# ilya16/isp-tts

Measured on AMD Instinct MI355X. Metric: mel-frames/s (whole node), batch=64 x 512-frame utterances per GPU, full forward incl. MAS, higher is better.
Workload: dtype bf16; 1 GPU; BASELINE config 3: AcousticModel.forward (TextEncoder + Aligner/MAS + TemporalAdaptor 1 flow eval + MelDecoder + to_mel), fixed-length synthetic random-phoneme batch, random-init weights of the recipe architecture (23.2 M params); batch_per_gpu=64, global_batch=64, text_len=100, mel_len=512, parallelism=single GPU, device=gfx950:sramecc+:xnack-, compute_units=256, launch=HIP graph replay, batches_in_flight=1

## Files before the change

include/ispk.h:

```cpp
#ifndef ISPK_H
#define ISPK_H

#include <stdint.h>

#ifdef __cplusplus
extern "C" {
#endif

typedef struct ihipStream_t* ispk_stream_t;

#define ISPK_ABI_VERSION 2

#define ISPK_E_NULL (-1)
#define ISPK_E_SHAPE (-2)
#define ISPK_E_ALIGN (-3)
#define ISPK_E_UNSUPPORTED (-4)

int32_t ispk_abi_version(void);
const char* ispk_last_error_string(void);
int32_t ispk_device_info(char* name, int32_t cap);

int32_t ispk_mas_f32(const float* logits, const int64_t* text_len, const int64_t* mel_len, int16_t* attn_hard,
                     int64_t* dur, int16_t* path, int32_t B, int32_t M_max, int32_t L_max, int64_t stride_b,
                     int64_t stride_m, ispk_stream_t stream);

int32_t ispk_layernorm_f32(const float* x, int64_t ldx, const float* gamma, const float* beta, const float* ada_scale,
                           const float* ada_shift, int64_t ada_stride, int32_t rows_per_batch,
                           const uint8_t* row_mask, float* y, int64_t ldy, int32_t rows, int32_t D, float eps,
                           ispk_stream_t stream);
int32_t ispk_layernorm_f32_bf16(const float* x, int64_t ldx, const float* gamma, const float* beta,
                                const float* ada_scale, const float* ada_shift, int64_t ada_stride,
                                int32_t rows_per_batch, const uint8_t* row_mask, uint16_t* y, int64_t ldy, int32_t rows,
                                int32_t D, float eps, ispk_stream_t stream);

#define ISPK_EP_GELU 1u
#define ISPK_EP_SILU 2u
#define ISPK_EP_MASK_ACC 4u
#define ISPK_EP_MASK_OUT 8u
#define ISPK_EP_BIAS_ROW 16u
#define ISPK_EP_MASK_COL 32u
#define ISPK_EP_OUT_BF16 64u
#define ISPK_EP_RESID_BF16 128u
#define ISPK_EP_DUAL_GELU 1024u
#define ISPK_EP_GELU_BWD 2048u
#define ISPK_EP_OUT_SPLIT 512u
#define ISPK_EP_ROWS_T 256u

int32_t ispk_gemm_f32_tile(int32_t M, int32_t N, int32_t K);
int32_t ispk_gemm_f32(const float* A, int64_t lda, const float* W, int64_t ldw, float* C, int64_t ldc, const float* bias,
                      const float* resid, int64_t ldr, const uint8_t* mask, int32_t M, int32_t N, int32_t K,
                      uint32_t flags, int32_t cols_per_batch, int64_t batch_stride, ispk_stream_t stream);
int32_t ispk_gemm_f32_batched(const float* A, int64_t lda, int64_t stride_a, const float* W, int64_t ldw, int64_t stride_w,
                              float* C, int64_t ldc, int64_t stride_c, int32_t batch, int32_t M, int32_t N, int32_t K,
                              ispk_stream_t stream);
int32_t ispk_gemm_bf16_gelu_train(const uint16_t* A, int64_t lda, const uint16_t* W, int64_t ldw, uint16_t* u, int64_t ldu,
                                  uint16_t* a, int64_t ld_a, int32_t M, int32_t N, int32_t K, float dropout_p, uint64_t seed,
                                  ispk_stream_t stream);
int32_t ispk_gemm_bf16_gelu_bwd(const uint16_t* dY, int64_t lddy, const uint16_t* W2t, int64_t ldw, const uint16_t* u,
                                int64_t ldu, uint16_t* du, int64_t lddu, const uint8_t* row_mask, int32_t M, int32_t N,
                                int32_t K, float dropout_p, uint64_t seed, ispk_stream_t stream);
int32_t ispk_gemm_bf16_last_variant(void);
int32_t ispk_gemm_bf16(const uint16_t* A, int64_t lda, const uint16_t* W, int64_t ldw, void* C, int64_t ldc,
                       const float* bias, const void* resid, int64_t ldr, const uint8_t* mask, int32_t M, int32_t N,
                       int32_t K, uint32_t flags, int32_t cols_per_batch, int64_t batch_stride, ispk_stream_t stream);
int32_t ispk_gemm_bf16_splitk_plan(int32_t M, int32_t N, int32_t K, uint32_t flags);
int32_t ispk_gemm_bf16_splitk(const uint16_t* A, int64_t lda, const uint16_t* W, int64_t ldw, void* C, int64_t ldc,
                              const float* bias, const void* resid, int64_t ldr, const uint8_t* mask, int32_t M, int32_t N,
                              int32_t K, uint32_t flags, float* workspace, int32_t ksplit, ispk_stream_t stream);

int32_t ispk_ffn_bf16(const uint16_t* x, int64_t ldx, const uint16_t* W1, int64_t ldw1, const float* bias1,
                      const uint16_t* W2, int64_t ldw2, const float* bias2, const float* resid, int64_t ldr,
                      const uint8_t* mask, float* out, int64_t ldo, int32_t rows, int32_t dim, int32_t inner, uint32_t flags,
                      ispk_stream_t stream);

int32_t ispk_ffn_bf16_prenorm(const float* x, int64_t ldx, const float* norm_gamma, const float* norm_beta, float norm_eps,
                              const uint16_t* W1, int64_t ldw1, const uint16_t* W2_packed, const float* bias2,
                              const uint8_t* mask, float* out, int64_t ldo, int32_t rows, int32_t dim, int32_t inner,
                              uint32_t flags, float* row_stats, float stats_eps, ispk_stream_t stream);

int32_t ispk_ffn_chunk_w2_bf16(const uint16_t* W2, int64_t ldw2, int32_t dim, int32_t inner, uint16_t* out,
                               ispk_stream_t stream);
int32_t ispk_ffn_bf16_prenorm2_split(const float* x, int64_t ldx, const float* norm_gamma, const float* norm_beta,
                                     float norm_eps, const uint16_t* W1, const uint16_t* W2_chunks, float* parts,
                                     int64_t part_stride, int32_t splits, int32_t rows, int32_t dim, int32_t inner,
                                     ispk_stream_t stream);
int32_t ispk_ffn_combine_ln_f32(const float* x, int64_t ldx, const float* parts, int64_t part_stride, int32_t splits,
                                const uint8_t* mask, float* y, int64_t ldy, const float* ln_gamma, const float* ln_beta,
                                float ln_eps, int32_t ln_mask, void* ln_out, int64_t ld_ln, int32_t ln_bf16, int32_t rows,
                                int32_t dim, ispk_stream_t stream);
int32_t ispk_ffn_bf16_prenorm2(const float* x, int64_t ldx, const float* norm_gamma, const float* norm_beta, float norm_eps,
                               const uint16_t* W1, const uint16_t* W2_chunks, const uint8_t* mask, float* out, int64_t ldo,
                               int32_t rows, int32_t dim, int32_t inner, uint32_t flags, float* row_stats, float stats_eps,
                               ispk_stream_t stream);
int32_t ispk_attn_out_ffn_bf16(const float* x, int64_t ldx, const uint16_t* attn_out, int64_t ld_attn,
                               const uint16_t* Wo_chunks, const float* norm_gamma, const float* norm_beta, float norm_eps,
                               const uint16_t* W1, const uint16_t* W2_chunks, const uint8_t* mask, float* out, int64_t ldo,
                               int32_t rows, int32_t dim, int32_t inner, uint32_t flags, float* row_stats, float stats_eps,
                               ispk_stream_t stream);

int32_t ispk_attn_out_ffn_norm_bf16(const float* x, int64_t ldx, const uint16_t* attn_out, int64_t ld_attn,
                                    const uint16_t* Wo_chunks, const float* norm_gamma, const float* norm_beta, float norm_eps,
                                    const uint16_t* W1, const uint16_t* W2_chunks, const uint8_t* mask, float* out, int64_t ldo,
                                    int32_t rows, int32_t dim, int32_t inner, uint32_t flags, const float* final_gamma,
                                    const float* final_beta, float final_eps, int32_t ln_mask, void* ln_out, int64_t ld_ln,
                                    int32_t ln_bf16, ispk_stream_t stream);
int32_t ispk_attn_out_ffn_split_bf16(const float* x, int64_t ldx, const uint16_t* attn_out, int64_t ld_attn,
                                     const uint16_t* Wo_chunks, const float* norm_gamma, const float* norm_beta, float norm_eps,
                                     const uint16_t* W1, const uint16_t* W2_chunks, const uint8_t* mask, uint32_t flags,
                                     float* parts, int64_t part_stride, int32_t splits, int32_t rows, int32_t dim, int32_t inner,
                                     ispk_stream_t stream);
int32_t ispk_chunk_k16_bf16(const uint16_t* W, int64_t ldw, int32_t N, int32_t K, uint16_t* out, ispk_stream_t stream);
int32_t ispk_attn_out_ffn_qkv_bf16(const float* x, int64_t ldx, const uint16_t* attn_out, int64_t ld_attn,
                                   const uint16_t* Wo_chunks, const float* norm_gamma, const float* norm_beta, float norm_eps,
                                   const uint16_t* W1, const uint16_t* W2_chunks, const uint8_t* mask, float* out, int64_t ldo,
                                   int32_t rows, int32_t dim, int32_t inner, uint32_t flags, const float* next_gamma,
                                   const float* next_beta, float next_eps, const uint16_t* Wqkv_chunks, uint16_t* qkv,
                                   int64_t ld_qkv, ispk_stream_t stream);

int32_t ispk_gemm_bf16_lnin(const float* x, int64_t ldx, const float* row_stats, const float* ln_gamma, const float* ln_beta,
                            float ln_eps, const uint16_t* W, int64_t ldw, void* C, int64_t ldc, const float* bias, const void* resid,
                            int64_t ldr, const uint8_t* mask, int32_t M, int32_t N, int32_t K, uint32_t flags,
                            ispk_stream_t stream);

int32_t ispk_ffn_pack_w2_bf16(const uint16_t* W2, int64_t ldw2, int32_t dim, int32_t inner, uint16_t* packed,
                              ispk_stream_t stream);

int32_t ispk_linear_small_f32(const float* a, int64_t lda, const float* w, int64_t ldw, const float* bias,
                              const float* resid, int64_t ldr, float* out, int64_t ldo, int32_t M, int32_t N, int32_t K,
                              uint32_t act, ispk_stream_t stream);

int32_t ispk_alibi_mqa_attn_f32(const float* q, int64_t ldq, const float* k, const float* v, int64_t ldkv,
                                const float* slopes, const int64_t* key_len, float* out, int64_t ldo, int32_t B,
                                int32_t N, int32_t H, ispk_stream_t stream);
int32_t ispk_alibi_mqa_attn_bf16(const uint16_t* q, int64_t ldq, const uint16_t* k, const uint16_t* v, int64_t ldkv,
                                 const float* slopes, const int64_t* key_len, uint16_t* out, int64_t ldo, int32_t B,
                                 int32_t N, int32_t H, ispk_stream_t stream);
int32_t ispk_alibi_mqa_attn_bf16_tiles(const uint16_t* q, int64_t ldq, const uint16_t* k, const uint16_t* v, int64_t ldkv,
                                       const float* slopes, const int64_t* key_len, uint16_t* out, int64_t ldo, int32_t B,
                                       int32_t N, int32_t H, int32_t q_tiles_per_workgroup, ispk_stream_t stream);

int32_t ispk_pad_rows_f32(const float* x, int64_t stride_b, int64_t stride_t, int64_t stride_c, const int64_t* len,
                          void* out, int32_t out_bf16, int32_t B, int32_t T, int32_t C, ispk_stream_t stream);
int32_t ispk_masked_instnorm_f32(const float* y, const float* weight, const float* bias, const int64_t* len, void* out,
                                 int32_t out_bf16, int32_t B, int32_t T, int32_t C, float eps, ispk_stream_t stream);
int32_t ispk_aligner_scores_f32(const float* q_enc, int64_t q_stride_b, const float* k_enc, int64_t k_stride_b,
                                const int64_t* text_len, const int64_t* mel_len, float* attn_logits, float* attn_soft,
                                int32_t B, int32_t M, int32_t L, int32_t D, ispk_stream_t stream);
int32_t ispk_aligner_scores_fast_f32(const float* q_enc, int64_t q_stride_b, const float* k_enc, int64_t k_stride_b,
                                const int64_t* text_len, const int64_t* mel_len, float* attn_logits, float* attn_soft,
                                int32_t B, int32_t M, int32_t L, int32_t D, ispk_stream_t stream);
int32_t ispk_soft_average_f32(const float* attn_soft, const float* pitch, const float* energy, const int64_t* duration,
                              const int64_t* text_len, float* feats, int32_t B, int32_t M, int32_t L,
                              ispk_stream_t stream);

int32_t ispk_flow_head_f32(const float* y, int64_t ldy, const float* norm_gamma, const float* norm_beta, float norm_eps,
                           const float* W, const float* bias, const float* flow, const float* x0, const uint8_t* mask,
                           float* pred, float* duration, float* loss_ratio, float* loss_mean, float* workspace, int32_t B,
                           int32_t L, int32_t D, int32_t C, ispk_stream_t stream);
int32_t ispk_flow_euler_f32(const float* x_t, const float* velocity, float dt, const uint8_t* mask, float* out, int32_t B,
                            int32_t L, int32_t C, ispk_stream_t stream);
int32_t ispk_infer_features_f32(const float* pred, const float* duration_target_f32, const int64_t* duration_target_i64,
                                const float* pitch_target, const float* energy_target, float duration_factor, float pitch_factor,
                                float pitch_delta, float energy_factor, float energy_delta, float* duration, float* features,
                                int32_t B, int32_t L, ispk_stream_t stream);
int32_t ispk_infer_features_round_f32(const float* pred, const float* duration_target_f32, const int64_t* duration_target_i64,
                                      const float* pitch_target, const float* energy_target, float duration_factor,
                                      float pitch_factor, float pitch_delta, float energy_factor, float energy_delta,
                                      float* duration, float* features, int32_t B, int32_t L, ispk_stream_t stream);
int32_t ispk_flow_mix_f32(const float* x0, const float* x1, const float* t, float sigma, float* x_t, float* flow, int32_t B,
                          int32_t L, int32_t C, ispk_stream_t stream);
int32_t ispk_flow_finish_f32(const float* pred_raw, const float* flow, const float* x0, const uint8_t* mask, float* pred,
                             float* duration, float* loss_ratio, float* loss_mean, int32_t B, int32_t L, int32_t C,
                             ispk_stream_t stream);

int32_t ispk_embed_tokens_f32(const int64_t* text, const float* table, int64_t ld_table, int32_t vocab,
                              const int64_t* text_len, float* emb, uint8_t* mask, int32_t B, int32_t L, int32_t D,
                              ispk_stream_t stream);
int32_t ispk_add_speaker_f32(float* x, const float* table, int64_t ld_table, int32_t speakers, const int64_t* speaker,
                             int32_t id_stride, int32_t B, int32_t L, int32_t D, ispk_stream_t stream);
int32_t ispk_add_speaker_out_f32(const float* x, float* out, const float* table, int64_t ld_table, int32_t speakers,
                                 const int64_t* speaker, int32_t id_stride, int32_t B, int32_t L, int32_t D, ispk_stream_t stream);
int32_t ispk_speaker_grad_f32(const float* d_x, const int64_t* speaker, int32_t id_stride, const int64_t* text_len,
                              float* workspace, int64_t workspace_floats, float* d_table, int64_t ld_table, int32_t speakers,
                              int32_t B, int32_t L, int32_t D, int32_t accumulate, ispk_stream_t stream);
int32_t ispk_time_embedding_f32(const float* t, int32_t n, const float* inv_freq, const float* freq_scale, int32_t half_dim,
                                const float* w0, const float* b0, const float* w1, const float* b1, int32_t emb_dim,
                                float* out, ispk_stream_t stream);
int32_t ispk_length_regulate_f32(const float* alignment, const float* dur_f32, const int64_t* dur_i64, const int64_t* enc_len,
                                 const float* x, int64_t ldx, float* out, int64_t* dec_len, uint8_t* dec_mask, int32_t B,
                                 int32_t M, int32_t L, int32_t D, int32_t max_len, int32_t dur_cols, ispk_stream_t stream);
int32_t ispk_length_regulate_split_bf16(const float* alignment, const float* dur_f32, const int64_t* dur_i64, const int64_t* enc_len,
                                 const float* x, int64_t ldx, float* out, int64_t* dec_len, uint8_t* dec_mask, int32_t B,
                                 int32_t M, int32_t L, int32_t D, int32_t max_len, int32_t dur_cols, ispk_stream_t stream);
int32_t ispk_length_regulate_split_f16(const float* alignment, const float* dur_f32, const int64_t* dur_i64, const int64_t* enc_len,
                                const float* x, int64_t ldx, float* out, int64_t* dec_len, uint8_t* dec_mask, int32_t B,
                                int32_t M, int32_t L, int32_t D, int32_t max_len, int32_t dur_cols, ispk_stream_t stream);

int32_t ispk_hard_regulate_f32(const float* dur_f32, const int64_t* dur_i64, const float* x, int64_t ldx, float* out,
                               int64_t* dec_len, uint8_t* dec_mask, int32_t B, int32_t frames, int32_t L, int32_t D,
                               int32_t max_len, ispk_stream_t stream);
int32_t ispk_hard_regulate_bwd_f32(const float* dur_f32, const int64_t* dur_i64, const float* d_out, float* d_x, int32_t B,
                                   int32_t rows, int32_t L, int32_t D, int32_t max_len, ispk_stream_t stream);
int32_t ispk_hard_average_f32(const float* pitch, const float* energy, const int64_t* duration, const int64_t* text_len,
                              float* feats, int32_t B, int32_t M, int32_t L, ispk_stream_t stream);

int32_t ispk_transpose_f32(const float* x, int64_t ldx, float* y, int64_t ldy, int32_t rows, int32_t cols,
                           ispk_stream_t stream);
int32_t ispk_gemm_tn_f32(const float* A, int64_t lda, const float* B, int64_t ldb, float* C, int64_t ldc, int32_t M,
                         int32_t N1, int32_t N2, const uint8_t* row_mask, int32_t accumulate, float* workspace,
                         int64_t workspace_floats, ispk_stream_t stream);
int32_t ispk_gemm_tn_bf16(const float* A, int64_t lda, const float* B, int64_t ldb, float* C, int64_t ldc, int32_t M,
                          int32_t N1, int32_t N2, const uint8_t* row_mask, int32_t accumulate, float* workspace,
                          int64_t workspace_floats, ispk_stream_t stream);
int32_t ispk_gemm_tn_b16(const uint16_t* A, int64_t lda, const uint16_t* B, int64_t ldb, float* C, int64_t ldc, int32_t M,
                         int32_t N1, int32_t N2, const uint8_t* row_mask, int32_t accumulate, float* workspace,
                         int64_t workspace_floats, ispk_stream_t stream);
int32_t ispk_gemm_tn_last_plan(int32_t* splits, int32_t* rows_per_split);
int32_t ispk_gemm_tn_batched_f32(const float* A, int64_t lda, int64_t stride_a, const float* B, int64_t ldb, int64_t stride_b,
                                 float* C, int64_t ldc, int64_t stride_c, int32_t batch, int32_t M, int32_t N1, int32_t N2,
                                 const uint8_t* row_mask, int32_t accumulate, float* workspace, int64_t workspace_floats,
                                 ispk_stream_t stream);
int32_t ispk_layernorm_bwd_f32(const float* x, int64_t ldx, const float* dy, int64_t lddy, const float* gamma,
                               const uint8_t* row_mask, float* dx, int64_t lddx, int32_t add_to_dx, float* dgamma,
                               float* dbeta, float* workspace, int64_t workspace_floats, int64_t rows, int32_t dim,
                               float eps, ispk_stream_t stream);
int32_t ispk_layernorm_bwd_dual_f32(const float* x, int64_t ldx, const float* dy, int64_t lddy, const float* gamma,
                                    const uint8_t* row_mask, float* dx, int64_t lddx, int32_t add_to_dx, float* dgamma,
                                    float* dbeta, float* workspace, int64_t workspace_floats, int64_t rows, int32_t dim,
                                    float eps, uint16_t* dx_bf16, int64_t ld_dx_bf16, ispk_stream_t stream);
int32_t ispk_gelu_f32(const float* u, float* a, int64_t n, float dropout_p, uint64_t seed, ispk_stream_t stream);
int32_t ispk_gelu_bwd_f32(const float* da, const float* u, float* du, int64_t n, float dropout_p, uint64_t seed,
                          ispk_stream_t stream);
int32_t ispk_gelu_f32_bf16(const float* u, uint16_t* a, int64_t n, float dropout_p, uint64_t seed, ispk_stream_t stream);
int32_t ispk_gelu_bwd_bf16(const uint16_t* da, const float* u, uint16_t* du, int64_t n, float dropout_p, uint64_t seed,
                           ispk_stream_t stream);
int32_t ispk_gelu_bf16(const uint16_t* u, uint16_t* a, int64_t n, float dropout_p, uint64_t seed, ispk_stream_t stream);
int32_t ispk_gelu_bwd_b16(const uint16_t* da, const uint16_t* u, uint16_t* du, int64_t n, float dropout_p, uint64_t seed,
                          ispk_stream_t stream);
int32_t ispk_dropout_mask_u8(uint8_t* out, int64_t n, float dropout_p, uint64_t seed, ispk_stream_t stream);
int32_t ispk_alibi_mqa_attn_train_f32(const float* qkv, int64_t ld_qkv, const float* slopes, const int64_t* key_len, float* o,
                                      int64_t ld_o, float* lse, int32_t B, int32_t N, int32_t H, float dropout_p, uint64_t seed,
                                      ispk_stream_t stream);
int32_t ispk_alibi_mqa_attn_bwd_f32(const float* qkv, int64_t ld_qkv, const float* o, const float* d_o, int64_t ld_o,
                                    const float* slopes, const int64_t* key_len, float* dqkv, float* dlogslopes,
                                    float* workspace, int64_t workspace_floats, int32_t B, int32_t N, int32_t H,
                                    const float* lse_in, float dropout_p, uint64_t seed, ispk_stream_t stream);
int32_t ispk_alibi_mqa_attn_train_bf16(const uint16_t* qkv, int64_t ld_qkv, const float* slopes, const int64_t* key_len,
                                       uint16_t* o, int64_t ld_o, float* lse, int32_t B, int32_t N, int32_t H, float dropout_p,
                                       uint64_t seed, ispk_stream_t stream);
int32_t ispk_alibi_mqa_attn_bwd_bf16(const uint16_t* qkv, int64_t ld_qkv, const uint16_t* o, const uint16_t* d_o, int64_t ld_o,
                                     const float* slopes, const int64_t* key_len, const float* lse, uint16_t* dqkv,
                                     float* dlogslopes, float* workspace, int64_t workspace_floats, int32_t B, int32_t N,
                                     int32_t H, float dropout_p, uint64_t seed, ispk_stream_t stream);
int32_t ispk_mel_loss_f32(const float* mel_out, const float* mel_target, const int64_t* mel_len, float* ratio, float* loss,
                          float* grad, float grad_out, int32_t B, int32_t C, int32_t T, ispk_stream_t stream);
int32_t ispk_acoustic_metrics_f32(const float* mel_out, int64_t out_sb, int64_t out_sc, int64_t out_st, const float* mel_target,
                                  int64_t tgt_sb, int64_t tgt_sc, int64_t tgt_st, const int64_t* mel_len, const int64_t* text_len,
                                  const float* attn_soft, int64_t attn_sb, int64_t attn_st, const float* dct, float* workspace,
                                  int64_t workspace_floats, float* out, int32_t B, int32_t C, int32_t T, int32_t L,
                                  int32_t n_mfcc, ispk_stream_t stream);
int32_t ispk_dtw_f32(const float* cost, int64_t cost_sb, int64_t cost_sn, const int64_t* n_len, const int64_t* m_len,
                     float* total, int32_t* steps, int16_t* path, float* workspace, int64_t workspace_floats, int32_t B,
                     int32_t N, int32_t M, ispk_stream_t stream);
int32_t ispk_mcd_dtw_f32(const float* mel_out, int64_t out_sb, int64_t out_sc, int64_t out_st, const float* mel_target,
                         int64_t tgt_sb, int64_t tgt_sc, int64_t tgt_st, const float* dct, const int64_t* n_len,
                         const int64_t* m_len, const float* pitch_out, int64_t pitch_out_sb, const float* pitch_target,
                         int64_t pitch_target_sb, float* workspace, int64_t workspace_floats, float* per_item, float* means,
                         float* cost_out, int32_t B, int32_t C, int32_t N, int32_t M, int32_t n_mfcc, ispk_stream_t stream);
int32_t ispk_audio_features_f32(const float* audio, int64_t ld_audio, const int64_t* audio_len, const float* tables,
                                int64_t table_floats, const int32_t* fb_index, int32_t n_mels, float* mel, int64_t* mel_len, float* pitch, float* energy,
                                int32_t B, int32_t S, int32_t M, int32_t tau_min, int32_t tau_max, float sample_rate,
                                float threshold, float pitch_mean, float pitch_std, ispk_stream_t stream);
int32_t ispk_resample_f32(const float* audio, int64_t ld_b, int64_t ld_c, const int64_t* audio_len, const float* taps,
                          int64_t tap_floats, const int32_t* first, float* out, int64_t ld_out, int64_t* out_len, int32_t B,
                          int32_t C, int32_t S, int32_t S_out, int32_t orig, int32_t dest, int32_t width, int32_t T,
                          ispk_stream_t stream);
int32_t ispk_feature_stats_f64(const float* pitch, int64_t ld_pitch, const float* energy, int64_t ld_energy,
                               const int64_t* mel_len, double* partial, double* state, int32_t B, int32_t M, int32_t reset,
                               ispk_stream_t stream);
int32_t ispk_audio_measure_f64(const float* audio, int64_t ld_audio, const int64_t* audio_len, const double* table,
                               int64_t table_doubles, int64_t* bounds, double* loudness, float* peak, float* gain,
                               float* workspace, int64_t workspace_floats, int32_t B, int32_t S, int32_t sample_rate,
                               int32_t trim_mode, double trim_threshold, int32_t pad_frames, int32_t gain_mode,
                               double target_lufs, double peak_limit, ispk_stream_t stream);
int32_t ispk_audio_apply_f32(const float* audio, int64_t ld_audio, const int64_t* bounds, const float* gain, float* out,
                             int64_t ld_out, int64_t* out_len, int32_t B, int32_t S, int32_t S_out, ispk_stream_t stream);
int32_t ispk_pcm16(const float* audio, int64_t ld_audio, const int64_t* audio_len, int16_t* out, int64_t ld_out, int32_t B,
                   int32_t S, int32_t dither, uint64_t seed, ispk_stream_t stream);
int32_t ispk_vocoder_unfold(const void* mel, int32_t mel_f16, int64_t sb, int64_t sc, int64_t st, const int64_t* mel_len,
                            void* rows, int32_t rows_bf16, int64_t ldr, uint8_t* row_mask, int32_t B, int32_t C, int32_t T,
                            int32_t K, ispk_stream_t stream);
int32_t ispk_dwconv7_ln_f32(const float* x, int64_t ldx, const float* w, const float* bias, const float* gamma,
                            const float* beta, float eps, const int64_t* mel_len, void* y, int32_t y_bf16, int64_t ldy,
                            int32_t B, int32_t T, int32_t D, ispk_stream_t stream);
int32_t ispk_istft_head_f32(const float* h, int64_t ldh, const int64_t* mel_len, const float* tables, int64_t table_floats,
                            float* audio, int64_t ld_audio, int64_t* audio_len, int32_t B, int32_t T, int32_t S,
                            ispk_stream_t stream);
int32_t ispk_aligner_scores_bwd_f32(const float* attn_logits, const float* attn_soft, const float* d_soft, const float* d_logits,
                                    const int64_t* text_len, const int64_t* mel_len, float* dS, int64_t ld_s, float* dSt,
                                    int64_t ld_t, int32_t B, int32_t M, int32_t L, float scale, ispk_stream_t stream);
int32_t ispk_masked_instnorm_bwd_f32(const float* y, const float* d_out, const float* weight, const int64_t* lengths, float* d_y,
                                     float* d_weight, float* d_bias, float* workspace, int64_t workspace_floats, int32_t B,
                                     int32_t T, int32_t C, float eps, ispk_stream_t stream);
int32_t ispk_soft_average_bwd_f32(const float* attn_soft, const float* pitch, const float* energy, const float* d_feats,
                                  const int64_t* text_len, float* workspace, int64_t workspace_floats, float* d_attn,
                                  int32_t accumulate, int32_t B, int32_t M, int32_t L, ispk_stream_t stream);
int32_t ispk_flow_loss_bwd_f32(const float* pred_raw, const float* flow, const uint8_t* mask, float grad_out, float* d_raw, int32_t B,
                               int32_t L, int32_t C, ispk_stream_t stream);
int32_t ispk_adaln_bwd_f32(const float* x, int64_t ldx, const float* dy, int64_t lddy, const float* scale, int64_t ld_scale,
                           const uint8_t* row_mask, float* dx, int64_t lddx, int32_t add_to_dx, float* dscale, float* dshift,
                           int64_t ld_out, int32_t B, int32_t rows_per_batch, int32_t dim, float eps, ispk_stream_t stream);
int32_t ispk_time_embedding_bwd_f32(const float* t, int32_t n, const float* inv_freq, const float* freq_scale, int32_t half_dim,
                                    const float* w0, const float* b0, const float* w1, int32_t emb_dim, const float* d_out,
                                    float* dw0, float* db0, float* dw1, float* db1, ispk_stream_t stream);
int32_t ispk_attn_ctc_loss_f32(const float* attn_logits, const int64_t* text_len, const int64_t* mel_len, float blank_logprob,
                               float* workspace, int64_t workspace_floats, float* loss, float* grad, float grad_out, int32_t B,
                               int32_t M, int32_t L, ispk_stream_t stream);
int32_t ispk_attn_bin_loss_f32(const float* attn_soft, const int16_t* attn_hard, float eps, float* workspace, float* loss,
                               float* grad, float grad_out, int32_t B, int32_t M, int32_t L, ispk_stream_t stream);
int32_t ispk_mel_grad_rows_f32(const float* dmel, const uint8_t* mask, float* g, int32_t B, int32_t C, int32_t T,
                               ispk_stream_t stream);
int32_t ispk_colsum_f32(const float* x, int64_t ldx, int64_t rows, int32_t cols, const uint8_t* row_mask, float* workspace,
                        int64_t workspace_floats, float* out, ispk_stream_t stream);
int32_t ispk_smallk_wgrad_f32(const float* g, int64_t ldg, const float* x, int64_t ldx, int64_t rows, int32_t N, int32_t K,
                              float* workspace, int64_t workspace_floats, float* out, ispk_stream_t stream);
int32_t ispk_embedding_bwd_f32(const int64_t* ids, const float* d_emb, int64_t rows, int32_t dim, int32_t vocab,
                               int32_t padding_idx, float* d_table, int64_t ld_table, ispk_stream_t stream);
int32_t ispk_grad_sqnorm_f32(const float* g, int64_t n, float* partial, float* out, ispk_stream_t stream);
int32_t ispk_adamw_f32(float* p, const float* g, float* m, float* v, int64_t n, int64_t n_decay, float lr, float beta1,
                       float beta2, float eps, float weight_decay, int32_t step, const float* grad_sqnorm, float max_norm,
                       float grad_scale, ispk_stream_t stream);

int32_t ispk_split_f16(const float* x, int64_t ldx, uint16_t* hi, uint16_t* lo, int64_t ldy, int32_t rows, int32_t cols,
                       ispk_stream_t stream);
int32_t ispk_gemm_split_f16_tile(int32_t M, int32_t N, int32_t K);
int32_t ispk_gemm_split_f16(const uint16_t* A, int64_t lda, int64_t a_plane, const uint16_t* W, int64_t ldw, int64_t w_plane,
                            void* C, int64_t ldc, int64_t c_plane, const float* bias, const float* resid, int64_t ldr,
                            const uint8_t* mask, int32_t M, int32_t N, int32_t K, uint32_t flags, int32_t cols_per_batch,
                            int64_t batch_stride, ispk_stream_t stream);
int32_t ispk_layernorm_f32_split(const float* x, int64_t ldx, const float* gamma, const float* beta, const float* ada_scale,
                                 const float* ada_shift, int64_t ada_stride, int32_t rows_per_batch, const uint8_t* row_mask,
                                 uint16_t* y_hi, int64_t ldy, int64_t y_plane, int32_t rows, int32_t D, float eps,
                                 ispk_stream_t stream);
int32_t ispk_alibi_mqa_attn_split_f16(const float* q, int64_t ldq, const float* k, const float* v, int64_t ldkv,
                                      const float* slopes, const int64_t* key_len, void* out, int64_t ldo, int64_t o_plane,
                                      int32_t B, int32_t N, int32_t H, ispk_stream_t stream);
// ... 49 lines not shown
```

isp_tts_amd/acoustic/model.py:

```python
from __future__ import annotations

import warnings
from typing import NamedTuple, Optional

import torch
import torch.nn as nn
import torch.nn.functional as F
from torch import Tensor

from .. import runtime
from ..staging import StagedWeights
from ..modules.constructor import Constructor
from ..modules.transformer import Transformer
from ..utils import get_mask_from_lengths
from .alignment import Aligner, AlignerOutput
from .temporal_adaptor import FlowTemporalAdaptor, TemporalAdaptorOutput


class AcousticModelOutput(NamedTuple):
    mel: Tensor
    adaptor_output: TemporalAdaptorOutput
    aligner_output: AlignerOutput
    loss: Optional[Tensor] = None
    losses: Optional[dict] = None


class AcousticModel(nn.Module, Constructor):
    def __init__(self, encoding_map: dict, mel_dim: int, text_dim: int = 384, encoder=None, decoder=None,
                 temporal_adaptor=None, aligner=None, num_speakers: Optional[int] = 0, pitch_mean=None, pitch_std=None,
                 speaker_in_forward: bool = False):
        super().__init__()
        self.encoding_map = dict(encoding_map)
        self.mel_dim, self.text_dim = mel_dim, text_dim
        self.text_embedding = nn.Embedding(len(encoding_map), text_dim, padding_idx=0)
        self.encoder = Transformer.init(encoder, emb_dim=text_dim)
        enc_dim = self.encoder.dim
        self.aligner = Aligner.init(aligner, mel_dim=mel_dim, text_dim=enc_dim)
        self.speaker_embedding = None
        if (num_speakers or 0) > 0:
            self.speaker_embedding = nn.Embedding(num_speakers, enc_dim)
            nn.init.xavier_uniform_(self.speaker_embedding.weight)
        self.speaker_in_forward = bool(speaker_in_forward)
        self.train_amp: Optional[bool] = None
        self.temporal_adaptor = FlowTemporalAdaptor.init(temporal_adaptor, encoder_dim=enc_dim)
        self.decoder = Transformer.init(decoder, emb_dim=enc_dim)
        self.to_mel = nn.Linear(self.decoder.dim, mel_dim)
        self.overlap_streams = True
        self._side_streams: dict = {}
        self.register_buffer("pitch_mean", torch.tensor(float(pitch_mean or 0.)))
        self.register_buffer("pitch_std", torch.tensor(float(pitch_std or 1.)))
        self.compute_dtype = torch.float32
        self._cache = StagedWeights()

    def set_compute_dtype(self, dtype: torch.dtype, *, alignment_dtype: Optional[torch.dtype] = None):
        chain = alignment_dtype if alignment_dtype is not None else dtype
        assert chain in (torch.float32, torch.bfloat16, torch.float16)
        self.encoder.set_compute_dtype(chain)
        self.decoder.set_compute_dtype(dtype)
        self.temporal_adaptor.predictor.transformer.set_compute_dtype(dtype)
        self.temporal_adaptor.embedding.transformer.set_compute_dtype(dtype)
        self.aligner.attention.compute_dtype = chain
        self.temporal_adaptor.length_regulator.split_bf16 = (True if dtype == torch.bfloat16 else
                                                             "f16" if dtype == torch.float16 else False)
        self.compute_dtype = dtype
        return self

    def _to_mel(self, dec_out: Tensor, dec_mask: Optional[Tensor]) -> Tensor:
        w = self.to_mel.weight
        if dec_out.dtype == torch.float16:
            ws = self._cache.get(torch.float16, (w,), lambda: runtime.split_f16(w.detach().float().contiguous()))
            return runtime.to_mel_split(dec_out, ws, self.to_mel.bias, dec_mask)
        if dec_out.dtype == torch.bfloat16:
            w = self._cache.get(torch.bfloat16, (w,), lambda: w.detach().to(torch.bfloat16).contiguous())
        return runtime.to_mel(dec_out, w, self.to_mel.bias, dec_mask)

    def forward(self, text: Tensor, text_len: Tensor, mel: Tensor, mel_len: Tensor, pitch: Optional[Tensor] = None,
                energy: Optional[Tensor] = None, speaker: Optional[Tensor] = None, sigma: float = 0., steps: int = 1, *,
                flow_noise: Optional[Tensor] = None, flow_time: Optional[Tensor] = None) -> AcousticModelOutput:
        if self.speaker_embedding is None:
            speaker = None
        elif not self.speaker_in_forward:
            raise AttributeError(f"'{type(self).__name__}' object has no attribute 'speaker_encoder'")
        elif speaker is None:
            raise ValueError("speaker_in_forward is on and the model has a speaker table: forward() needs `speaker` "
                             "([B, 1] int64 ids, or a single id for the whole batch)")
        if torch.is_grad_enabled() and text.is_cuda and any(p.requires_grad for p in self.parameters()):
            from ..train.model import acoustic_train_outputs
            amp = self.train_amp if self.train_amp is not None else torch.is_autocast_enabled("cuda")
            train_aligner = any(p.requires_grad for p in self.aligner.parameters())
            with torch.autocast("cuda", enabled=False):
                return acoustic_train_outputs(self, text, text_len, mel, mel_len, pitch, energy, flow_noise, flow_time, amp=amp,
                                              train_aligner=train_aligner, speaker=speaker)
        with torch.no_grad():
            return self._forward_values(text, text_len, mel, mel_len, pitch, energy, flow_noise=flow_noise, flow_time=flow_time,
                                        speaker=speaker)

    def _forward_values(self, text: Tensor, text_len: Tensor, mel: Tensor, mel_len: Tensor, pitch: Optional[Tensor] = None,
                        energy: Optional[Tensor] = None, *, flow_noise: Optional[Tensor] = None,
                        flow_time: Optional[Tensor] = None, speaker: Optional[Tensor] = None) -> AcousticModelOutput:
        q_proj = None
        if mel.is_cuda and self.overlap_streams:
            main = torch.cuda.current_stream()
            side = self._side_streams.setdefault(mel.device, torch.cuda.Stream(device=mel.device))
            side.wait_stream(main)
            with torch.cuda.stream(side):
                q_proj = self.aligner.attention.project_queries(mel, mel_len)
        token_emb, enc_mask = runtime.embed_tokens(text, self.text_embedding.weight, text_len)
        enc_out = self.encoder(token_emb, mask=enc_mask, key_len=text_len).out
        if q_proj is not None:
            main.wait_stream(side)
            q_proj.record_stream(main)
        branch = side if q_proj is not None else None
        hard = not self.temporal_adaptor.soft_duration
        aligner_output = self.aligner(mel=mel, enc_text=enc_out.transpose(1, 2).detach(), mel_len=mel_len,
                                      text_len=text_len, q_proj=q_proj, mas_stream=None if hard else branch)
        if speaker is not None:
            enc_out = runtime.add_speaker(enc_out, self.speaker_embedding.weight, speaker)
        adaptor_output = self.temporal_adaptor(
            enc_out=enc_out, enc_mask=enc_mask, max_dec_len=mel.size(2),
            duration_target=aligner_output.attn_hard_duration, alignment=aligner_output.attn_soft,
            pitch_target_dense=pitch, energy_target_dense=energy, noise=flow_noise, time_steps=flow_time,
            enc_len=text_len, predictor_stream=branch, duration_sum=mel_len if branch is not None and not hard else None)
        dec_len = adaptor_output.dec_lengths
        dec_mask = adaptor_output.dec_mask
        dec_out = self.decoder(adaptor_output.enc_out, mask=dec_mask, key_len=dec_len, out_dtype=self.compute_dtype).out
        mel_out = self._to_mel(dec_out, dec_mask)
        if q_proj is not None:
            main.wait_stream(side)
            for t in (adaptor_output.log_duration, adaptor_output.duration, adaptor_output.pitch, adaptor_output.energy,
                      aligner_output.attn_hard, aligner_output.attn_hard_duration, *(adaptor_output.losses or {}).values()):
                if isinstance(t, Tensor):
                    t.record_stream(main)
        return AcousticModelOutput(mel=mel_out, adaptor_output=adaptor_output, aligner_output=aligner_output)

    @torch.no_grad()
    def forward_front(self, text: Tensor, text_len: Tensor, mel: Tensor, mel_len: Tensor, pitch: Tensor, energy: Tensor):
        main = torch.cuda.current_stream()
        side = self._side_streams.setdefault(mel.device, torch.cuda.Stream(device=mel.device))
        side.wait_stream(main)
        with torch.cuda.stream(side):
            q_proj = self.aligner.attention.project_queries(mel, mel_len)
        token_emb, enc_mask = runtime.embed_tokens(text, self.text_embedding.weight, text_len)
        enc_out = self.encoder(token_emb, mask=enc_mask, key_len=text_len).out
        main.wait_stream(side)
        q_proj.record_stream(main)
        attn_soft, attn_logits = self.aligner.attention(mel, enc_out.transpose(1, 2).detach(), mel_len, text_len,
                                                        q_proj=q_proj)
        feats = runtime.soft_average(attn_soft, pitch, energy, None, text_len)
        return {"enc_out": enc_out, "enc_mask": enc_mask, "attn_soft": attn_soft, "attn_logits": attn_logits, "feats": feats}

    @torch.no_grad()
    def forward_side(self, st: dict, text_len: Tensor, mel_len: Tensor, pitch: Tensor, energy: Tensor,
                     flow_noise: Optional[Tensor], flow_time: Optional[Tensor]):
        attn_hard, dur = self.aligner.binarize_attention_parallel(st["attn_logits"], text_len, mel_len, return_duration=True)
        ad = self.temporal_adaptor
        targets = runtime.soft_average(st["attn_soft"], pitch, energy, dur, text_len)
        pred, losses = ad.predictor(st["enc_out"], targets, st["enc_mask"][..., None], noise=flow_noise, time_steps=flow_time,
                                    key_len=text_len)
        return {"attn_hard": attn_hard, "dur": dur, "pred": pred, "losses": losses,
                "duration_pred": ad.predictor._duration_estimate}

    @torch.no_grad()
    def forward_back(self, st: dict, text_len: Tensor, mel_len: Tensor, max_dec_len: int):
        ad = self.temporal_adaptor
        feats = st["feats"]
        x = ad.embedding(feats[..., 1:3], mask=st["enc_mask"][..., None], key_len=text_len, residual=st["enc_out"])
        dec_in, dec_len = ad.length_regulator(x, mel_len.view(-1, 1), max_len=max_dec_len, alignment=st["attn_soft"])
        dec_mask = ad.length_regulator.dec_mask
        dec_out = self.decoder(dec_in, mask=dec_mask, key_len=dec_len, out_dtype=self.compute_dtype).out
        return {"mel": self._to_mel(dec_out, dec_mask), "dec_in": dec_in, "dec_len": dec_len, "dec_mask": dec_mask}

    @staticmethod
    def assemble_output(front: dict, side: dict, back: dict) -> AcousticModelOutput:
        feats, pred = front["feats"], side["pred"]
        adaptor = TemporalAdaptorOutput(enc_out=back["dec_in"], log_duration=pred[..., 0], duration=side["duration_pred"],
                                        dec_lengths=back["dec_len"], pitch=pred[..., 1], energy=pred[..., 2],
                                        pitch_target=feats[..., 1], energy_target=feats[..., 2], losses=side["losses"],
                                        dec_mask=back["dec_mask"])
        aligner = AlignerOutput(attn_soft=front["attn_soft"], attn_logits=front["attn_logits"], attn_hard=side["attn_hard"],
                                attn_hard_duration=side["dur"])
        return AcousticModelOutput(mel=back["mel"], adaptor_output=adaptor, aligner_output=aligner)

    @torch.no_grad()
    def infer(self, input_sequence: Tensor, text_lengths: Optional[Tensor] = None,
              duration_target: Optional[Tensor] = None, duration_factor: float = 1.0,
              pitch_target: Optional[Tensor] = None, pitch_factor: float = 1.0, pitch_delta: float = 0.,
              pitch_normalize: bool = False, energy_target: Optional[Tensor] = None, steps: int = 4,
              speaker: Optional[Tensor] = None, *, flow_noise: Optional[Tensor] = None,
              max_dec_len: Optional[int] = None):
        batch_infer = input_sequence.shape[0] > 1
        token_emb, enc_mask = runtime.embed_tokens(input_sequence, self.text_embedding.weight,
                                                   text_lengths if batch_infer else None, want_mask=batch_infer)
        enc_out = self.encoder(token_emb, mask=enc_mask, key_len=text_lengths if batch_infer else None).out
        if self.speaker_embedding is not None and speaker is not None:
            enc_out = runtime.add_speaker_(enc_out, self.speaker_embedding.weight, speaker)
        if pitch_normalize:
            if pitch_target is not None:
                pitch_target = (pitch_target - self.pitch_mean) / self.pitch_std
            pitch_delta = pitch_delta / self.pitch_std
        adaptor_output = self.temporal_adaptor.infer(
            enc_out=enc_out, enc_mask=enc_mask, duration_target=duration_target, pitch_target=pitch_target,
            energy_target=energy_target, duration_factor=duration_factor, pitch_factor=pitch_factor,
            pitch_delta=pitch_delta, steps=steps, noise=flow_noise, max_dec_len=max_dec_len,
            enc_len=text_lengths if batch_infer else None)
        dec_mask = adaptor_output.dec_mask if batch_infer else None
        dec_out = self.decoder(adaptor_output.enc_out, mask=dec_mask, key_len=adaptor_output.dec_lengths if batch_infer else None,
                               out_dtype=self.compute_dtype).out
        return self._to_mel(dec_out, dec_mask), adaptor_output

    @classmethod
    def from_pretrained(cls, checkpoint_path: str, strict: bool = True) -> "AcousticModel":
        checkpoint = torch.load(checkpoint_path, map_location="cpu", weights_only=False)
        model = cls.init(checkpoint["model"]["config"])
        state_dict = dict(checkpoint["model"]["state_dict"])
        for key, weight in model.state_dict().items():
            if key not in state_dict:
                state_dict[key] = weight
        model.load_state_dict(state_dict, strict=strict)
        return model

    def load(self, state_dict: dict, ignore_layers: Optional[list] = None, ignore_mismatched_keys: bool = False):
        own = self.state_dict()
        extra = [k for k in state_dict if k not in own]
        if extra:
            warnings.warn(f"checkpoint keys absent from the model are ignored: {extra}")
        kept = {k: v for k, v in state_dict.items() if k in own}
        ignored = []
        if ignore_mismatched_keys:
            ignored += [k for k, v in kept.items() if v.shape != own[k].shape]
        if ignore_layers:
            ignored += [k for k in kept if any(layer in k for layer in ignore_layers)]
        kept = {k: v for k, v in kept.items() if k not in ignored}
        own.update(kept)
        self.load_state_dict(own)
        return self

    def freeze(self, exception_list: Optional[list] = None):
        exception_list = exception_list or []
        for name, param in self.named_parameters():
            param.requires_grad = any(name.startswith(layer) for layer in exception_list)
        return self

    def extend_speakers(self, count: int) -> int:
        if self.speaker_embedding is None:
            raise ValueError("extend_speakers: the model has no speaker table (num_speakers = 0)")
        if count < 1:
            raise ValueError(f"extend_speakers: count = {count}")
        old = self.speaker_embedding.weight
        first = old.shape[0]
        table = nn.Embedding(first + count, old.shape[1], device=old.device, dtype=old.dtype)
        with torch.no_grad():
            table.weight[:first] = old
            table.weight[first:] = old.double().mean(dim=0).to(old.dtype)
        table.weight.requires_grad_(old.requires_grad)
        self.speaker_embedding = table
        return first

    def prepare_inputs(self, inputs: dict) -> dict:
        return {"text": inputs["text_vector"], "text_len": inputs["text_vector_len"], "mel": inputs["mel"],
                "mel_len": inputs["mel_len"], "pitch": inputs["pitch"], "energy": inputs["energy"],
                "speaker": inputs.get("speaker")}
```

isp_tts_amd/acoustic/temporal_adaptor.py:

```python
from __future__ import annotations

from typing import NamedTuple, Optional

import torch
import torch.nn as nn
import torch.nn.functional as F
from torch import Tensor

from .. import runtime
from ..staging import StagedWeights
from ..modules.constructor import Constructor
from ..modules.transformer import Transformer, TimePositionalEmbedding
from ..utils import get_float_mask_from_lengths, get_mask_3d, masked_mean


class TransformerTemporalModule(nn.Module, Constructor):

    def __init__(self, input_dim: int = 256, output_dim: int = 256, transformer=None, detach_inputs: bool = False):
        super().__init__()
        self.transformer = Transformer.init(transformer, emb_dim=input_dim)
        self.linear_layer = nn.Linear(self.transformer.dim, output_dim, bias=True)
        self.detach_inputs = detach_inputs
        self._cache = StagedWeights()

    def _weight(self, dtype: torch.dtype) -> Tensor:
        w = self.linear_layer.weight
        if dtype == torch.float16:
            return self._cache.get(dtype, (w,), lambda: runtime.split_f16(w.detach().float().contiguous()))
        return self._cache.get(dtype, (w,), lambda: w.detach().to(dtype).contiguous())

    def forward(self, x: Tensor, mask: Optional[Tensor] = None, *, key_len: Optional[Tensor] = None,
                residual: Optional[Tensor] = None) -> Tensor:
        m2 = mask[..., 0] if mask is not None else None
        cdt = self.transformer.layers[0].attention.compute_dtype
        out = self.transformer(x, mask=m2, out_dtype=cdt, key_len=key_len if m2 is not None else None).out
        flags = runtime.EP_MASK_ACC if m2 is not None else 0
        if cdt == torch.float16:
            return runtime.gemm_split(out, self._weight(cdt), bias=self.linear_layer.bias, mask=m2, flags=flags, resid=residual)
        return runtime.gemm(out, self._weight(cdt), bias=self.linear_layer.bias, mask=m2, flags=flags, resid=residual,
                            out_dtype=torch.float32)

    def infer(self, x: Tensor, mask: Optional[Tensor] = None, steps: int = 4) -> Tensor:
        return self.forward(x, mask)


class FlowTransformerTemporalModule(nn.Module, Constructor):

    def __init__(self, input_dim: int = 256, output_dim: int = 256, transformer=None,
                 time_embedding_dim: Optional[int] = None, sigma: float = 1e-5, detach_inputs: bool = False):
        super().__init__()
        time_embedding_dim = time_embedding_dim or input_dim
        self.time_embedding = TimePositionalEmbedding(freq_dim=64, emb_dim=time_embedding_dim, with_steps=True)
        self.transformer = Transformer.init(transformer, emb_dim=output_dim + input_dim, adaptive_norm=True,
                                            condition_dim=time_embedding_dim)
        self.linear_layer = nn.Linear(self.transformer.dim, output_dim, bias=True)
        self.output_dim, self.sigma, self.detach_inputs = output_dim, sigma, detach_inputs
        self.fused_head = True
        self._cache = StagedWeights()
        self._grids: dict = {}

    def _cond_weight(self, dtype: torch.dtype) -> Tensor:
        w = self.transformer.project_emb.weight
        if dtype == torch.float16:
            return self._cache.get(dtype, (w,), lambda: runtime.split_f16(w.detach()[:, self.output_dim:].float().contiguous()))
        return self._cache.get(dtype, (w,), lambda: w.detach()[:, self.output_dim:].to(dtype).contiguous())

    def _project(self, x_t: Tensor, cond_proj: Tensor) -> Tensor:
        w = self.transformer.project_emb.weight
        return runtime.linear_small(x_t.contiguous(), w[:, :self.output_dim], None, resid=cond_proj)

    def _cond_projection(self, cond: Tensor) -> Tensor:
        cdt = self.transformer.layers[0].attention.compute_dtype
        c = cond.float().contiguous()
        if cdt == torch.float16:
            return runtime.gemm_split(runtime.split_f16(c), self._cond_weight(cdt), bias=self.transformer.project_emb.bias)
        if cdt == torch.bfloat16:
            c = runtime.cast_bf16(c)
        return runtime.gemm(c, self._cond_weight(cdt), bias=self.transformer.project_emb.bias, out_dtype=torch.float32)

    def forward(self, x: Tensor, targets: Tensor, mask: Optional[Tensor] = None, *, noise: Optional[Tensor] = None,
                time_steps: Optional[Tensor] = None, key_len: Optional[Tensor] = None):
        cond = x
        have_mask = mask is not None
        if mask is None:
            mask = torch.ones(x.shape[:2], dtype=torch.bool, device=x.device)
        elif mask.ndim == 3:
            mask = mask[..., 0]
        x1 = targets.detach()
        x0 = torch.randn_like(x1) if noise is None else noise.to(x1)
        t = torch.rand((x1.shape[0],), dtype=x1.dtype, device=x1.device) if time_steps is None else time_steps.to(x1)
        time_emb = self.time_embedding(t)
        x_t, flow = runtime.flow_mix(x0, x1, t, self.sigma)
        proj = self._project(x_t, self._cond_projection(cond))
        tr = self.transformer
        head = (self.fused_head and tr.dim == 256 and self.output_dim == 3 and tr.norm.weight is not None and tr.norm.bias is not None
                and self.linear_layer.bias is not None)
        out = tr(None, mask=mask, adaptive_condition=time_emb, projected=proj, key_len=key_len if have_mask else None,
                 final_norm=not head).out
        if head:
            pred, self._duration_estimate, _, loss = runtime.flow_head(out, tr.norm.weight, tr.norm.bias, tr.norm.eps,
                                                                       self.linear_layer.weight, self.linear_layer.bias, flow, x0, mask)
            return pred, {"flow_loss": loss}
        raw = runtime.linear_small(out, self.linear_layer.weight, self.linear_layer.bias)
        pred, self._duration_estimate, _, loss = runtime.flow_finish(raw, flow, x0, mask)
        return pred, {"flow_loss": loss}

    def euler_grid(self, steps: int, step_factor: float, device=None) -> Tensor:
        assert step_factor <= 1.
        key = (int(steps), float(step_factor))
        grid = self._grids.get(key)
        if grid is None:
            if step_factor == 1.:
                grid = torch.linspace(0, 1, steps + 1)
            else:
                ts = -torch.diff(torch.logspace(0, steps, steps + 1, base=step_factor))
                ts = torch.cat([torch.zeros(1), ts])
                grid = torch.cumsum(ts / ts.sum(), dim=0)
            self._grids[key] = grid
        return grid if device is None else grid.to(device)

    def infer(self, x: Tensor, mask: Optional[Tensor] = None, steps: int = 4, step_factor: float = 0.75, *,
              noise: Optional[Tensor] = None, key_len: Optional[Tensor] = None) -> Tensor:
        dev = x.device
        if mask is not None and mask.ndim == 3:
            mask = mask.squeeze(-1)
        x_t = (torch.randn(x.shape[0], x.shape[1], self.output_dim, device=dev) if noise is None
               else noise.to(device=dev, dtype=torch.float32))
        dts = self._grids.get(("dt", int(steps), float(step_factor)))
        if dts is None:
            ts = self.euler_grid(steps, step_factor)
            dts = self._grids[("dt", int(steps), float(step_factor))] = (ts[1:] - ts[:-1]).tolist()
        temb = self.time_embedding(self._grid_on(dev, steps, step_factor)[:steps])
        cond_proj = self._cond_projection(x)
        if mask is not None and key_len is None:
            key_len = mask.sum(dim=1)
        for i in range(steps):
            out = self.transformer(None, mask=mask, adaptive_condition=temb[i].view(1, 1, -1),
                                   projected=self._project(x_t, cond_proj), key_len=key_len).out
            vel = runtime.linear_small(out, self.linear_layer.weight, self.linear_layer.bias)
            x_t = runtime.flow_euler(x_t, vel, dts[i], mask if i == steps - 1 else None)
        return x_t

    def _grid_on(self, device, steps: int, step_factor: float) -> Tensor:
        key = (str(device), int(steps), float(step_factor))
        g = self._grids.get(key)
        if g is None:
            g = self._grids[key] = self.euler_grid(steps, step_factor).to(device)
        return g


class TemporalAdaptorOutput(NamedTuple):
    enc_out: Tensor
    log_duration: Optional[Tensor]
    duration: Tensor
    dec_lengths: Tensor
    pitch: Optional[Tensor]
    energy: Optional[Tensor]
    pitch_target: Optional[Tensor]
    energy_target: Optional[Tensor]
    losses: Optional[dict] = None
    dec_mask: Optional[Tensor] = None


class LengthRegulator(nn.Module):
    split_bf16 = False

    def forward(self, x: Tensor, durations: Tensor, max_len: Optional[int] = None, alignment: Optional[Tensor] = None, *,
                enc_len: Optional[Tensor] = None, frames: Optional[int] = None, hard: bool = False):
        if alignment is None and (hard or frames is None or durations.dtype == torch.int64):
            if frames is None:
                frames = int((durations.float() + 0.5).long().sum(dim=1).max().item())
            if max_len is not None:
                frames = min(frames, max_len)
            if frames == 0:
                self.dec_mask = torch.zeros((x.shape[0], 0), dtype=torch.bool, device=x.device)
                return x.new_zeros((x.shape[0], 0, x.shape[2])), torch.zeros((x.shape[0],), dtype=torch.int64, device=x.device)
            out, dec_lens, self.dec_mask = runtime.hard_regulate(x.float(), durations, frames,
                                                                 max_len=-1 if max_len is None else max_len)
            return out, dec_lens
        rows = alignment.shape[1] if alignment is not None else frames
        if max_len is not None and alignment is not None:
            rows = min(rows, max_len)
            alignment = alignment[:, :rows]
        out, dec_lens, self.dec_mask = runtime.length_regulate(x.float(), durations, alignment, rows,
                                                               max_len=-1 if max_len is None else max_len, enc_len=enc_len,
                                                               split_bf16=self.split_bf16)
        return out, dec_lens


class TemporalAverager(nn.Module):

    def forward(self, x: Tensor, durations: Tensor, alignment: Optional[Tensor] = None) -> Tensor:
        if alignment is None:
            b, c, _ = x.shape
            if durations.dtype != torch.int64:
                ends = torch.cumsum(durations, dim=1).long()
                durations = torch.diff(ends, dim=1, prepend=torch.zeros_like(ends[:, :1]))
            every = torch.full((b,), durations.shape[1], dtype=torch.int64, device=x.device)
            cols = []
            for i in range(0, c, 2):
                f = runtime.hard_average(x[:, i], x[:, min(i + 1, c - 1)], durations, every)
                cols.append(f[..., 1:min(3, 1 + c - i)])
            return torch.cat(cols, dim=-1).transpose(1, 2)
        return x @ alignment / (alignment.sum(dim=1, keepdim=True) + 1e-5)


def generate_soft_path(duration: Tensor, mask: Tensor) -> Tensor:
    b, t_x, t_y = mask.shape
    cum = torch.cumsum(duration, 1).view(b * t_x)
    path = get_float_mask_from_lengths(cum, t_y).to(mask.dtype).view(b, t_x, t_y)
    path = path - F.pad(path, [0, 0, 1, 0, 0, 0])[:, :-1]
    return path * mask


class FlowTemporalAdaptor(nn.Module, Constructor):
    predictor_first = False

    def __init__(self, encoder_dim: int = 384, predictor=None, embedding=None, pitch: bool = True, energy: bool = True,
                 soft_duration: bool = False):
        super().__init__()
        if not (pitch and energy):
            raise NotImplementedError("built with pitch and energy both on (either duration mode): without one of them the "
                                      "feature tensors change shape")
        self.length_regulator = LengthRegulator()
        self.averager = TemporalAverager()
        self.encoder_dim = encoder_dim
        self.feature_dim = 3
        self.pitch, self.energy, self.soft_duration = pitch, energy, soft_duration
        self.pitch_idx, self.energy_idx = 1, 2
        self.predictor = FlowTransformerTemporalModule.init(predictor, input_dim=encoder_dim, output_dim=self.feature_dim)
        self.embedding = TransformerTemporalModule.init(embedding, input_dim=self.feature_dim - 1, output_dim=encoder_dim)

    def _process_target(self, dense: Tensor, duration_target: Tensor, alignment: Tensor, enc_mask: Tensor) -> Tensor:
        if dense.ndim == 2:
            dense = dense[:, None]
        return self.averager(dense, duration_target, alignment).transpose(1, 2) * enc_mask

    def forward(self, enc_out: Tensor, enc_mask: Tensor, max_dec_len: int, duration_target: Optional[Tensor] = None,
                alignment: Optional[Tensor] = None, pitch_target_dense: Optional[Tensor] = None,
                energy_target_dense: Optional[Tensor] = None, *, noise: Optional[Tensor] = None,
                time_steps: Optional[Tensor] = None, enc_len: Optional[Tensor] = None,
                predictor_stream=None, duration_sum: Optional[Tensor] = None) -> TemporalAdaptorOutput:
        assert duration_target is not None and (alignment is not None or not self.soft_duration)
        assert pitch_target_dense is not None and energy_target_dense is not None
        hard = not self.soft_duration
        m3 = enc_mask[..., None]
        if enc_len is None:
            enc_len = enc_mask.sum(dim=1)
        side = predictor_stream if (predictor_stream is not None and enc_out.is_cuda) else None
        cond = enc_out
        if hard:
            alignment = None
            targets = runtime.hard_average(pitch_target_dense, energy_target_dense, duration_target, enc_len)
            feats = targets
            len_src = duration_target
        elif side is None or duration_sum is None:
            targets = runtime.soft_average(alignment, pitch_target_dense, energy_target_dense, duration_target, enc_len)
            feats = targets
            len_src = duration_target
        else:
            feats = runtime.soft_average(alignment, pitch_target_dense, energy_target_dense, None, enc_len)
            targets = None
            len_src = duration_sum.view(-1, 1)
        if side is not None:
            ready = torch.cuda.Event()
            ready.record()
        pitch_target, energy_target = feats[..., 1:2], feats[..., 2:3]
        features = feats[..., 1:3]

        def decoder_input(enc_out_):
            enc_out_ = self.embedding(features, mask=m3, key_len=enc_len, residual=enc_out_)
            return self.length_regulator(enc_out_, len_src, max_len=max_dec_len, alignment=alignment,
                                         frames=max_dec_len if hard else None)

        if not (side is not None and self.predictor_first):
            enc_out, dec_lens = decoder_input(enc_out)

        def predict():
            tg = targets
            if tg is None:
                tg = runtime.soft_average(alignment, pitch_target_dense, energy_target_dense, duration_target, enc_len)
            pred_, losses_ = self.predictor(cond, tg, m3, noise=noise, time_steps=time_steps, key_len=enc_len)
            return pred_, losses_, self.predictor._duration_estimate

        if side is not None:
            side.wait_event(ready)
            with torch.cuda.stream(side):
                pred, losses, duration_pred = predict()
            for t in (cond, feats, alignment, pitch_target_dense, energy_target_dense):
                if t is not None:
                    t.record_stream(side)
            if self.predictor_first:
                enc_out, dec_lens = decoder_input(enc_out)
        else:
            pred, losses, duration_pred = predict()
        log_duration_pred = pred[..., 0]
        return TemporalAdaptorOutput(enc_out=enc_out, log_duration=log_duration_pred, duration=duration_pred,
                                     dec_lengths=dec_lens, pitch=pred[..., 1], energy=pred[..., 2],
                                     pitch_target=pitch_target.squeeze(-1), energy_target=energy_target.squeeze(-1),
                                     losses=losses, dec_mask=self.length_regulator.dec_mask)

    def infer(self, enc_out: Tensor, enc_mask: Optional[Tensor] = None, duration_target: Optional[Tensor] = None,
              duration_factor: float = 1.0, pitch_target: Optional[Tensor] = None, pitch_factor: float = 1.0,
              pitch_delta: float = 0., energy_target: Optional[Tensor] = None, energy_factor: float = 1.0,
              energy_delta: float = 0., steps: int = 4, *, noise: Optional[Tensor] = None,
              max_dec_len: Optional[int] = None, enc_len: Optional[Tensor] = None) -> TemporalAdaptorOutput:
        m3 = enc_mask[..., None] if enc_mask is not None else None
        pred = self.predictor.infer(enc_out, mask=m3, steps=steps, noise=noise, key_len=enc_len)
        duration_pred, feats = runtime.infer_features(pred, duration_target, pitch_target, energy_target, duration_factor,
                                                      pitch_factor, pitch_delta, energy_factor, energy_delta,
                                                      round_duration=not self.soft_duration)
        pitch, energy = feats[..., 0:1], feats[..., 1:2]
        enc_out = self.embedding(feats, residual=enc_out)
        enc_lens = enc_len
        if enc_lens is None and enc_mask is not None:
            enc_lens = enc_mask.sum(dim=1)
        if not self.soft_duration:
            enc_out, dec_lens = self.length_regulator(enc_out, duration_pred, alignment=None, frames=max_dec_len, hard=True)
            return TemporalAdaptorOutput(enc_out=enc_out, log_duration=None, duration=duration_pred, dec_lengths=dec_lens,
                                         pitch=pitch.squeeze(-1), energy=energy.squeeze(-1), pitch_target=pitch_target,
                                         energy_target=energy_target, dec_mask=self.length_regulator.dec_mask)
        if max_dec_len is None:
            max_dec_len = int((duration_pred.sum(dim=1) + 0.5).long().max().item())
        enc_out, dec_lens = self.length_regulator(enc_out, duration_pred, alignment=None, enc_len=enc_lens,
                                                  frames=max_dec_len)
        return TemporalAdaptorOutput(enc_out=enc_out, log_duration=None, duration=duration_pred, dec_lengths=dec_lens,
                                     pitch=pitch.squeeze(-1), energy=energy.squeeze(-1), pitch_target=pitch_target,
                                     energy_target=energy_target, dec_mask=self.length_regulator.dec_mask)
```

isp_tts_amd/csrc/glue.hip:

```cpp
#include "common.h"

namespace {

__global__ __launch_bounds__(256) void embed_tokens_kernel(const int64_t* __restrict__ text, const float* __restrict__ table,
                                                           int64_t ld_table, int vocab, const int64_t* __restrict__ text_len,
                                                           float* __restrict__ emb, uint8_t* __restrict__ mask, int rows,
                                                           int L, int D) {
    const int row = blockIdx.x * 4 + (threadIdx.x >> 6), lane = threadIdx.x & 63;
    if (row >= rows) return;
    int64_t id = text[row];
    id = (id < 0 || id >= vocab) ? 0 : id;
    const f32x4* src = reinterpret_cast<const f32x4*>(table + id * ld_table);
    f32x4* dst = reinterpret_cast<f32x4*>(emb + (int64_t)row * D);
    for (int c = lane; c < D / 4; c += 64) dst[c] = src[c];
    if (mask && lane == 0) {
        const int b = row / L, l = row - b * L;
        mask[row] = text_len ? (uint8_t)(l < text_len[b]) : (uint8_t)1;
    }
}

__device__ __forceinline__ int64_t speaker_row(const int64_t* __restrict__ speaker, int b, int id_stride, int speakers) {
    const int64_t id = speaker[(int64_t)b * id_stride];
    return id < 0 ? 0 : (id >= speakers ? speakers - 1 : id);
}

__global__ __launch_bounds__(256) void add_speaker_kernel(float* __restrict__ x, const float* __restrict__ table, int64_t ld_table,
                                                          int speakers, const int64_t* __restrict__ speaker, int id_stride,
                                                          int rows, int L, int D) {
    const int row = blockIdx.x * 4 + (threadIdx.x >> 6), lane = threadIdx.x & 63;
    if (row >= rows) return;
    const int64_t id = speaker_row(speaker, row / L, id_stride, speakers);
    const f32x4* src = reinterpret_cast<const f32x4*>(table + id * ld_table);
    f32x4* dst = reinterpret_cast<f32x4*>(x + (int64_t)row * D);
    for (int c = lane; c < D / 4; c += 64) {
        f32x4 v = dst[c];
        const f32x4 e = src[c];
        v[0] += e[0]; v[1] += e[1]; v[2] += e[2]; v[3] += e[3];
        dst[c] = v;
    }
}

__global__ __launch_bounds__(256) void add_speaker_out_kernel(const float* __restrict__ x, float* __restrict__ out,
                                                              const float* __restrict__ table, int64_t ld_table, int speakers,
                                                              const int64_t* __restrict__ speaker, int id_stride, int rows,
                                                              int L, int D) {
    const int row = blockIdx.x * 4 + (threadIdx.x >> 6), lane = threadIdx.x & 63;
    if (row >= rows) return;
    const int64_t id = speaker_row(speaker, row / L, id_stride, speakers);
    const f32x4* src = reinterpret_cast<const f32x4*>(table + id * ld_table);
    const f32x4* in = reinterpret_cast<const f32x4*>(x + (int64_t)row * D);
    f32x4* dst = reinterpret_cast<f32x4*>(out + (int64_t)row * D);
    for (int c = lane; c < D / 4; c += 64) {
        f32x4 v = in[c];
        const f32x4 e = src[c];
        v[0] += e[0]; v[1] += e[1]; v[2] += e[2]; v[3] += e[3];
        dst[c] = v;
    }
}

constexpr int kSgRows = 16;
__device__ __forceinline__ int speaker_grad_len(const int64_t* __restrict__ text_len, int b, int L) {
    if (!text_len) return L;
    const int64_t n = text_len[b];
    return n < 0 ? 0 : (n > L ? L : (int)n);
}

__global__ __launch_bounds__(256) void speaker_grad_stage1_kernel(const float* __restrict__ d_x, const int64_t* __restrict__ text_len,
                                                                  float* __restrict__ part, int L, int D, int chunks) {
    __shared__ f32x4 sums[3][64];
    const int b = blockIdx.z, chunk = blockIdx.y, wave = threadIdx.x >> 6, lane = threadIdx.x & 63;
    const int n = speaker_grad_len(text_len, b, L), r0 = chunk * kSgRows;
    if (r0 >= n) return;
    const int r1 = r0 + kSgRows < n ? r0 + kSgRows : n, c = blockIdx.x * 64 + lane;
    const bool live = c < D / 4;
    f32x4 s = {0.f, 0.f, 0.f, 0.f};
    if (live)
        for (int r = r0 + wave; r < r1; r += 4) {
            const f32x4 v = *reinterpret_cast<const f32x4*>(d_x + ((int64_t)b * L + r) * D + 4 * c);
            s[0] += v[0]; s[1] += v[1]; s[2] += v[2]; s[3] += v[3];
        }
    if (wave > 0) sums[wave - 1][lane] = s;
    __syncthreads();
    if (wave == 0 && live) {
#pragma unroll
        for (int w = 0; w < 3; ++w) {
            const f32x4 v = sums[w][lane];
            s[0] += v[0]; s[1] += v[1]; s[2] += v[2]; s[3] += v[3];
        }
        *reinterpret_cast<f32x4*>(part + ((int64_t)b * chunks + chunk) * D + 4 * c) = s;
    }
}

__global__ __launch_bounds__(256) void speaker_grad_stage2_kernel(const float* __restrict__ part, const int64_t* __restrict__ speaker,
                                                                  int id_stride, const int64_t* __restrict__ text_len,
                                                                  float* __restrict__ d_table, int64_t ld_table, int speakers,
                                                                  int B, int L, int D, int chunks, int accumulate) {
    __shared__ f32x4 sums[3][64];
    const int s = blockIdx.x, wave = threadIdx.x >> 6, lane = threadIdx.x & 63, c = blockIdx.y * 64 + lane;
    const bool live = c < D / 4;
    f32x4 acc = {0.f, 0.f, 0.f, 0.f};
    for (int b = wave; b < B; b += 4) {
        if (speaker_row(speaker, b, id_stride, speakers) != s) continue;
        const int nk = (speaker_grad_len(text_len, b, L) + kSgRows - 1) / kSgRows;
        const float* src = part + (int64_t)b * chunks * D + 4 * c;
        for (int k0 = 0; k0 < nk && live; k0 += 8) {
            f32x4 v[8];
#pragma unroll
            for (int u = 0; u < 8; ++u)
                if (k0 + u < nk) v[u] = *reinterpret_cast<const f32x4*>(src + (int64_t)(k0 + u) * D);
#pragma unroll
            for (int u = 0; u < 8; ++u)
                if (k0 + u < nk) { acc[0] += v[u][0]; acc[1] += v[u][1]; acc[2] += v[u][2]; acc[3] += v[u][3]; }
        }
    }
    if (wave > 0) sums[wave - 1][lane] = acc;
    __syncthreads();
    if (wave == 0 && live) {
#pragma unroll
        for (int w = 0; w < 3; ++w) {
            const f32x4 v = sums[w][lane];
            acc[0] += v[0]; acc[1] += v[1]; acc[2] += v[2]; acc[3] += v[3];
        }
        f32x4* dst = reinterpret_cast<f32x4*>(d_table + (int64_t)s * ld_table + 4 * c);
        if (accumulate) {
            const f32x4 old = *dst;
            acc[0] += old[0]; acc[1] += old[1]; acc[2] += old[2]; acc[3] += old[3];
        }
        *dst = acc;
    }
}

__global__ __launch_bounds__(64) void time_embedding_kernel(const float* __restrict__ t, const float* __restrict__ inv_freq,
                                                            const float* __restrict__ freq_scale, int H,
                                                            const float* __restrict__ w0, const float* __restrict__ b0,
                                                            const float* __restrict__ w1, const float* __restrict__ b1,
                                                            int E, float* __restrict__ out) {
#pragma clang fp contract(off)
    __shared__ float f[1 + 2 * 64];
    __shared__ float h[64];
    const int n = blockIdx.x, j = threadIdx.x;
    const float pos = t[n], fs = freq_scale[0];
    if (j == 0) f[0] = pos;
    for (int i = j; i < H; i += 64) {
        const float a = pos * fs * inv_freq[i];
        f[1 + i] = sinf(a);
        f[1 + H + i] = cosf(a);
    }
    __syncthreads();
    const int K0 = 1 + 2 * H;
    if (j < E) {
        float acc = b0[j];
        for (int k = 0; k < K0; ++k) acc = fmaf(f[k], w0[(int64_t)j * K0 + k], acc);
        h[j] = acc / (1.0f + expf(-acc));
    }
    __syncthreads();
    if (j < E) {
        float acc = b1[j];
        for (int k = 0; k < E; ++k) acc = fmaf(h[k], w1[(int64_t)j * E + k], acc);
        out[(int64_t)n * E + j] = acc;
    }
}

constexpr int kLrRows = 64, kLrChunk = 16, kLrAld = kLrChunk + 1;

typedef uint32_t lr_u32x4 __attribute__((ext_vector_type(4)));
typedef _Float16 lr_f16x8 __attribute__((ext_vector_type(8)));
template <int kSplit>
__device__ __forceinline__ void lr_split8(const float (&v)[8], bf16x8& hi, bf16x8& lo) {
    typedef float f2 __attribute__((ext_vector_type(2)));
    union { lr_u32x4 u; bf16x8 f; } h, l;
#pragma unroll
    for (int e = 0; e < 4; ++e) {
        f2 a;
        a.x = v[2 * e]; a.y = v[2 * e + 1];
        if constexpr (kSplit == 2) {
            typedef _Float16 h2 __attribute__((ext_vector_type(2)));
            a.x = __builtin_amdgcn_fmed3f(a.x, -65504.0f, 65504.0f);
            a.y = __builtin_amdgcn_fmed3f(a.y, -65504.0f, 65504.0f);
            h2 ph, pl;
            ph.x = (_Float16)a.x; ph.y = (_Float16)a.y;
            pl.x = (_Float16)(a.x - (float)ph.x); pl.y = (_Float16)(a.y - (float)ph.y);
            h.u[e] = __builtin_bit_cast(uint32_t, ph);
            l.u[e] = __builtin_bit_cast(uint32_t, pl);
        } else {
            typedef __bf16 bf2 __attribute__((ext_vector_type(2)));
            const uint32_t ph = __builtin_bit_cast(uint32_t, __builtin_convertvector(a, bf2));
            f2 r;
            r.x = a.x - __builtin_bit_cast(float, ph << 16);
            r.y = a.y - __builtin_bit_cast(float, ph & 0xffff0000u);
            h.u[e] = ph;
            l.u[e] = __builtin_bit_cast(uint32_t, __builtin_convertvector(r, bf2));
        }
    }
    hi = h.f;
    lo = l.f;
}
template <int kSplit>
__device__ __forceinline__ f32x16 lr_mfma(const bf16x8& a, const bf16x8& b, const f32x16& c) {
    if constexpr (kSplit == 2)
        return __builtin_amdgcn_mfma_f32_32x32x16_f16(__builtin_bit_cast(lr_f16x8, a), __builtin_bit_cast(lr_f16x8, b), c, 0, 0, 0);
    else
        return __builtin_amdgcn_mfma_f32_32x32x16_bf16(a, b, c, 0, 0, 0);
}

template <int NT, int kSplit = 0>
__global__ __launch_bounds__(256) void length_regulate_kernel(const float* __restrict__ align, const float* __restrict__ dur_f,
                                                              const int64_t* __restrict__ dur_i,
                                                              const int64_t* __restrict__ enc_len,
                                                              const float* __restrict__ x, int64_t ldx,
                                                              float* __restrict__ out, int64_t* __restrict__ dec_len,
                                                              uint8_t* __restrict__ dec_mask, int M, int L, int max_len,
                                                              int dur_cols) {
    constexpr int D = 128 * NT;
    extern __shared__ __attribute__((aligned(16))) char smem[];
    int64_t& s_dec = *reinterpret_cast<int64_t*>(smem);
    float* As = reinterpret_cast<float*>(smem + 16);
    float* Xs = As + kLrRows * kLrAld;
    float* cum = Xs + kLrChunk * D;
    const int b = blockIdx.y, y0 = blockIdx.x * kLrRows, tid = threadIdx.x, lane = tid & 63, wave = __builtin_amdgcn_readfirstlane(tid >> 6);
    const bool soft = align == nullptr;

    if (wave == 0) {
        int64_t dl;
        if (dur_i) {
            int64_t s = 0;
            for (int t = lane; t < dur_cols; t += 64) s += dur_i[(int64_t)b * dur_cols + t];
#pragma unroll
            for (int off = 32; off > 0; off >>= 1) s += __shfl_xor(s, off, 64);
            dl = (int64_t)((float)s + 0.5f);
        } else {
            float s = 0.f;
            if (lane == 0) {
                cum[0] = 0.f;
                for (int t = 0; t < L; ++t) {
                    s += dur_f[(int64_t)b * L + t];
                    cum[t + 1] = s;
                }
            }
            s = __builtin_bit_cast(float, __builtin_amdgcn_readfirstlane(__builtin_bit_cast(int, s)));
            dl = (int64_t)(s + 0.5f);
        }
        if (max_len >= 0 && dl > max_len) dl = max_len;
        if (lane == 0) {
            s_dec = dl;
            if (blockIdx.x == 0) dec_len[b] = dl;
        }
    }
    __syncthreads();
    const int64_t dl = s_dec;
    if (dec_mask)
        for (int r = tid; r < kLrRows; r += 256)
            if (y0 + r < M) dec_mask[(int64_t)b * M + y0 + r] = (uint8_t)(y0 + r < dl);
    const int el = enc_len ? (int)enc_len[b] : L;

    f32x16 acc[2][NT];
#pragma unroll
    for (int rt = 0; rt < 2; ++rt)
#pragma unroll
        for (int ct = 0; ct < NT; ++ct)
#pragma unroll
            for (int i = 0; i < 16; ++i) acc[rt][ct][i] = 0.f;

    const float* xb = x + (int64_t)b * L * ldx;
    const float* ab = soft ? nullptr : align + (int64_t)b * M * L;
    float ar[4];
    f32x4 xr[D / 64];
    const int a_row = tid >> 2, a_k = (tid & 3) * 4, x_t = tid >> 4, x_c = tid & 15;
    auto fetch = [&](int t0) {
        const int y = y0 + a_row;
#pragma unroll
        for (int u = 0; u < 4; ++u) {
            const int t = t0 + a_k + u;
            float v = 0.f;
            if (y < M && t < L) {
                if (!soft) {
                    v = ab[(int64_t)y * L + t];
                } else {
                    const float fy = (float)y;
                    const float hi = fminf(fmaxf(cum[t + 1] - fy, 0.f), 1.f), lo = fminf(fmaxf(cum[t] - fy, 0.f), 1.f);
                    v = (t < el && y < dl) ? hi - lo : 0.f;
                }
            }
            ar[u] = v;
        }
        const int t = t0 + x_t;
#pragma unroll
        for (int i = 0; i < D / 64; ++i) {
            f32x4 v = {0.f, 0.f, 0.f, 0.f};
            if (t < L) v = *reinterpret_cast<const f32x4*>(xb + (int64_t)t * ldx + (x_c + 16 * i) * 4);
            xr[i] = v;
        }
    };
    auto stash = [&]() {
#pragma unroll
        for (int u = 0; u < 4; ++u) As[a_row * kLrAld + a_k + u] = ar[u];
#pragma unroll
        for (int i = 0; i < D / 64; ++i) *reinterpret_cast<f32x4*>(Xs + x_t * D + (x_c + 16 * i) * 4) = xr[i];
    };

    fetch(0);
    for (int t0 = 0; t0 < L; t0 += kLrChunk) {
        __syncthreads();
        stash();
        __syncthreads();
        if (t0 + kLrChunk < L) fetch(t0 + kLrChunk);
        const int r = lane & 31, kh = lane >> 5;
        if constexpr (kSplit != 0) {
            bf16x8 ah[2], al[2];
#pragma unroll
            for (int rt = 0; rt < 2; ++rt) {
                float av[8];
#pragma unroll
                for (int e = 0; e < 8; ++e) av[e] = As[(32 * rt + r) * kLrAld + 8 * kh + e];
                lr_split8<kSplit>(av, ah[rt], al[rt]);
            }
#pragma unroll
            for (int ct = 0; ct < NT; ++ct) {
                float bv[8];
#pragma unroll
                for (int e = 0; e < 8; ++e) bv[e] = Xs[(8 * kh + e) * D + wave * (32 * NT) + ct * 32 + r];
                bf16x8 bh, bl;
                lr_split8<kSplit>(bv, bh, bl);
#pragma unroll
                for (int rt = 0; rt < 2; ++rt) {
                    acc[rt][ct] = lr_mfma<kSplit>(al[rt], bh, acc[rt][ct]);
                    acc[rt][ct] = lr_mfma<kSplit>(ah[rt], bl, acc[rt][ct]);
                    acc[rt][ct] = lr_mfma<kSplit>(ah[rt], bh, acc[rt][ct]);
                }
            }
            continue;
        }
#pragma unroll
        for (int kk = 0; kk < kLrChunk; kk += 2) {
            const float a0 = As[r * kLrAld + kk + kh], a1 = As[(32 + r) * kLrAld + kk + kh];
#pragma unroll
            for (int ct = 0; ct < NT; ++ct) {
                const float bv = Xs[(kk + kh) * D + wave * (32 * NT) + ct * 32 + r];
                acc[0][ct] = __builtin_amdgcn_mfma_f32_32x32x2f32(a0, bv, acc[0][ct], 0, 0, 0);
                acc[1][ct] = __builtin_amdgcn_mfma_f32_32x32x2f32(a1, bv, acc[1][ct], 0, 0, 0);
            }
        }
    }
    float* ob = out + (int64_t)b * M * D;
#pragma unroll
    for (int rt = 0; rt < 2; ++rt)
#pragma unroll
        for (int ct = 0; ct < NT; ++ct)
#pragma unroll
            for (int i = 0; i < 16; ++i) {
                const int y = y0 + rt * 32 + (i & 3) + 8 * (i >> 2) + 4 * (lane >> 5);
                if (y < M) ob[(int64_t)y * D + wave * (32 * NT) + ct * 32 + (lane & 31)] = acc[rt][ct][i];
            }
}

}

extern "C" int32_t ispk_embed_tokens_f32(const int64_t* text, const float* table, int64_t ld_table, int32_t vocab,
                                         const int64_t* text_len, float* emb, uint8_t* mask, int32_t B, int32_t L,
                                         int32_t D, ispk_stream_t stream) {
    ISPK_REQUIRE(text && table && emb, ISPK_E_NULL, "embed_tokens: null pointer");
    ISPK_REQUIRE(B >= 0 && L >= 1 && D >= 4 && vocab >= 1, ISPK_E_SHAPE, "embed_tokens: bad shape B=%d L=%d D=%d V=%d", B, L,
                 D, vocab);
    ISPK_REQUIRE(D % 4 == 0 && ld_table % 4 == 0 && ld_table >= D && ispk_aligned(table, 16) && ispk_aligned(emb, 16),
                 ISPK_E_ALIGN, "embed_tokens: D / ld_table must be multiples of 4 and table / emb 16-byte aligned");
    if (B == 0) return 0;
    const int rows = B * L;
    hipLaunchKernelGGL(embed_tokens_kernel, dim3((rows + 3) / 4), dim3(256), 0, reinterpret_cast<hipStream_t>(stream), text,
                       table, ld_table, vocab, text_len, emb, mask, rows, L, D);
    return ispk_launch_status();
}

extern "C" int32_t ispk_add_speaker_f32(float* x, const float* table, int64_t ld_table, int32_t speakers, const int64_t* speaker,
                                        int32_t id_stride, int32_t B, int32_t L, int32_t D, ispk_stream_t stream) {
    ISPK_REQUIRE(x && table && speaker, ISPK_E_NULL, "add_speaker: null pointer");
    ISPK_REQUIRE(B >= 0 && L >= 1 && D >= 4 && speakers >= 1 && (id_stride == 0 || id_stride == 1), ISPK_E_SHAPE,
                 "add_speaker: bad shape B=%d L=%d D=%d speakers=%d id_stride=%d", B, L, D, speakers, id_stride);
    ISPK_REQUIRE(D % 4 == 0 && ld_table % 4 == 0 && ld_table >= D && ispk_aligned(table, 16) && ispk_aligned(x, 16),
                 ISPK_E_ALIGN, "add_speaker: D / ld_table must be multiples of 4 and table / x 16-byte aligned");
    if (B == 0) return 0;
    const int rows = B * L;
    hipLaunchKernelGGL(add_speaker_kernel, dim3((rows + 3) / 4), dim3(256), 0, reinterpret_cast<hipStream_t>(stream), x, table,
                       ld_table, speakers, speaker, id_stride, rows, L, D);
    return ispk_launch_status();
}

extern "C" int32_t ispk_add_speaker_out_f32(const float* x, float* out, const float* table, int64_t ld_table, int32_t speakers,
                                            const int64_t* speaker, int32_t id_stride, int32_t B, int32_t L, int32_t D,
                                            ispk_stream_t stream) {
    ISPK_REQUIRE(x && out && table && speaker, ISPK_E_NULL, "add_speaker_out: null pointer");
    ISPK_REQUIRE(B >= 0 && L >= 1 && D >= 4 && speakers >= 1 && (id_stride == 0 || id_stride == 1), ISPK_E_SHAPE,
                 "add_speaker_out: bad shape B=%d L=%d D=%d speakers=%d id_stride=%d", B, L, D, speakers, id_stride);
    ISPK_REQUIRE(D % 4 == 0 && ld_table % 4 == 0 && ld_table >= D && ispk_aligned(table, 16) && ispk_aligned(x, 16) &&
                     ispk_aligned(out, 16),
                 ISPK_E_ALIGN, "add_speaker_out: D / ld_table must be multiples of 4 and table / x / out 16-byte aligned");
    ISPK_REQUIRE(x != out, ISPK_E_UNSUPPORTED, "add_speaker_out: x and out are the same buffer (ispk_add_speaker_f32 works in place)");
    if (B == 0) return 0;
    const int rows = B * L;
    hipLaunchKernelGGL(add_speaker_out_kernel, dim3((rows + 3) / 4), dim3(256), 0, reinterpret_cast<hipStream_t>(stream), x, out,
                       table, ld_table, speakers, speaker, id_stride, rows, L, D);
    return ispk_launch_status();
}

extern "C" int32_t ispk_speaker_grad_f32(const float* d_x, const int64_t* speaker, int32_t id_stride, const int64_t* text_len,
                                         float* workspace, int64_t workspace_floats, float* d_table, int64_t ld_table,
                                         int32_t speakers, int32_t B, int32_t L, int32_t D, int32_t accumulate,
                                         ispk_stream_t stream) {
    ISPK_REQUIRE(d_x && speaker && workspace && d_table, ISPK_E_NULL, "speaker_grad: null pointer");
    ISPK_REQUIRE(B >= 0 && B <= 65535 && L >= 1 && L <= 512 && D >= 4 && speakers >= 1 && (id_stride == 0 || id_stride == 1),
                 ISPK_E_SHAPE, "speaker_grad: bad shape B=%d L=%d (<= 512) D=%d speakers=%d id_stride=%d", B, L, D, speakers,
                 id_stride);
    ISPK_REQUIRE(D % 4 == 0 && ld_table % 4 == 0 && ld_table >= D && ispk_aligned(d_table, 16) && ispk_aligned(d_x, 16) &&
                     ispk_aligned(workspace, 16),
                 ISPK_E_ALIGN, "speaker_grad: D / ld_table must be multiples of 4 and d_x / d_table / workspace 16-byte aligned");
    const int chunks = (L + kSgRows - 1) / kSgRows;
    ISPK_REQUIRE(workspace_floats >= (int64_t)B * chunks * D, ISPK_E_SHAPE, "speaker_grad: workspace needs %lld floats (B * ceil(L / %d) * D)",
                 (long long)B * chunks * D, kSgRows);
    hipStream_t s = reinterpret_cast<hipStream_t>(stream);
    if (B > 0)
        hipLaunchKernelGGL(speaker_grad_stage1_kernel, dim3((D / 4 + 63) / 64, chunks, B), dim3(256), 0, s, d_x, text_len, workspace,
                           L, D, chunks);
    hipLaunchKernelGGL(speaker_grad_stage2_kernel, dim3(speakers, (D / 4 + 63) / 64), dim3(256), 0, s, workspace, speaker, id_stride, text_len, d_table,
                       ld_table, speakers, B, L, D, chunks, accumulate);
    return ispk_launch_status();
}

extern "C" int32_t ispk_time_embedding_f32(const float* t, int32_t n, const float* inv_freq, const float* freq_scale,
                                           int32_t half_dim, const float* w0, const float* b0, const float* w1,
                                           const float* b1, int32_t emb_dim, float* out, ispk_stream_t stream) {
    ISPK_REQUIRE(t && inv_freq && freq_scale && w0 && b0 && w1 && b1 && out, ISPK_E_NULL, "time_embedding: null pointer");
    ISPK_REQUIRE(n >= 0 && half_dim >= 1 && half_dim <= 64 && emb_dim >= 1 && emb_dim <= 64, ISPK_E_SHAPE,
                 "time_embedding: bad shape n=%d half_dim=%d emb_dim=%d (both <= 64)", n, half_dim, emb_dim);
    if (n == 0) return 0;
    hipLaunchKernelGGL(time_embedding_kernel, dim3(n), dim3(64), 0, reinterpret_cast<hipStream_t>(stream), t, inv_freq,
                       freq_scale, half_dim, w0, b0, w1, b1, emb_dim, out);
    return ispk_launch_status();
}

static int32_t length_regulate_launch(const float* alignment, const float* dur_f32, const int64_t* dur_i64, const int64_t* enc_len,
                                      const float* x, int64_t ldx, float* out, int64_t* dec_len, uint8_t* dec_mask, int32_t B,
                                      int32_t M, int32_t L, int32_t D, int32_t max_len, int32_t dur_cols, ispk_stream_t stream,
                                      int split) {
    ISPK_REQUIRE(x && out && dec_len, ISPK_E_NULL, "length_regulate: null pointer");
    ISPK_REQUIRE((dur_f32 != nullptr) != (dur_i64 != nullptr), ISPK_E_NULL,
                 "length_regulate: exactly one of dur_f32 / dur_i64 must be given");
    ISPK_REQUIRE(alignment || dur_f32, ISPK_E_NULL, "length_regulate: the soft path (alignment NULL) needs fp32 durations");
    ISPK_REQUIRE(dur_cols == L || (dur_i64 && dur_cols >= 1), ISPK_E_SHAPE,
                 "length_regulate: dur_cols=%d (L, or any width >= 1 for int64 durations that are only summed)", dur_cols);
    ISPK_REQUIRE(B >= 0 && M >= 1 && L >= 1 && L <= 4096 && B <= 65535, ISPK_E_SHAPE,
                 "length_regulate: bad shape B=%d M=%d L=%d", B, M, L);
    ISPK_REQUIRE(D == 256 || D == 384, ISPK_E_UNSUPPORTED, "length_regulate: dim %d (built for 256 / 384)", D);
    ISPK_REQUIRE(ldx % 4 == 0 && ldx >= D && ispk_aligned(x, 16) && ispk_aligned(out, 16), ISPK_E_ALIGN,
                 "length_regulate: x / out must be 16-byte aligned, ldx a multiple of 4");
    if (B == 0) return 0;
    const size_t lds = 16 + (size_t)(kLrRows * kLrAld + kLrChunk * D + L + 1) * sizeof(float);
    const dim3 grid((M + kLrRows - 1) / kLrRows, B);
    hipStream_t s = reinterpret_cast<hipStream_t>(stream);
#define ISPK_LR(NT_, SP_)                                                                                              \
    do {                                                                                                               \
        ISPK_RESERVE_LDS((&length_regulate_kernel<NT_, SP_>), lds, "length_regulate");                                 \
        hipLaunchKernelGGL((length_regulate_kernel<NT_, SP_>), grid, dim3(256), lds, s, alignment, dur_f32, dur_i64, enc_len, x, \
                           ldx, out, dec_len, dec_mask, M, L, max_len, dur_cols);                                      \
    } while (0)
    if (D == 384) { if (split == 2) ISPK_LR(3, 2); else if (split) ISPK_LR(3, 1); else ISPK_LR(3, 0); }
    else { if (split == 2) ISPK_LR(2, 2); else if (split) ISPK_LR(2, 1); else ISPK_LR(2, 0); }
#undef ISPK_LR
    return ispk_launch_status();
}

extern "C" int32_t ispk_length_regulate_f32(const float* alignment, const float* dur_f32, const int64_t* dur_i64,
                                            const int64_t* enc_len, const float* x, int64_t ldx, float* out,
                                            int64_t* dec_len, uint8_t* dec_mask, int32_t B, int32_t M, int32_t L, int32_t D,
                                            int32_t max_len, int32_t dur_cols, ispk_stream_t stream) {
    return length_regulate_launch(alignment, dur_f32, dur_i64, enc_len, x, ldx, out, dec_len, dec_mask, B, M, L, D, max_len, dur_cols,
                                  stream, 0);
}

extern "C" int32_t ispk_length_regulate_split_bf16(const float* alignment, const float* dur_f32, const int64_t* dur_i64,
                                                   const int64_t* enc_len, const float* x, int64_t ldx, float* out,
                                                   int64_t* dec_len, uint8_t* dec_mask, int32_t B, int32_t M, int32_t L,
                                                   int32_t D, int32_t max_len, int32_t dur_cols, ispk_stream_t stream) {
    return length_regulate_launch(alignment, dur_f32, dur_i64, enc_len, x, ldx, out, dec_len, dec_mask, B, M, L, D, max_len, dur_cols,
                                  stream, 1);
}

extern "C" int32_t ispk_length_regulate_split_f16(const float* alignment, const float* dur_f32, const int64_t* dur_i64,
                                                  const int64_t* enc_len, const float* x, int64_t ldx, float* out,
                                                  int64_t* dec_len, uint8_t* dec_mask, int32_t B, int32_t M, int32_t L,
                                                  int32_t D, int32_t max_len, int32_t dur_cols, ispk_stream_t stream) {
    return length_regulate_launch(alignment, dur_f32, dur_i64, enc_len, x, ldx, out, dec_len, dec_mask, B, M, L, D, max_len, dur_cols,
                                  stream, 2);
}
```

isp_tts_amd/graph.py:

```python
from __future__ import annotations

import gc
from typing import Optional

import torch
from torch import Tensor

from . import staging


class GraphedCall:

    def __init__(self, fn, warmup: int = 2):
        self._fn = fn
        side = torch.cuda.Stream()
        side.wait_stream(torch.cuda.current_stream())
        with torch.cuda.stream(side):
            for _ in range(warmup):
                self.out = fn()
        torch.cuda.current_stream().wait_stream(side)
        torch.cuda.synchronize()
        self.graph = torch.cuda.CUDAGraph()
        gc.collect()
        gc_was_on = gc.isenabled()
        gc.disable()
        try:
            with torch.cuda.graph(self.graph):
                self.out = fn()
        finally:
            if gc_was_on:
                gc.enable()
        self._staged_at_capture = staging.replacements()

    def replay(self):
        if staging.replacements() != self._staged_at_capture:
            raise RuntimeError("a staged weight image was rebuilt after this graph was captured (parameters changed: "
                               "load() / an optimizer step); the graph points at freed memory - capture a new one")
        self.graph.replay()
        return self.out


class GraphedForward(GraphedCall):
    def __init__(self, model, text: Tensor, text_len: Tensor, mel: Tensor, mel_len: Tensor, pitch: Tensor,
                 energy: Tensor, flow_noise: Optional[Tensor] = None, flow_time: Optional[Tensor] = None,
                 warmup: int = 2, *, speaker: Optional[Tensor] = None):
        self.model = model
        self.static = {"text": text.clone(), "text_len": text_len.clone(), "mel": mel.clone(), "mel_len": mel_len.clone(),
                       "pitch": pitch.clone(), "energy": energy.clone()}
        b, l = text.shape
        dev = text.device
        self.static["flow_noise"] = (flow_noise.clone() if flow_noise is not None
                                     else torch.randn(b, l, 3, device=dev))
        self.static["flow_time"] = flow_time.clone() if flow_time is not None else torch.rand(b, device=dev)
        if speaker is not None:
            self.static["speaker"] = speaker.clone()
        super().__init__(self._run, warmup)

    def _run(self):
        s = self.static
        with torch.no_grad():
            return self.model(s["text"], s["text_len"], s["mel"], s["mel_len"], s["pitch"], s["energy"],
                              speaker=s.get("speaker"), flow_noise=s["flow_noise"], flow_time=s["flow_time"])

    def __call__(self, **inputs: Tensor):
        for k, v in inputs.items():
            self.static[k].copy_(v)
        return self.replay()


class SegmentedForward:

    def __init__(self, model, text: Tensor, text_len: Tensor, mel: Tensor, mel_len: Tensor, pitch: Tensor, energy: Tensor,
                 flow_noise: Optional[Tensor] = None, flow_time: Optional[Tensor] = None, warmup: int = 2, side_priority: int = 0):
        if not model.temporal_adaptor.soft_duration:
            raise NotImplementedError("SegmentedForward is built for soft durations: its back piece (embedding stack, length "
                                      "regulator, decoder) is launched without waiting for the side piece, and with hard "
                                      "durations both its targets and its regulator read the MAS durations that piece computes; "
                                      "use GraphedForward")
        if model.speaker_embedding is not None and model.speaker_in_forward:
            raise NotImplementedError("SegmentedForward does not add the speaker rows (its three pieces hand the encoder output "
                                      "on as one tensor); use GraphedForward(..., speaker=ids)")
        b, l = text.shape
        dev = text.device
        s = self.static = {"text": text.clone(), "text_len": text_len.clone(), "mel": mel.clone(), "mel_len": mel_len.clone(),
                           "pitch": pitch.clone(), "energy": energy.clone(),
                           "flow_noise": flow_noise.clone() if flow_noise is not None else torch.randn(b, l, 3, device=dev),
                           "flow_time": flow_time.clone() if flow_time is not None else torch.rand(b, device=dev)}
        self.model, self.side = model, torch.cuda.Stream(device=dev, priority=side_priority)
        frames = mel.shape[2]
        self.g_front = GraphedCall(lambda: model.forward_front(s["text"], s["text_len"], s["mel"], s["mel_len"], s["pitch"],
                                                               s["energy"]), warmup)
        st = self.g_front.out
        self.side.wait_stream(torch.cuda.current_stream())
        with torch.cuda.stream(self.side):
            self.g_side = GraphedCall(lambda: model.forward_side(st, s["text_len"], s["mel_len"], s["pitch"], s["energy"],
                                                                 s["flow_noise"], s["flow_time"]), warmup)
        torch.cuda.current_stream().wait_stream(self.side)
        self.g_back = GraphedCall(lambda: model.forward_back(st, s["text_len"], s["mel_len"], frames), warmup)
        self.out = model.assemble_output(st, self.g_side.out, self.g_back.out)
        self.front_done, self.side_done = torch.cuda.Event(), torch.cuda.Event()

    def replay(self):
        main = torch.cuda.current_stream()
        self.g_front.replay()
        self.front_done.record(main)
        self.side.wait_event(self.front_done)
        with torch.cuda.stream(self.side):
            self.g_side.replay()
            self.side_done.record(self.side)
        self.g_back.replay()
        main.wait_event(self.side_done)
        return self.out

    def __call__(self, **inputs: Tensor):
        for k, v in inputs.items():
            self.static[k].copy_(v)
        return self.replay()


class GraphedForwardLanes:

    def __init__(self, model, *inputs, lanes: int = 2, calibrate: bool = True, **kw):
        self.dev = inputs[0].device
        self.lanes = [(GraphedForward(model, *inputs, **kw), None) for _ in range(max(1, lanes))]
        self.count = 0
        self._new_streams()
        self.overlap = None
        if calibrate and len(self.lanes) > 1:
            for _ in range(6):
                one, alt = self._time(False), self._time(True)
                self.overlap = one / alt
                if alt < 0.93 * one:
                    break
                self._new_streams()

    def _new_streams(self) -> None:
        self.lanes = [(g, torch.cuda.Stream(device=self.dev)) for g, _ in self.lanes]
        for _, stream in self.lanes:
            with torch.cuda.stream(stream):
                torch.zeros(1, device=self.dev)
        torch.cuda.synchronize()

    def _time(self, alternate: bool, n: int = 6) -> float:
        import time
        torch.cuda.synchronize()
        t0 = time.perf_counter()
        for k in range(n):
            g, stream = self.lanes[k % len(self.lanes) if alternate else 0]
            with torch.cuda.stream(stream):
                g.replay()
        torch.cuda.synchronize()
        return (time.perf_counter() - t0) / n

    def __len__(self) -> int:
        return len(self.lanes)

    def next_lane(self):
        lane = self.lanes[self.count % len(self.lanes)]
        self.count += 1
        return lane

    def replay(self):
        g, stream = self.next_lane()
        stream.wait_stream(torch.cuda.current_stream())
        with torch.cuda.stream(stream):
            return g.replay()
```

isp_tts_amd/modules/transformer/transformer.py:

```python
from __future__ import annotations

from dataclasses import dataclass, field
from typing import NamedTuple, Optional, Union

import torch
import torch.nn as nn
from torch import Tensor

from ... import runtime
from ...staging import StagedWeights
from ..constructor import Constructor, ModuleConfig
from .attend import AttentionIntermediates
from .attention import Attention, AttentionConfig, AttentionSharedIntermediates
from .feedforward import FeedForward, FeedForwardConfig
from .normalization import AdaptiveLayerNorm, LayerNorm
from .plan import ATTN_OUT_FFN_FORMS, Consumer, Form, Hand, Handed, Next, Plan, Qkv, Seams, select_plan


class TransformerLayerIntermediates(NamedTuple):
    attention: Optional[AttentionIntermediates] = None


class TransformerLayerOutput(NamedTuple):
    out: Optional[Tensor]
# ... 25 lines not shown
        self.attention = Attention.init(attention if attention is not None else AttentionConfig(), dim=dim)
        self.feed_forward_norm = norm()
        self.feed_forward = FeedForward.init(feed_forward if feed_forward is not None else FeedForwardConfig(), dim=dim)

    def _plan(self, dim: int, rows: int, prev: Handed, consumer: Consumer, seams: Optional[Seams]) -> Plan:
        att, ff = self.attention, self.feed_forward
        plain = all(isinstance(n, nn.LayerNorm) and n.weight is not None and n.bias is not None
                    for n in (self.attention_norm, self.feed_forward_norm))
        nxt = consumer.attention
        return select_plan(cdt=att.compute_dtype, dim=dim, heads=att.heads, out_dim=att.out_dim, inner=ff.net[0].weight.shape[0],
                           rows=rows, plain_norms=plain, bias1=ff.net[0].bias is not None, bias2=ff.net[3].bias is not None,
                           gelu=ff.act_flag == runtime.EP_GELU, dropout=ff.training and ff.dropout_p > 0, prev=prev.kind,
                           consumer=consumer.kind, consumer_dtype=consumer.dtype, next_heads=nxt.heads if nxt is not None else 0,
                           next_dim=nxt.dim if nxt is not None else 0, only_normed=consumer.only_normed, seams=seams)

    def forward(self, x: Tensor, mask: Optional[Tensor] = None, context: Optional[Tensor] = None,
                context_mask: Optional[Tensor] = None, attention_mask: Optional[Tensor] = None,
                adaptive_condition: Optional[Tensor] = None, cache: Optional[TransformerLayerIntermediates] = None,
                shared_cache: Optional[AttentionSharedIntermediates] = None, *, key_len: Optional[Tensor] = None,
                ada: Optional[tuple] = None, prev: Handed = Handed(), consumer: Consumer = Consumer(),
                seams: Optional[Seams] = None):
        assert not self.adaptive_norm or adaptive_condition is not None or ada is not None, \
            "`adaptive_condition` should be provided for AdaptiveLayerNorm"
        if cache is not None:
            raise NotImplementedError("KV caches are not on the acoustic-model forward path")
        if context is not None or context_mask is not None or attention_mask is not None:
            raise NotImplementedError("cross-attention / explicit attention masks are not on the forward path")
        x = x.float().contiguous()
        if mask is not None and key_len is None:
            key_len = mask.sum(dim=1)
        att, ff, fn = self.attention, self.feed_forward, self.feed_forward_norm
        cdt = att.compute_dtype
        p = self._plan(x.shape[-1], x.numel() // x.shape[-1], prev, consumer, seams)

        def norm(n, t: Tensor, scale_shift: Optional[tuple], row_mask: Optional[Tensor] = None) -> Tensor:
            if cdt == torch.float16:
                return self._norm_split(n, t, adaptive_condition, scale_shift, row_mask)
            kw = {} if scale_shift is None else {"scale_shift": scale_shift}
            return n(t, adaptive_condition, row_mask=row_mask, out_dtype=cdt, **kw)

        qkv = None
        if p.qkv is Qkv.HANDED_QKV:
            qkv = prev.tensor
        elif p.qkv in (Qkv.LNIN_STATS, Qkv.LNIN_SELF):
            qkv = att.qkv_lnin(x, self.attention_norm, prev.tensor if p.qkv is Qkv.LNIN_STATS else None)
        h = x if qkv is not None else prev.tensor if p.qkv is Qkv.HANDED_ROWS else norm(self.attention_norm, x, ada and ada[0])
        x1, inter, shared = att(h, mask=mask, key_len=key_len, residual=x, qkv=qkv, defer_out=p.defer_out)

        second = None
        served = consumer if p.hands is not Hand.NONE else None
        if p.form in ATTN_OUT_FFN_FORMS:
            y, second = ff.attn_out_ffn(x, x1, att._chunked_wo(), fn, mask, p.form, served, p.store_out)
        elif p.form in (Form.FFN_PRENORM2, Form.FFN_PRENORM):
            y, second = ff.prenorm(x1, fn, mask, p.form is Form.FFN_PRENORM2, served.eps if served is not None else None)
        elif p.form is Form.SPLIT_PROJ:
            y, second = ff.prenorm_split(x, fn, mask, p.splits, served, p.hand_dtype, attn_proj=(x1, att._chunked_wo()))
        elif p.form is Form.SPLIT:
            y, second = ff.prenorm_split(x1, fn, mask, p.splits, served, p.hand_dtype)
        elif p.form is Form.LNIN_GEMM:
            y = ff.lnin_gemm(x1, fn, mask)
        else:
            y = ff(norm(fn, x1, ada and ada[1], mask), residual=x1, mask=mask, fused=p.form is Form.NORM_FFN_FUSED)
        return TransformerLayerOutput(out=y, intermediates=TransformerLayerIntermediates(attention=inter),
                                      shared_intermediates=shared, handed=Handed(p.hands, second))

    def _norm_split(self, norm, x: Tensor, condition: Optional[Tensor], scale_shift: Optional[tuple],
                    row_mask: Optional[Tensor]) -> Tensor:
        if isinstance(norm, AdaptiveLayerNorm):
            if scale_shift is None and condition is not None:
                cond = condition.reshape(-1, condition.shape[-1]).float().contiguous()
                scale_shift = (runtime.linear_small(cond, norm.weight.weight, norm.weight.bias),
                               runtime.linear_small(cond, norm.bias.weight, norm.bias.bias) if norm.bias is not None else None)
            if scale_shift is None:
                return runtime.layernorm_split(x, None, None, row_mask=row_mask, eps=norm.eps)
            rows_per_batch = x.numel() // (x.shape[0] * x.shape[-1])
            return runtime.layernorm_split(x, None, None, scale_shift[0], scale_shift[1], rows_per_batch, row_mask, norm.eps)
        return runtime.layernorm_split(x, norm.weight, norm.bias, row_mask=row_mask, eps=norm.eps)


class TransformerOutput(NamedTuple):
    out: Tensor
    intermediates: Optional[list] = None


@dataclass
class TransformerConfig(ModuleConfig):
    dim: int = 384
    depth: int = 6
    transformer_layer: Union[TransformerLayerConfig, dict] = field(default_factory=TransformerLayerConfig)
    emb_dim: Optional[int] = None
    use_abs_pos_emb: bool = True
    adaptive_norm: bool = False
    condition_dim: Optional[int] = None


class Transformer(nn.Module, Constructor):
    seams: Optional[Seams] = None

    def __init__(self, dim: int = 384, depth: int = 6, transformer_layer=None, emb_dim: Optional[int] = None,
                 use_abs_pos_emb: bool = True, adaptive_norm: bool = False, condition_dim: Optional[int] = None):
        super().__init__()
        self.dim = dim
        self.emb_dim = emb_dim = emb_dim or dim
        self.adaptive_norm = adaptive_norm
        layer_cfg = transformer_layer if transformer_layer is not None else TransformerLayerConfig()
        self.layers = nn.ModuleList([
            TransformerLayer.init(layer_cfg, dim=dim, adaptive_norm=adaptive_norm, condition_dim=condition_dim)
            for _ in range(depth)])
        if use_abs_pos_emb and self.layers[0].attention.rel_pos is None:
            raise NotImplementedError("absolute sinusoidal position embeddings (no ALiBi) are unused by the recipes")
        self.pos_emb = None
        self.project_emb = nn.Linear(emb_dim, dim) if emb_dim != dim else nn.Identity()
        self.norm = nn.LayerNorm(dim)
        self._ada_cache = StagedWeights()

    def _ada_all(self, condition: Tensor):
        norms = [n for layer in self.layers for n in (layer.attention_norm, layer.feed_forward_norm)]
        ps = [p for n in norms for p in (n.weight.weight, n.weight.bias, n.bias.weight, n.bias.bias)]

        def build():
            with torch.no_grad():
                return (torch.cat([torch.cat([n.weight.weight, n.bias.weight]) for n in norms]).contiguous(),
                        torch.cat([torch.cat([n.weight.bias, n.bias.bias]) for n in norms]).contiguous())
        w_all, b_all = self._ada_cache.get("ada", ps, build)
        cond = condition.reshape(-1, condition.shape[-1]).float().contiguous()
        proj = runtime.linear_small(cond, w_all, b_all)
        d = self.dim
        parts = [(proj[:, (2 * i) * d:(2 * i + 1) * d], proj[:, (2 * i + 1) * d:(2 * i + 2) * d])
                 for i in range(len(norms))]
        return [(parts[2 * li], parts[2 * li + 1]) for li in range(len(self.layers))]

    def set_compute_dtype(self, dtype: torch.dtype):
        assert dtype in (torch.float32, torch.bfloat16, torch.float16)
        for layer in self.layers:
            layer.attention.compute_dtype = dtype
            layer.feed_forward.compute_dtype = dtype
        return self

    def _consumer(self, li: int, mask: Optional[Tensor], out_dtype: torch.dtype, final_norm: bool) -> Consumer:
        if li + 1 < len(self.layers):
            nxt = self.layers[li + 1]
            c = Consumer(Next.LAYER, nxt.attention_norm.weight, nxt.attention_norm.bias, nxt.attention_norm.eps,
                         attention=nxt.attention)
        else:
            c = Consumer(Next.FINAL, self.norm.weight, self.norm.bias, self.norm.eps, mask is not None, out_dtype,
                         only_normed=True)
        served = not self.adaptive_norm and (li + 1 < len(self.layers) or final_norm)
        return c if served and c.weight is not None and c.bias is not None else Consumer()

    def forward(self, x: Tensor, mask: Optional[Tensor] = None, context: Optional[Tensor] = None,
                context_mask: Optional[Tensor] = None, attention_mask: Optional[Tensor] = None,
                adaptive_condition: Optional[Tensor] = None, return_intermediates: bool = False, *,
                key_len: Optional[Tensor] = None, projected: Optional[Tensor] = None,
                out_dtype: torch.dtype = torch.float32, final_norm: bool = True):
        if projected is not None:
            out = projected
        elif isinstance(self.project_emb, nn.Identity):
            out = x.float()
        else:
            out = runtime.linear(x.float(), self.project_emb.weight, self.project_emb.bias)
        if mask is not None and key_len is None:
            key_len = mask.sum(dim=1)
        intermediates = []
        ada = self._ada_all(adaptive_condition) if (self.adaptive_norm and adaptive_condition is not None) else None
        handed = Handed()
        for li, layer in enumerate(self.layers):
            res = layer(out, mask=mask, context=context, context_mask=context_mask, attention_mask=attention_mask,
                        adaptive_condition=adaptive_condition, key_len=key_len, ada=None if ada is None else ada[li],
                        prev=handed, consumer=self._consumer(li, mask, out_dtype, final_norm), seams=self.seams)
            out, handed = res.out, res.handed
            if return_intermediates:
                intermediates.append(res.intermediates)
        if not final_norm:
            return TransformerOutput(out=out, intermediates=intermediates)
        if handed.kind is Hand.ROWS:
            normed = handed.tensor
        elif out_dtype == torch.float16:
            normed = runtime.layernorm_split(out, self.norm.weight, self.norm.bias, row_mask=mask, eps=self.norm.eps)
        else:
            normed = runtime.layernorm(out, self.norm.weight, self.norm.bias, row_mask=mask, eps=self.norm.eps,
                                       out_dtype=out_dtype)
        return TransformerOutput(out=normed, intermediates=intermediates)
```

isp_tts_amd/runtime.py:

```python
from __future__ import annotations

import ctypes
import os
from typing import Optional

import torch
from torch import Tensor

_HERE = os.path.dirname(os.path.abspath(__file__))
LIB_PATH = os.path.join(_HERE, "libispk.so")

EP_GELU, EP_SILU, EP_MASK_ACC, EP_MASK_OUT, EP_BIAS_ROW, EP_MASK_COL, EP_OUT_BF16, EP_RESID_BF16, EP_ROWS_T, EP_OUT_SPLIT = (
    1, 2, 4, 8, 16, 32, 64, 128, 256, 512)

_P, _I32, _I64, _U32, _F32 = ctypes.c_void_p, ctypes.c_int32, ctypes.c_int64, ctypes.c_uint32, ctypes.c_float
_U64, _F64 = ctypes.c_uint64, ctypes.c_double

SIGNATURES = {
    "ispk_abi_version": [],
    "ispk_last_error_string": [],
    "ispk_device_info": [ctypes.c_char_p, _I32],
    "ispk_mas_f32": [_P, _P, _P, _P, _P, _P, _I32, _I32, _I32, _I64, _I64, _P],
    "ispk_layernorm_f32": [_P, _I64, _P, _P, _P, _P, _I64, _I32, _P, _P, _I64, _I32, _I32, _F32, _P],
    "ispk_layernorm_f32_bf16": [_P, _I64, _P, _P, _P, _P, _I64, _I32, _P, _P, _I64, _I32, _I32, _F32, _P],
    "ispk_gemm_f32_tile": [_I32, _I32, _I32],
    "ispk_gemm_f32": [_P, _I64, _P, _I64, _P, _I64, _P, _P, _I64, _P, _I32, _I32, _I32, _U32, _I32, _I64, _P],
    "ispk_gemm_f32_batched": [_P, _I64, _I64, _P, _I64, _I64, _P, _I64, _I64, _I32, _I32, _I32, _I32, _P],
    "ispk_gemm_bf16_gelu_train": [_P, _I64, _P, _I64, _P, _I64, _P, _I64, _I32, _I32, _I32, _F32, _U64, _P],
    "ispk_gemm_bf16_gelu_bwd": [_P, _I64, _P, _I64, _P, _I64, _P, _I64, _P, _I32, _I32, _I32, _F32, _U64, _P],
    "ispk_segments_f32": [_P, _I32, _P],
    "ispk_stage_weights": [_P, _I32, _P],
    "ispk_fill_zero": [_P, _I64, _P],
    "ispk_scale_f32": [_P, _I64, _P, _F32, _P],
    "ispk_sum_scalars_f32": [_P, _P, _I32, _P, _P],
    "ispk_exp_pad_f32": [_P, _P, _I32, _I32, _P],
    "ispk_sqrt_scale_f32": [_P, _P, _I32, _F32, _P],
    "ispk_copy2d_f32": [_P, _I64, _P, _I64, _I32, _I32, _P],
    "ispk_permute021_f32": [_P, _P, _I32, _I32, _I32, _P],
    "ispk_conv_weight_flip_f32": [_P, _P, _I32, _I32, _I32, _P],
    "ispk_gemm_bf16_last_variant": [],
    "ispk_gemm_bf16": [_P, _I64, _P, _I64, _P, _I64, _P, _P, _I64, _P, _I32, _I32, _I32, _U32, _I32, _I64, _P],
    "ispk_gemm_bf16_splitk_plan": [_I32, _I32, _I32, _U32],
    "ispk_gemm_bf16_splitk": [_P, _I64, _P, _I64, _P, _I64, _P, _P, _I64, _P, _I32, _I32, _I32, _U32, _P, _I32, _P],
    "ispk_ffn_bf16": [_P, _I64, _P, _I64, _P, _P, _I64, _P, _P, _I64, _P, _P, _I64, _I32, _I32, _I32, _U32, _P],
    "ispk_ffn_pack_w2_bf16": [_P, _I64, _I32, _I32, _P, _P],
    "ispk_ffn_bf16_prenorm": [_P, _I64, _P, _P, _F32, _P, _I64, _P, _P, _P, _P, _I64, _I32, _I32, _I32, _U32, _P, _F32, _P],
    "ispk_ffn_chunk_w2_bf16": [_P, _I64, _I32, _I32, _P, _P],
    "ispk_ffn_bf16_prenorm2_split": [_P, _I64, _P, _P, _F32, _P, _P, _P, _I64, _I32, _I32, _I32, _I32, _P],
    "ispk_ffn_combine_ln_f32": [_P, _I64, _P, _I64, _I32, _P, _P, _I64, _P, _P, _F32, _I32, _P, _I64, _I32, _I32, _I32, _P],
    "ispk_ffn_bf16_prenorm2": [_P, _I64, _P, _P, _F32, _P, _P, _P, _P, _I64, _I32, _I32, _I32, _U32, _P, _F32, _P],
    "ispk_attn_out_ffn_bf16": [_P, _I64, _P, _I64, _P, _P, _P, _F32, _P, _P, _P, _P, _I64, _I32, _I32, _I32, _U32, _P, _F32, _P],
    "ispk_attn_out_ffn_qkv_bf16": [_P, _I64, _P, _I64, _P, _P, _P, _F32, _P, _P, _P, _P, _I64, _I32, _I32, _I32, _U32, _P, _P, _F32,
                                   _P, _P, _I64, _P],
    "ispk_chunk_k16_bf16": [_P, _I64, _I32, _I32, _P, _P],
    "ispk_attn_out_ffn_norm_bf16": [_P, _I64, _P, _I64, _P, _P, _P, _F32, _P, _P, _P, _P, _I64, _I32, _I32, _I32, _U32, _P, _P, _F32,
                                    _I32, _P, _I64, _I32, _P],
    "ispk_attn_out_ffn_split_bf16": [_P, _I64, _P, _I64, _P, _P, _P, _F32, _P, _P, _P, _U32, _P, _I64, _I32, _I32, _I32, _I32, _P],
    "ispk_gemm_bf16_lnin": [_P, _I64, _P, _P, _P, _F32, _P, _I64, _P, _I64, _P, _P, _I64, _P, _I32, _I32, _I32, _U32, _P],
    "ispk_linear_small_f32": [_P, _I64, _P, _I64, _P, _P, _I64, _P, _I64, _I32, _I32, _I32, _U32, _P],
    "ispk_alibi_mqa_attn_f32": [_P, _I64, _P, _P, _I64, _P, _P, _P, _I64, _I32, _I32, _I32, _P],
    "ispk_alibi_mqa_attn_bf16": [_P, _I64, _P, _P, _I64, _P, _P, _P, _I64, _I32, _I32, _I32, _P],
    "ispk_alibi_mqa_attn_bf16_tiles": [_P, _I64, _P, _P, _I64, _P, _P, _P, _I64, _I32, _I32, _I32, _I32, _P],
    "ispk_cast_f32_bf16": [_P, _I64, _P, _I64, _I32, _I32, _P],
    "ispk_split_f16": [_P, _I64, _P, _P, _I64, _I32, _I32, _P],
    "ispk_gemm_split_f16_tile": [_I32, _I32, _I32],
    "ispk_gemm_split_f16": [_P, _I64, _I64, _P, _I64, _I64, _P, _I64, _I64, _P, _P, _I64, _P, _I32, _I32, _I32, _U32, _I32,
                            _I64, _P],
    "ispk_layernorm_f32_split": [_P, _I64, _P, _P, _P, _P, _I64, _I32, _P, _P, _I64, _I64, _I32, _I32, _F32, _P],
    "ispk_alibi_mqa_attn_split_f16": [_P, _I64, _P, _P, _I64, _P, _P, _P, _I64, _I64, _I32, _I32, _I32, _P],
    "ispk_flow_mix_f32": [_P, _P, _P, _F32, _P, _P, _I32, _I32, _I32, _P],
    "ispk_flow_finish_f32": [_P, _P, _P, _P, _P, _P, _P, _P, _I32, _I32, _I32, _P],
    "ispk_flow_head_f32": [_P, _I64, _P, _P, _F32, _P, _P, _P, _P, _P, _P, _P, _P, _P, _P, _I32, _I32, _I32, _I32, _P],
    "ispk_flow_euler_f32": [_P, _P, _F32, _P, _P, _I32, _I32, _I32, _P],
    "ispk_infer_features_f32": [_P, _P, _P, _P, _P, _F32, _F32, _F32, _F32, _F32, _P, _P, _I32, _I32, _P],
    "ispk_infer_features_round_f32": [_P, _P, _P, _P, _P, _F32, _F32, _F32, _F32, _F32, _P, _P, _I32, _I32, _P],
    "ispk_hard_regulate_f32": [_P, _P, _P, _I64, _P, _P, _P, _I32, _I32, _I32, _I32, _I32, _P],
    "ispk_hard_regulate_bwd_f32": [_P, _P, _P, _P, _I32, _I32, _I32, _I32, _I32, _P],
    "ispk_hard_average_f32": [_P, _P, _P, _P, _P, _I32, _I32, _I32, _P],
    "ispk_embed_tokens_f32": [_P, _P, _I64, _I32, _P, _P, _P, _I32, _I32, _I32, _P],
    "ispk_add_speaker_f32": [_P, _P, _I64, _I32, _P, _I32, _I32, _I32, _I32, _P],
    "ispk_add_speaker_out_f32": [_P, _P, _P, _I64, _I32, _P, _I32, _I32, _I32, _I32, _P],
    "ispk_speaker_grad_f32": [_P, _P, _I32, _P, _P, _I64, _P, _I64, _I32, _I32, _I32, _I32, _I32, _P],
    "ispk_time_embedding_f32": [_P, _I32, _P, _P, _I32, _P, _P, _P, _P, _I32, _P, _P],
    "ispk_length_regulate_f32": [_P, _P, _P, _P, _P, _I64, _P, _P, _P, _I32, _I32, _I32, _I32, _I32, _I32, _P],
    "ispk_length_regulate_split_bf16": [_P, _P, _P, _P, _P, _I64, _P, _P, _P, _I32, _I32, _I32, _I32, _I32, _I32, _P],
    "ispk_length_regulate_split_f16": [_P, _P, _P, _P, _P, _I64, _P, _P, _P, _I32, _I32, _I32, _I32, _I32, _I32, _P],
    "ispk_pad_rows_f32": [_P, _I64, _I64, _I64, _P, _P, _I32, _I32, _I32, _I32, _P],
    "ispk_masked_instnorm_f32": [_P, _P, _P, _P, _P, _I32, _I32, _I32, _I32, _F32, _P],
    "ispk_aligner_scores_f32": [_P, _I64, _P, _I64, _P, _P, _P, _P, _I32, _I32, _I32, _I32, _P],
    "ispk_aligner_scores_fast_f32": [_P, _I64, _P, _I64, _P, _P, _P, _P, _I32, _I32, _I32, _I32, _P],
    "ispk_soft_average_f32": [_P, _P, _P, _P, _P, _P, _I32, _I32, _I32, _P],
    "ispk_transpose_f32": [_P, _I64, _P, _I64, _I32, _I32, _P],
    "ispk_gemm_tn_f32": [_P, _I64, _P, _I64, _P, _I64, _I32, _I32, _I32, _P, _I32, _P, _I64, _P],
    "ispk_gemm_tn_bf16": [_P, _I64, _P, _I64, _P, _I64, _I32, _I32, _I32, _P, _I32, _P, _I64, _P],
    "ispk_gemm_tn_b16": [_P, _I64, _P, _I64, _P, _I64, _I32, _I32, _I32, _P, _I32, _P, _I64, _P],
    "ispk_gelu_f32_bf16": [_P, _P, _I64, _F32, _U64, _P],
    "ispk_gelu_bf16": [_P, _P, _I64, _F32, _U64, _P],
    "ispk_gelu_bwd_b16": [_P, _P, _P, _I64, _F32, _U64, _P],
    "ispk_gelu_bwd_bf16": [_P, _P, _P, _I64, _F32, _U64, _P],
    "ispk_gemm_tn_last_plan": [_P, _P],
    "ispk_gemm_tn_batched_f32": [_P, _I64, _I64, _P, _I64, _I64, _P, _I64, _I64, _I32, _I32, _I32, _I32, _P, _I32, _P, _I64, _P],
    "ispk_layernorm_bwd_f32": [_P, _I64, _P, _I64, _P, _P, _P, _I64, _I32, _P, _P, _P, _I64, _I64, _I32, _F32, _P],
    "ispk_layernorm_bwd_dual_f32": [_P, _I64, _P, _I64, _P, _P, _P, _I64, _I32, _P, _P, _P, _I64, _I64, _I32, _F32, _P, _I64, _P],
    "ispk_gelu_f32": [_P, _P, _I64, _F32, _U64, _P],
    "ispk_gelu_bwd_f32": [_P, _P, _P, _I64, _F32, _U64, _P],
    "ispk_dropout_mask_u8": [_P, _I64, _F32, _U64, _P],
    "ispk_alibi_mqa_attn_train_f32": [_P, _I64, _P, _P, _P, _I64, _P, _I32, _I32, _I32, _F32, _U64, _P],
    "ispk_alibi_mqa_attn_bwd_f32": [_P, _I64, _P, _P, _I64, _P, _P, _P, _P, _P, _I64, _I32, _I32, _I32, _P, _F32, _U64, _P],
    "ispk_alibi_mqa_attn_train_bf16": [_P, _I64, _P, _P, _P, _I64, _P, _I32, _I32, _I32, _F32, _U64, _P],
    "ispk_alibi_mqa_attn_bwd_bf16": [_P, _I64, _P, _P, _I64, _P, _P, _P, _P, _P, _P, _I64, _I32, _I32, _I32, _F32, _U64, _P],
    "ispk_mel_loss_f32": [_P, _P, _P, _P, _P, _P, _F32, _I32, _I32, _I32, _P],
    "ispk_acoustic_metrics_f32": [_P, _I64, _I64, _I64, _P, _I64, _I64, _I64, _P, _P, _P, _I64, _I64, _P, _P, _I64, _P, _I32,
                                  _I32, _I32, _I32, _I32, _P],
    "ispk_dtw_f32": [_P, _I64, _I64, _P, _P, _P, _P, _P, _P, _I64, _I32, _I32, _I32, _P],
    "ispk_mcd_dtw_f32": [_P, _I64, _I64, _I64, _P, _I64, _I64, _I64, _P, _P, _P, _P, _I64, _P, _I64, _P, _I64, _P, _P, _P, _I32,
                         _I32, _I32, _I32, _I32, _P],
    "ispk_audio_features_f32": [_P, _I64, _P, _P, _I64, _P, _I32, _P, _P, _P, _P, _I32, _I32, _I32, _I32, _I32, _F32, _F32, _F32,
                                _F32, _P],
    "ispk_resample_f32": [_P, _I64, _I64, _P, _P, _I64, _P, _P, _I64, _P, _I32, _I32, _I32, _I32, _I32, _I32, _I32, _I32, _P],
    "ispk_feature_stats_f64": [_P, _I64, _P, _I64, _P, _P, _P, _I32, _I32, _I32, _P],
    "ispk_audio_measure_f64": [_P, _I64, _P, _P, _I64, _P, _P, _P, _P, _P, _I64, _I32, _I32, _I32, _I32, _F64, _I32, _I32, _F64,
                               _F64, _P],
    "ispk_audio_apply_f32": [_P, _I64, _P, _P, _P, _I64, _P, _I32, _I32, _I32, _P],
    "ispk_pcm16": [_P, _I64, _P, _P, _I64, _I32, _I32, _I32, _U64, _P],
    "ispk_aligner_scores_bwd_f32": [_P, _P, _P, _P, _P, _P, _P, _I64, _P, _I64, _I32, _I32, _I32, _F32, _P],
    "ispk_masked_instnorm_bwd_f32": [_P, _P, _P, _P, _P, _P, _P, _P, _I64, _I32, _I32, _I32, _F32, _P],
    "ispk_soft_average_bwd_f32": [_P, _P, _P, _P, _P, _P, _I64, _P, _I32, _I32, _I32, _I32, _P],
    "ispk_flow_loss_bwd_f32": [_P, _P, _P, _F32, _P, _I32, _I32, _I32, _P],
    "ispk_adaln_bwd_f32": [_P, _I64, _P, _I64, _P, _I64, _P, _P, _I64, _I32, _P, _P, _I64, _I32, _I32, _I32, _F32, _P],
    "ispk_time_embedding_bwd_f32": [_P, _I32, _P, _P, _I32, _P, _P, _P, _I32, _P, _P, _P, _P, _P, _P],
    "ispk_attn_ctc_loss_f32": [_P, _P, _P, _F32, _P, _I64, _P, _P, _F32, _I32, _I32, _I32, _P],
    "ispk_attn_bin_loss_f32": [_P, _P, _F32, _P, _P, _P, _F32, _I32, _I32, _I32, _P],
    "ispk_mel_grad_rows_f32": [_P, _P, _P, _I32, _I32, _I32, _P],
    "ispk_colsum_f32": [_P, _I64, _I64, _I32, _P, _P, _I64, _P, _P],
    "ispk_smallk_wgrad_f32": [_P, _I64, _P, _I64, _I64, _I32, _I32, _P, _I64, _P, _P],
    "ispk_embedding_bwd_f32": [_P, _P, _I64, _I32, _I32, _I32, _P, _I64, _P],
    "ispk_grad_sqnorm_f32": [_P, _I64, _P, _P, _P],
    "ispk_adamw_f32": [_P, _P, _P, _P, _I64, _I64, _F32, _F32, _F32, _F32, _F32, _I32, _P, _F32, _F32, _P],
    "ispk_adamw_f32_dev": [_P, _P, _P, _P, _I64, _I64, _P, _P, _P],
    "ispk_adam_args_f32": [_F32, _F32, _F32, _F32, _F32, _I32, _F32, _F32, _P],
    "ispk_set_dropout_seed_source": [_P],
    "ispk_vocoder_unfold": [_P, _I32, _I64, _I64, _I64, _P, _P, _I32, _I64, _P, _I32, _I32, _I32, _I32, _P],
    "ispk_dwconv7_ln_f32": [_P, _I64, _P, _P, _P, _P, _F32, _P, _P, _I32, _I64, _I32, _I32, _I32, _P],
    "ispk_istft_head_f32": [_P, _I64, _P, _P, _I64, _P, _I64, _P, _I32, _I32, _I32, _P],
    "ispk_hifigan_tile_rows": [],
    "ispk_hifigan_conv_f32": [_P, _I64, _P, _P, _P, _I64, _P, _I64, _P, _I32, _I32, _I32, _I32, _I32, _I32, _I32, _F32, _F32,
                              _I32, _P],
    "ispk_hifigan_conv_bf16": [_P, _I64, _P, _P, _P, _I64, _P, _I64, _P, _I32, _I32, _I32, _I32, _I32, _I32, _I32, _F32, _F32,
                               _I32, _P],
    "ispk_hifigan_upsample_f32": [_P, _I64, _P, _P, _P, _I64, _P, _I32, _I32, _I32, _I32, _I32, _I32, _I32, _F32, _P],
    "ispk_hifigan_upsample_bf16": [_P, _I64, _P, _P, _P, _I64, _P, _I32, _I32, _I32, _I32, _I32, _I32, _I32, _F32, _P],
    "ispk_hifigan_post_f32": [_P, _I64, _P, _P, _P, _I32, _P, _I64, _P, _I32, _I32, _I32, _I32, _F32, _P],
}

_lib = None


class IspkError(RuntimeError):
    pass


def lib() -> ctypes.CDLL:
    global _lib
    if _lib is None:
        if not os.path.exists(LIB_PATH):
            raise IspkError(f"{LIB_PATH} is missing: the HIP extension was not built "
                            f"(run `python -m isp_tts_amd.build` or `__graft_entry__.build()`); there is no CPU fallback")
        handle = ctypes.CDLL(LIB_PATH)
        for name, argtypes in SIGNATURES.items():
            fn = getattr(handle, name)
            fn.argtypes = argtypes
            fn.restype = ctypes.c_char_p if name == "ispk_last_error_string" else ctypes.c_int32
        if handle.ispk_abi_version() != 2:
            raise IspkError(f"libispk.so ABI version {handle.ispk_abi_version()} != 2 (rebuild: python -m isp_tts_amd.build)")
        _lib = handle
    return _lib


class LaunchProfiler:

    def __init__(self):
        self.records = []

    def summary(self) -> dict:
        out: dict = {}
        for label, flops, nbytes, e0, e1 in self.records:
            d = out.setdefault(label, {"launches": 0, "total_ms": 0.0, "flops": 0.0, "bytes": 0.0})
            d["launches"] += 1
            d["total_ms"] += e0.elapsed_time(e1)
            d["flops"] += flops
            d["bytes"] += nbytes
        for d in out.values():
            d["avg_us"] = 1e3 * d["total_ms"] / d["launches"]
        return out


_profiler: Optional[LaunchProfiler] = None


def set_profiler(p: Optional[LaunchProfiler]) -> None:
    global _profiler
    _profiler = p


_PANEL_EPS = (64, 65, 4 | (1 << 17), 256 | 8 | (1 << 16))


def _launch(label: str, flops: float, nbytes: float, fn, *args) -> None:
    if _profiler is None:
        _check(fn(*args), label)
        return
    e0, e1 = torch.cuda.Event(enable_timing=True), torch.cuda.Event(enable_timing=True)
    e0.record()
    rc = fn(*args)
    e1.record()
    _check(rc, label)
    if label == "gemm_bf16_kernel":
        v = lib().ispk_gemm_bf16_last_variant()
        if v // 1000 == 1:
            ep = (args[13] & 0xffff) | ((1 << 16) if args[6] else 0) | ((1 << 17) if args[7] else 0)
            label = f"gemm_bf16_panel_kernel<{v % 1000},{ep if ep in _PANEL_EPS else -1}>"
        else:
            label = {2: f"gemm_bf16_wide_kernel<{(v % 1000) // 10},{v % 10}>",
                     3: f"gemm_bf16_kernel<{(v % 1000) // 10},{v % 10}>"}.get(v // 1000, label)
    elif label.startswith("gemm_tn_b16_kernel") and lib().ispk_gemm_tn_last_plan(None, None) == 4:
        label = "gemm_tn_dma_kernel" + label[len("gemm_tn_b16_kernel"):]
    _profiler.records.append((label, flops, nbytes, e0, e1))


def _check(rc: int, what: str) -> None:
    if rc != 0:
        msg = lib().ispk_last_error_string()
        raise IspkError(f"{what} failed (rc={rc}): {msg.decode() if msg else '?'}")


def _dev(*tensors: Optional[Tensor]) -> None:
    for t in tensors:
        if t is not None and not t.is_cuda:
# ... 566 lines not shown


def conv5_padded(xpad: Tensor, w2d: Tensor, flags: int = 0) -> Tensor:
    _dev(xpad, w2d)
    B, TP, C = xpad.shape
    O, K = w2d.shape
    taps = K // C
    assert taps * C == K and taps in (1, 5) and xpad.is_contiguous() and w2d.is_contiguous()
    assert xpad.dtype == w2d.dtype
    bf16 = xpad.dtype == torch.bfloat16
    out = torch.empty((B, TP, O), dtype=torch.float32, device=xpad.device)
    a_ptr = xpad.data_ptr() + (0 if taps == 5 else 2 * C * xpad.element_size())
    M = B * TP - 4
    fn = lib().ispk_gemm_bf16 if bf16 else lib().ispk_gemm_f32
    _launch(_gemm_label(bf16, M, O, K), 2.0 * M * O * K, float(xpad.element_size()) * (M * C + O * K) + 4.0 * M * O, fn,
            a_ptr, C, w2d.data_ptr(), K, out.data_ptr(), O, None, None, 0, None, M, O, K, flags, 0, 0, _stream())
    return out


def masked_instnorm(y: Tensor, weight: Tensor, bias: Tensor, lengths: Tensor, eps: float = 1e-5,
                    out_dtype: torch.dtype = torch.float32) -> Tensor:
    _dev(y, weight, bias, lengths)
    B, TP, C = y.shape
    split = out_dtype == torch.float16
    out = torch.empty((2, *y.shape) if split else y.shape, dtype=out_dtype, device=y.device)
    lengths = lengths.to(torch.int64).contiguous()
    _launch("masked_instnorm_kernel", 0.0, 16.0 * B * TP * C, lib().ispk_masked_instnorm_f32, y.data_ptr(),
            weight.data_ptr(), bias.data_ptr(), lengths.data_ptr(), out.data_ptr(), 2 if split else int(out_dtype == torch.bfloat16), B,
            TP - 4, C, eps, _stream())
    return out


def aligner_scores(q_enc: Tensor, k_enc: Tensor, text_len: Tensor, mel_len: Tensor, M: int, L: int, fast: bool = False):
    _dev(q_enc, k_enc, text_len, mel_len)
    B, D = q_enc.shape[0], q_enc.shape[2]
    logits = torch.empty((B, M, L), dtype=torch.float32, device=q_enc.device)
    soft = torch.empty((B, M, L), dtype=torch.float32, device=q_enc.device)
    text_len = text_len.to(torch.int64).contiguous()
    mel_len = mel_len.to(torch.int64).contiguous()
    _launch("aligner_scores_kernel<bf16x3>" if fast else "aligner_scores_kernel", 2.0 * B * M * L * D, 4.0 * B * (M * D + L * D + 2 * M * L),
            lib().ispk_aligner_scores_fast_f32 if fast else lib().ispk_aligner_scores_f32, q_enc.data_ptr(), q_enc.stride(0), k_enc.data_ptr(), k_enc.stride(0),
            text_len.data_ptr(), mel_len.data_ptr(), logits.data_ptr(), soft.data_ptr(), B, M, L, D, _stream())
    return soft, logits


def soft_average(attn_soft: Tensor, pitch: Tensor, energy: Tensor, duration: Optional[Tensor], text_len: Tensor) -> Tensor:
    _dev(attn_soft, pitch, energy, duration, text_len)
    B, M, L = attn_soft.shape
    feats = torch.empty((B, L, 3), dtype=torch.float32, device=attn_soft.device)
    dur = None if duration is None else duration.to(torch.int64).contiguous()
    _launch("soft_average_kernel", 0.0, 4.0 * B * M * L, lib().ispk_soft_average_f32, attn_soft.contiguous().data_ptr(),
            pitch.contiguous().data_ptr(), energy.contiguous().data_ptr(), _ptr(dur),
            text_len.to(torch.int64).contiguous().data_ptr(), feats.data_ptr(), B, M, L, _stream())
    return feats


def flow_mix(x0: Tensor, x1: Tensor, t: Tensor, sigma: float):
    _dev(x0, x1, t)
    B, L, C = x1.shape
    x0c, x1c, tc = x0.float().contiguous(), x1.float().contiguous(), t.float().contiguous()
    xt, flow = torch.empty_like(x1c), torch.empty_like(x1c)
    _launch("flow_mix_kernel", 0.0, 16.0 * B * L * C, lib().ispk_flow_mix_f32, x0c.data_ptr(), x1c.data_ptr(), tc.data_ptr(),
            float(sigma), xt.data_ptr(), flow.data_ptr(), B, L, C, _stream())
    return xt, flow


def flow_finish(pred_raw: Tensor, flow: Tensor, x0: Tensor, mask: Tensor):
    _dev(pred_raw, flow, x0, mask)
    B, L, C = pred_raw.shape
    assert mask.dtype == torch.bool and mask.shape == (B, L)
    pr, fl, x0c, mk = pred_raw.float().contiguous(), flow.contiguous(), x0.float().contiguous(), mask.contiguous()
    pred = torch.empty_like(pr)
    dur = torch.empty((B, L), dtype=torch.float32, device=pr.device)
    ratio = torch.empty((B,), dtype=torch.float32, device=pr.device)
    loss = torch.empty((), dtype=torch.float32, device=pr.device)
    _launch("flow_finish_kernel", 0.0, 20.0 * B * L * C, lib().ispk_flow_finish_f32, pr.data_ptr(), fl.data_ptr(),
            x0c.data_ptr(), mk.data_ptr(), pred.data_ptr(), dur.data_ptr(), ratio.data_ptr(), loss.data_ptr(), B, L, C,
            _stream())
    return pred, dur, ratio, loss


def flow_head(y: Tensor, norm_weight: Tensor, norm_bias: Tensor, norm_eps: float, weight: Tensor, bias: Tensor, flow: Tensor,
              x0: Tensor, mask: Tensor):
    _dev(y, norm_weight, norm_bias, weight, bias, flow, x0, mask)
    B, L, D = y.shape
    C = weight.shape[0]
    assert y.dtype == torch.float32 and y.stride(2) == 1 and y.stride(0) == L * y.stride(1) and weight.shape == (C, D) and weight.is_contiguous()
    assert mask.dtype == torch.bool and mask.shape == (B, L)
    fl, x0c, mk = flow.contiguous(), x0.float().contiguous(), mask.contiguous()
    pred = torch.empty((B, L, C), dtype=torch.float32, device=y.device)
    dur = torch.empty((B, L), dtype=torch.float32, device=y.device)
    ratio = torch.empty((B,), dtype=torch.float32, device=y.device)
    loss = torch.empty((), dtype=torch.float32, device=y.device)
    ws = torch.empty((2 * B * ((L + 15) // 16),), dtype=torch.float32, device=y.device)
    _launch("flow_head_kernels", 0.0, 4.0 * B * L * D, lib().ispk_flow_head_f32, y.data_ptr(), y.stride(1), norm_weight.data_ptr(),
            norm_bias.data_ptr(), float(norm_eps), weight.data_ptr(), bias.data_ptr(), fl.data_ptr(), x0c.data_ptr(), mk.data_ptr(),
            pred.data_ptr(), dur.data_ptr(), ratio.data_ptr(), loss.data_ptr(), ws.data_ptr(), B, L, D, C, _stream())
    return pred, dur, ratio, loss


def flow_euler(x_t: Tensor, velocity: Tensor, dt: float, mask: Optional[Tensor] = None) -> Tensor:
    _dev(x_t, velocity, mask)
    B, L, C = x_t.shape
    xc, vc = x_t.float().contiguous(), velocity.float().contiguous()
    out = torch.empty_like(xc)
    if mask is not None:
        mask = mask.contiguous()
        assert mask.dtype == torch.bool and mask.shape == (B, L)
    _launch("flow_euler_kernel", 0.0, 12.0 * B * L * C, lib().ispk_flow_euler_f32, xc.data_ptr(), vc.data_ptr(), float(dt),
            _ptr(mask), out.data_ptr(), B, L, C, _stream())
    return out


def infer_features(pred: Tensor, duration_target: Optional[Tensor], pitch_target: Optional[Tensor],
                   energy_target: Optional[Tensor], duration_factor: float = 1.0, pitch_factor: float = 1.0,
                   pitch_delta: float = 0.0, energy_factor: float = 1.0, energy_delta: float = 0.0, round_duration: bool = False):
    _dev(pred, duration_target, pitch_target, energy_target)
    B, L, C = pred.shape
    assert C == 3 and pred.dtype == torch.float32
    pc = pred.contiguous()
    dur_f = dur_i = None
    if duration_target is not None:
        assert duration_target.shape == (B, L)
        if duration_target.dtype == torch.int64:
            dur_i = duration_target.contiguous()
        else:
            dur_f = duration_target.float().contiguous()
    pt = None if pitch_target is None else pitch_target.float().reshape(B, L).contiguous()
    et = None if energy_target is None else energy_target.float().reshape(B, L).contiguous()
    duration = torch.empty((B, L), dtype=torch.float32, device=pred.device)
    feats = torch.empty((B, L, 2), dtype=torch.float32, device=pred.device)
    _launch("infer_features_kernel<round>" if round_duration else "infer_features_kernel", 0.0, 24.0 * B * L,
            lib().ispk_infer_features_round_f32 if round_duration else lib().ispk_infer_features_f32, pc.data_ptr(), _ptr(dur_f), _ptr(dur_i),
            _ptr(pt), _ptr(et), float(duration_factor), float(pitch_factor), float(pitch_delta), float(energy_factor),
            float(energy_delta), duration.data_ptr(), feats.data_ptr(), B, L, _stream())
    return duration, feats


def embed_tokens(text: Tensor, table: Tensor, text_len: Optional[Tensor] = None, want_mask: bool = True):
    _dev(text, table, text_len)
    assert text.dtype == torch.int64 and text.ndim == 2 and table.dtype == torch.float32 and table.stride(1) == 1
    B, L = text.shape
    V, D = table.shape
    text = text.contiguous()
    emb = torch.empty((B, L, D), dtype=torch.float32, device=text.device)
    mask = torch.empty((B, L), dtype=torch.bool, device=text.device) if want_mask else None
    if text_len is not None:
        text_len = text_len.to(torch.int64).contiguous()
    _launch("embed_tokens_kernel", 0.0, 8.0 * B * L * D, lib().ispk_embed_tokens_f32, text.data_ptr(), table.data_ptr(),
            table.stride(0), V, _ptr(text_len), emb.data_ptr(), _ptr(mask), B, L, D, _stream())
    return emb, mask


def _speaker_ids(speaker: Tensor, B: int):
    assert speaker.dtype == torch.int64
    if speaker.numel() == 1:
        return speaker.contiguous(), 0
    if speaker.ndim == 2 and tuple(speaker.shape) == (B, 1):
        return speaker.contiguous(), 1
    raise ValueError(f"speaker of shape {tuple(speaker.shape)} does not broadcast against enc_out [B={B}, L, D] "
                     "(the reference takes [B, 1] ids or a single id)")


def add_speaker_(x: Tensor, table: Tensor, speaker: Tensor) -> Tensor:
    _dev(x, table, speaker)
    assert x.dtype == torch.float32 and x.ndim == 3 and x.is_contiguous() and table.dtype == torch.float32 and table.stride(1) == 1
    B, L, D = x.shape
    assert table.shape[1] == D
    speaker, stride = _speaker_ids(speaker, B)
    _launch("add_speaker_kernel", 0.0, 8.0 * B * L * D, lib().ispk_add_speaker_f32, x.data_ptr(), table.data_ptr(), table.stride(0),
            table.shape[0], speaker.data_ptr(), stride, B, L, D, _stream())
    return x


def add_speaker(x: Tensor, table: Tensor, speaker: Tensor) -> Tensor:
    _dev(x, table, speaker)
    assert x.dtype == torch.float32 and x.ndim == 3 and x.is_contiguous() and table.dtype == torch.float32 and table.stride(1) == 1
    B, L, D = x.shape
    assert table.shape[1] == D
    speaker, stride = _speaker_ids(speaker, B)
    out = torch.empty_like(x)
    _launch("add_speaker_out_kernel", 0.0, 8.0 * B * L * D, lib().ispk_add_speaker_out_f32, x.data_ptr(), out.data_ptr(),
            table.data_ptr(), table.stride(0), table.shape[0], speaker.data_ptr(), stride, B, L, D, _stream())
    return out


def speaker_grad(d_x: Tensor, speaker: Tensor, speakers: int, text_len: Optional[Tensor] = None, out: Optional[Tensor] = None,
                 accumulate: bool = False) -> Tensor:
    _dev(d_x, speaker, text_len, out)
    assert d_x.dtype == torch.float32 and d_x.ndim == 3
    d_x = d_x.contiguous()
    B, L, D = d_x.shape
    speaker, stride = _speaker_ids(speaker, B)
    if text_len is not None:
        text_len = text_len.to(torch.int64).contiguous()
        assert text_len.numel() == B
    if out is None:
        assert not accumulate
        out = torch.empty((speakers, D), dtype=torch.float32, device=d_x.device)
    assert out.dtype == torch.float32 and tuple(out.shape) == (speakers, D) and out.stride(1) == 1
    ws = workspace(d_x.device, B * -(-L // 16) * D)
    _launch("speaker_grad_kernels", 1.0 * B * L * D, 4.0 * B * L * D + 4.0 * speakers * D, lib().ispk_speaker_grad_f32, d_x.data_ptr(),
            speaker.data_ptr(), stride, _ptr(text_len), ws.data_ptr(), ws.numel(), out.data_ptr(), out.stride(0), speakers, B, L, D,
            1 if accumulate else 0, _stream())
    return out


def time_embedding(t: Tensor, inv_freq: Tensor, freq_scale: Tensor, w0: Tensor, b0: Tensor, w1: Tensor, b1: Tensor) -> Tensor:
    _dev(t, inv_freq, freq_scale, w0, b0, w1, b1)
    tf = t.to(torch.float32).contiguous()
    E, H = w1.shape[0], inv_freq.numel()
    assert w0.shape == (E, 1 + 2 * H) and w1.shape == (E, E) and w0.is_contiguous() and w1.is_contiguous()
    out = torch.empty((*t.shape, E), dtype=torch.float32, device=t.device)
    _launch("time_embedding_kernel", 0.0, 0.0, lib().ispk_time_embedding_f32, tf.data_ptr(), tf.numel(), inv_freq.data_ptr(),
            freq_scale.data_ptr(), H, w0.data_ptr(), b0.data_ptr(), w1.data_ptr(), b1.data_ptr(), E, out.data_ptr(),
            _stream())
    return out


def length_regulate(x: Tensor, durations: Tensor, alignment: Optional[Tensor], frames: int, max_len: int = -1,
                    enc_len: Optional[Tensor] = None, want_mask: bool = True, split_bf16=False):
    _dev(x, durations, alignment, enc_len)
    assert x.dtype == torch.float32 and x.ndim == 3
    if x.stride(2) != 1 or x.stride(0) != x.shape[1] * x.stride(1):
        x = x.contiguous()
    B, L, D = x.shape
    if alignment is not None:
        assert alignment.dtype == torch.float32 and alignment.shape == (B, frames, L)
        alignment = alignment.contiguous()
    dur_f = dur_i = None
    dur_cols = L
    if durations.dtype == torch.int64:
        assert alignment is not None, "the soft path is generated from fp32 durations"
        dur_i = durations.reshape(B, -1).contiguous()
        dur_cols = dur_i.shape[1]
    else:
        dur_f = durations.to(torch.float32).contiguous()
        assert dur_f.shape == (B, L)
    if enc_len is not None:
        enc_len = enc_len.to(torch.int64).contiguous()
    out = torch.empty((B, frames, D), dtype=torch.float32, device=x.device)
    dec_len = torch.empty((B,), dtype=torch.int64, device=x.device)
    mask = torch.empty((B, frames), dtype=torch.bool, device=x.device) if want_mask else None
    nb = 4.0 * B * (frames * D + L * D + (frames * L if alignment is not None else 0))
    fn = (lib().ispk_length_regulate_split_f16 if split_bf16 == "f16" else
          lib().ispk_length_regulate_split_bf16 if split_bf16 else lib().ispk_length_regulate_f32)
    _launch("length_regulate_kernel<split_f16>" if split_bf16 == "f16" else "length_regulate_kernel<bf16x3>" if split_bf16
            else "length_regulate_kernel", 2.0 * B * frames * L * D, nb, fn, _ptr(alignment),
            _ptr(dur_f), _ptr(dur_i), _ptr(enc_len), x.data_ptr(), x.stride(1), out.data_ptr(), dec_len.data_ptr(),
            _ptr(mask), B, frames, L, D, max_len, dur_cols, _stream())
    return out, dec_len, mask


def _hard_durations(durations: Tensor, B: int, L: int):
    assert durations.shape == (B, L), f"durations {tuple(durations.shape)}: one per token, [{B}, {L}]"
    if durations.dtype == torch.int64:
        return None, durations.contiguous()
    return durations.to(torch.float32).contiguous(), None


def hard_regulate(x: Tensor, durations: Tensor, frames: int, max_len: int = -1, want_mask: bool = True):
    _dev(x, durations)
    assert x.dtype == torch.float32 and x.ndim == 3
    if x.stride(2) != 1 or x.stride(0) != x.shape[1] * x.stride(1):
        x = x.contiguous()
    B, L, D = x.shape
    dur_f, dur_i = _hard_durations(durations, B, L)
    out = torch.empty((B, frames, D), dtype=torch.float32, device=x.device)
    dec_len = torch.empty((B,), dtype=torch.int64, device=x.device)
    mask = torch.empty((B, frames), dtype=torch.bool, device=x.device) if want_mask else None
    _launch("hard_regulate_kernel", 0.0, 4.0 * B * D * (frames + L), lib().ispk_hard_regulate_f32, _ptr(dur_f), _ptr(dur_i),
            x.data_ptr(), x.stride(1), out.data_ptr(), dec_len.data_ptr(), _ptr(mask), B, frames, L, D, max_len, _stream())
    return out, dec_len, mask


def hard_regulate_bwd(d_out: Tensor, durations: Tensor, max_len: int = -1) -> Tensor:
    _dev(d_out, durations)
    assert d_out.dtype == torch.float32 and d_out.ndim == 3
    d_out = d_out.contiguous()
    B, rows, D = d_out.shape
    L = durations.shape[1]
    dur_f, dur_i = _hard_durations(durations, B, L)
    d_x = torch.empty((B, L, D), dtype=torch.float32, device=d_out.device)
    _launch("hard_regulate_bwd_kernel", 1.0 * B * rows * D, 4.0 * B * D * (rows + L), lib().ispk_hard_regulate_bwd_f32, _ptr(dur_f),
            _ptr(dur_i), d_out.data_ptr(), d_x.data_ptr(), B, rows, L, D, max_len, _stream())
    return d_x


def hard_average(pitch: Tensor, energy: Tensor, duration: Tensor, text_len: Tensor) -> Tensor:
    _dev(pitch, energy, duration, text_len)
    B, M = pitch.shape
    L = duration.shape[1]
    assert duration.dtype == torch.int64 and duration.shape == (B, L) and energy.shape == (B, M)
    feats = torch.empty((B, L, 3), dtype=torch.float32, device=pitch.device)
    pc, ec, dc, tc = pitch.float().contiguous(), energy.float().contiguous(), duration.contiguous(), text_len.to(torch.int64).contiguous()
    _launch("hard_average_kernel", 0.0, 8.0 * B * M + 20.0 * B * L, lib().ispk_hard_average_f32, pc.data_ptr(), ec.data_ptr(),
            dc.data_ptr(), tc.data_ptr(), feats.data_ptr(), B, M, L, _stream())
    return feats


def cast_bf16(x: Tensor) -> Tensor:
    _dev(x)
    x2 = _rows2d(x)
    y = torch.empty(x.shape, dtype=torch.bfloat16, device=x.device)
    _launch("cast_bf16_kernel", 0.0, 6.0 * x2.numel(), lib().ispk_cast_f32_bf16, x2.data_ptr(), x2.stride(0),
            y.data_ptr(), x2.shape[1], x2.shape[0], x2.shape[1], _stream())
    return y


class _Segment(ctypes.Structure):
    _fields_ = [("src", ctypes.c_void_p), ("dst", ctypes.c_void_p), ("n", ctypes.c_int64), ("mode", ctypes.c_int32)]


SEG_COPY, SEG_ADD, SEG_BF16 = 0, 1, 2


class _Stage(ctypes.Structure):
    _fields_ = [("src", ctypes.c_void_p), ("dst", ctypes.c_void_p), ("rows", ctypes.c_int32), ("cols", ctypes.c_int32),
                ("ld_dst", ctypes.c_int64), ("flags", ctypes.c_int32)]


stage_calls = 0


def stage_weights(items) -> None:
    global stage_calls
    if not items:
        return
    stage_calls += 1
    arr = (_Stage * len(items))()
    nbytes = 0.0
    for k, (src, dst, tr, ex) in enumerate(items):
        _dev(src, dst)
        src = src.detach()
        assert src.dtype == torch.float32 and src.ndim == 2 and src.is_contiguous() and dst.ndim == 2 and dst.stride(1) == 1
        assert tuple(dst.shape) == ((src.shape[1], src.shape[0]) if tr else tuple(src.shape)) and dst.dtype in (torch.float32, torch.bfloat16)
        arr[k].src, arr[k].dst, arr[k].rows, arr[k].cols = src.data_ptr(), dst.data_ptr(), src.shape[0], src.shape[1]
        arr[k].ld_dst = dst.stride(0)
        arr[k].flags = (1 if tr else 0) | (2 if dst.dtype == torch.bfloat16 else 0) | (4 if ex else 0)
        nbytes += src.numel() * (4.0 + dst.element_size())
    _launch("stage_kernel", 0.0, nbytes, lib().ispk_stage_weights, ctypes.cast(arr, ctypes.c_void_p), len(items), _stream())


def segments(items) -> None:
    if not items:
        return
    arr = (_Segment * len(items))()
    nbytes = 0.0
    for k, (src, dst, mode) in enumerate(items):
        _dev(src, dst)
        assert src.dtype == torch.float32 and src.is_contiguous() and dst.is_contiguous() and src.numel() == dst.numel()
        assert dst.dtype == (torch.bfloat16 if mode == SEG_BF16 else torch.float32)
        arr[k].src, arr[k].dst, arr[k].n, arr[k].mode = src.data_ptr(), dst.data_ptr(), src.numel(), mode
        nbytes += src.numel() * (4.0 + dst.element_size() * (2 if mode == SEG_ADD else 1))
    _launch("segments_kernel", 0.0, nbytes, lib().ispk_segments_f32, ctypes.cast(arr, ctypes.c_void_p), len(items), _stream())


def cat0(tensors, dtype: torch.dtype = torch.float32) -> Tensor:
    srcs = [t.detach() for t in tensors]
    assert dtype in (torch.float32, torch.bfloat16) and all(t.dtype == torch.float32 and t.is_contiguous() for t in srcs)
    rows = sum(t.shape[0] for t in srcs)
    out = torch.empty((rows, *srcs[0].shape[1:]), dtype=dtype, device=srcs[0].device)
    items, r = [], 0
    for t in srcs:
        items.append((t, out[r:r + t.shape[0]], SEG_BF16 if dtype == torch.bfloat16 else SEG_COPY))
        r += t.shape[0]
    segments(items)
    return out


def deliver_grads(pairs) -> list:
    out, items, seen = [], [], set()
    for p, g in pairs:
        if g is not None and not p.requires_grad:
            out.append(None)
            continue
        buf = p.grad if g is not None else None
        if buf is not None and getattr(buf, "_ispk_grad_arena", False) and g.is_cuda:
            g = g.detach()
            g = g if g.dtype == torch.float32 and g.is_contiguous() else g.float().contiguous()
            if buf.data_ptr() in seen:
                segments(items)
                items, seen = [], set()
            seen.add(buf.data_ptr())
            items.append((g, buf, SEG_ADD if getattr(buf, "_ispk_dirty", False) else SEG_COPY))
            buf._ispk_dirty = True
            out.append(None)
        else:
            out.append(g)
    segments(items)
    return out


def zero_(t: Tensor) -> Tensor:
    _dev(t)
    assert t.is_contiguous()
    _launch("fill_zero_kernel", 0.0, float(t.numel() * t.element_size()), lib().ispk_fill_zero, t.data_ptr(),
# ... 1027 lines not shown
```

Baseline: 16.13 million mel-frames/s.

## Fuse first-layer LayerNorm+QKV into token embedding and length regulator

```diff
diff --git a/include/ispk.h b/include/ispk.h
--- a/include/ispk.h
+++ b/include/ispk.h
@@ -176,6 +176,9 @@
 int32_t ispk_embed_tokens_f32(const int64_t* text, const float* table, int64_t ld_table, int32_t vocab,
                               const int64_t* text_len, float* emb, uint8_t* mask, int32_t B, int32_t L, int32_t D,
                               ispk_stream_t stream);
+int32_t ispk_embed_tokens_qkv(const int64_t* text, const float* table, int64_t ld_table, int32_t vocab, const int64_t* text_len,
+                              float* emb, uint8_t* mask, const uint16_t* qkv_table, int64_t ld_qkv_table, uint16_t* qkv,
+                              int32_t B, int32_t L, int32_t D, int32_t N, ispk_stream_t stream);
 int32_t ispk_add_speaker_f32(float* x, const float* table, int64_t ld_table, int32_t speakers, const int64_t* speaker,
                              int32_t id_stride, int32_t B, int32_t L, int32_t D, ispk_stream_t stream);
 int32_t ispk_add_speaker_out_f32(const float* x, float* out, const float* table, int64_t ld_table, int32_t speakers,
@@ -192,6 +195,11 @@
 int32_t ispk_length_regulate_split_bf16(const float* alignment, const float* dur_f32, const int64_t* dur_i64, const int64_t* enc_len,
                                  const float* x, int64_t ldx, float* out, int64_t* dec_len, uint8_t* dec_mask, int32_t B,
                                  int32_t M, int32_t L, int32_t D, int32_t max_len, int32_t dur_cols, ispk_stream_t stream);
+int32_t ispk_length_regulate_qkv_bf16(const float* alignment, const float* dur_f32, const int64_t* dur_i64, const int64_t* enc_len,
+                                      const float* x, int64_t ldx, float* out, int64_t* dec_len, uint8_t* dec_mask,
+                                      const float* norm_gamma, const float* norm_beta, float norm_eps, const uint16_t* Wqkv_chunks,
+                                      uint16_t* qkv, int64_t ld_qkv, int32_t B, int32_t M, int32_t L, int32_t D, int32_t max_len,
+                                      int32_t dur_cols, ispk_stream_t stream);
 int32_t ispk_length_regulate_split_f16(const float* alignment, const float* dur_f32, const int64_t* dur_i64, const int64_t* enc_len,
                                 const float* x, int64_t ldx, float* out, int64_t* dec_len, uint8_t* dec_mask, int32_t B,
                                 int32_t M, int32_t L, int32_t D, int32_t max_len, int32_t dur_cols, ispk_stream_t stream);
diff --git a/isp_tts_amd/acoustic/model.py b/isp_tts_amd/acoustic/model.py
--- a/isp_tts_amd/acoustic/model.py
+++ b/isp_tts_amd/acoustic/model.py
@@ -12,6 +12,7 @@
 from ..staging import StagedWeights
 from ..modules.constructor import Constructor
 from ..modules.transformer import Transformer
+from ..modules.transformer.plan import Hand, Handed
 from ..utils import get_mask_from_lengths
 from .alignment import Aligner, AlignerOutput
 from .temporal_adaptor import FlowTemporalAdaptor, TemporalAdaptorOutput
@@ -45,6 +46,7 @@
         self.temporal_adaptor = FlowTemporalAdaptor.init(temporal_adaptor, encoder_dim=enc_dim)
         self.decoder = Transformer.init(decoder, emb_dim=enc_dim)
         self.to_mel = nn.Linear(self.decoder.dim, mel_dim)
+        self.token_qkv_table = True
         self.overlap_streams = True
         self._side_streams: dict = {}
         self.register_buffer("pitch_mean", torch.tensor(float(pitch_mean or 0.)))
@@ -73,6 +75,36 @@
         if dec_out.dtype == torch.bfloat16:
             w = self._cache.get(torch.bfloat16, (w,), lambda: w.detach().to(torch.bfloat16).contiguous())
         return runtime.to_mel(dec_out, w, self.to_mel.bias, dec_mask)
+
+    def _embed(self, text: Tensor, text_len: Optional[Tensor], want_mask: bool = True):
+        table, enc = self.text_embedding.weight, self.encoder
+        first = enc.layers[0]
+        norm, att = first.attention_norm, first.attention
+        if not (self.token_qkv_table and text.is_cuda and att.compute_dtype == torch.bfloat16 and not first.adaptive_norm
+                and norm.weight is not None and norm.bias is not None and isinstance(enc.project_emb, nn.Identity)
+                and (att.heads * 64 + 128) % 8 == 0):
+            return (*runtime.embed_tokens(text, table, text_len, want_mask=want_mask), Handed())
+
+        def build():
+            with torch.no_grad():
+                rows = runtime.layernorm(table.detach().float().contiguous(), norm.weight, norm.bias, eps=norm.eps,
+                                         out_dtype=torch.bfloat16)
+                return runtime.gemm(rows, att._staged(torch.bfloat16)[0])
+        qkv_table = self._cache.get("token_qkv", (table, norm.weight, norm.bias, att.to_q.weight, att.to_kv.weight), build)
+        emb, mask, qkv = runtime.embed_tokens_qkv(text, table, qkv_table, text_len, want_mask=want_mask)
+        return emb, mask, Handed(Hand.QKV, qkv)
+
+    def _decoder_first(self):
+        dec = self.decoder
+        first = dec.layers[0]
+        norm, att = first.attention_norm, first.attention
+        ok = (att.compute_dtype == torch.bfloat16 and not first.adaptive_norm and norm.weight is not None and norm.bias is not None
+              and isinstance(dec.project_emb, nn.Identity) and dec.dim == 384 and att.heads * 64 + 128 == 512)
+        return first if ok else None
+
+    def _decoder_handed(self) -> Handed:
+        qkv = self.temporal_adaptor.length_regulator.qkv
+        return Handed(Hand.QKV, qkv) if qkv is not None else Handed()
 
     def forward(self, text: Tensor, text_len: Tensor, mel: Tensor, mel_len: Tensor, pitch: Optional[Tensor] = None,
                 energy: Optional[Tensor] = None, speaker: Optional[Tensor] = None, sigma: float = 0., steps: int = 1, *,
@@ -105,8 +137,8 @@
             side.wait_stream(main)
             with torch.cuda.stream(side):
                 q_proj = self.aligner.attention.project_queries(mel, mel_len)
-        token_emb, enc_mask = runtime.embed_tokens(text, self.text_embedding.weight, text_len)
-        enc_out = self.encoder(token_emb, mask=enc_mask, key_len=text_len).out
+        token_emb, enc_mask, handed = self._embed(text, text_len)
+        enc_out = self.encoder(token_emb, mask=enc_mask, key_len=text_len, handed=handed).out
         if q_proj is not None:
             main.wait_stream(side)
             q_proj.record_stream(main)
@@ -120,10 +152,12 @@
             enc_out=enc_out, enc_mask=enc_mask, max_dec_len=mel.size(2),
             duration_target=aligner_output.attn_hard_duration, alignment=aligner_output.attn_soft,
             pitch_target_dense=pitch, energy_target_dense=energy, noise=flow_noise, time_steps=flow_time,
-            enc_len=text_len, predictor_stream=branch, duration_sum=mel_len if branch is not None and not hard else None)
+            enc_len=text_len, predictor_stream=branch, duration_sum=mel_len if branch is not None and not hard else None,
+            qkv_for=self._decoder_first())
         dec_len = adaptor_output.dec_lengths
         dec_mask = adaptor_output.dec_mask
-        dec_out = self.decoder(adaptor_output.enc_out, mask=dec_mask, key_len=dec_len, out_dtype=self.compute_dtype).out
+        dec_out = self.decoder(adaptor_output.enc_out, mask=dec_mask, key_len=dec_len, out_dtype=self.compute_dtype,
+                               handed=self._decoder_handed()).out
         mel_out = self._to_mel(dec_out, dec_mask)
         if q_proj is not None:
             main.wait_stream(side)
@@ -140,8 +174,8 @@
         side.wait_stream(main)
         with torch.cuda.stream(side):
             q_proj = self.aligner.attention.project_queries(mel, mel_len)
-        token_emb, enc_mask = runtime.embed_tokens(text, self.text_embedding.weight, text_len)
-        enc_out = self.encoder(token_emb, mask=enc_mask, key_len=text_len).out
+        token_emb, enc_mask, handed = self._embed(text, text_len)
+        enc_out = self.encoder(token_emb, mask=enc_mask, key_len=text_len, handed=handed).out
         main.wait_stream(side)
         q_proj.record_stream(main)
         attn_soft, attn_logits = self.aligner.attention(mel, enc_out.transpose(1, 2).detach(), mel_len, text_len,
@@ -165,9 +199,11 @@
         ad = self.temporal_adaptor
         feats = st["feats"]
         x = ad.embedding(feats[..., 1:3], mask=st["enc_mask"][..., None], key_len=text_len, residual=st["enc_out"])
-        dec_in, dec_len = ad.length_regulator(x, mel_len.view(-1, 1), max_len=max_dec_len, alignment=st["attn_soft"])
+        dec_in, dec_len = ad.length_regulator(x, mel_len.view(-1, 1), max_len=max_dec_len, alignment=st["attn_soft"],
+                                              qkv_for=self._decoder_first())
         dec_mask = ad.length_regulator.dec_mask
-        dec_out = self.decoder(dec_in, mask=dec_mask, key_len=dec_len, out_dtype=self.compute_dtype).out
+        dec_out = self.decoder(dec_in, mask=dec_mask, key_len=dec_len, out_dtype=self.compute_dtype,
+                               handed=self._decoder_handed()).out
         return {"mel": self._to_mel(dec_out, dec_mask), "dec_in": dec_in, "dec_len": dec_len, "dec_mask": dec_mask}
 
     @staticmethod
@@ -189,9 +225,8 @@
               speaker: Optional[Tensor] = None, *, flow_noise: Optional[Tensor] = None,
               max_dec_len: Optional[int] = None):
         batch_infer = input_sequence.shape[0] > 1
-        token_emb, enc_mask = runtime.embed_tokens(input_sequence, self.text_embedding.weight,
-                                                   text_lengths if batch_infer else None, want_mask=batch_infer)
-        enc_out = self.encoder(token_emb, mask=enc_mask, key_len=text_lengths if batch_infer else None).out
+        token_emb, enc_mask, handed = self._embed(input_sequence, text_lengths if batch_infer else None, want_mask=batch_infer)
+        enc_out = self.encoder(token_emb, mask=enc_mask, key_len=text_lengths if batch_infer else None, handed=handed).out
         if self.speaker_embedding is not None and speaker is not None:
             enc_out = runtime.add_speaker_(enc_out, self.speaker_embedding.weight, speaker)
         if pitch_normalize:
@@ -202,10 +237,10 @@
             enc_out=enc_out, enc_mask=enc_mask, duration_target=duration_target, pitch_target=pitch_target,
             energy_target=energy_target, duration_factor=duration_factor, pitch_factor=pitch_factor,
             pitch_delta=pitch_delta, steps=steps, noise=flow_noise, max_dec_len=max_dec_len,
-            enc_len=text_lengths if batch_infer else None)
+            enc_len=text_lengths if batch_infer else None, qkv_for=self._decoder_first())
         dec_mask = adaptor_output.dec_mask if batch_infer else None
         dec_out = self.decoder(adaptor_output.enc_out, mask=dec_mask, key_len=adaptor_output.dec_lengths if batch_infer else None,
-                               out_dtype=self.compute_dtype).out
+                               out_dtype=self.compute_dtype, handed=self._decoder_handed()).out
         return self._to_mel(dec_out, dec_mask), adaptor_output
 
     @classmethod
diff --git a/isp_tts_amd/acoustic/temporal_adaptor.py b/isp_tts_amd/acoustic/temporal_adaptor.py
--- a/isp_tts_amd/acoustic/temporal_adaptor.py
+++ b/isp_tts_amd/acoustic/temporal_adaptor.py
@@ -164,9 +164,12 @@
 
 class LengthRegulator(nn.Module):
     split_bf16 = False
+    hand_qkv = True
+    qkv: Optional[Tensor] = None
 
     def forward(self, x: Tensor, durations: Tensor, max_len: Optional[int] = None, alignment: Optional[Tensor] = None, *,
-                enc_len: Optional[Tensor] = None, frames: Optional[int] = None, hard: bool = False):
+                enc_len: Optional[Tensor] = None, frames: Optional[int] = None, hard: bool = False, qkv_for=None):
+        self.qkv = None
         if alignment is None and (hard or frames is None or durations.dtype == torch.int64):
             if frames is None:
                 frames = int((durations.float() + 0.5).long().sum(dim=1).max().item())
@@ -182,6 +185,12 @@
         if max_len is not None and alignment is not None:
             rows = min(rows, max_len)
             alignment = alignment[:, :rows]
+        if self.hand_qkv and qkv_for is not None and self.split_bf16 is True and x.is_cuda and x.shape[-1] == 384:
+            norm, att = qkv_for.attention_norm, qkv_for.attention
+            out, dec_lens, self.dec_mask, self.qkv = runtime.length_regulate(
+                x.float(), durations, alignment, rows, max_len=-1 if max_len is None else max_len, enc_len=enc_len,
+                split_bf16=True, next_qkv=(norm.weight, norm.bias, norm.eps, att._chunked_wqkv()))
+            return out, dec_lens
         out, dec_lens, self.dec_mask = runtime.length_regulate(x.float(), durations, alignment, rows,
                                                                max_len=-1 if max_len is None else max_len, enc_len=enc_len,
                                                                split_bf16=self.split_bf16)
@@ -240,7 +249,7 @@
                 alignment: Optional[Tensor] = None, pitch_target_dense: Optional[Tensor] = None,
                 energy_target_dense: Optional[Tensor] = None, *, noise: Optional[Tensor] = None,
                 time_steps: Optional[Tensor] = None, enc_len: Optional[Tensor] = None,
-                predictor_stream=None, duration_sum: Optional[Tensor] = None) -> TemporalAdaptorOutput:
+                predictor_stream=None, duration_sum: Optional[Tensor] = None, qkv_for=None) -> TemporalAdaptorOutput:
         assert duration_target is not None and (alignment is not None or not self.soft_duration)
         assert pitch_target_dense is not None and energy_target_dense is not None
         hard = not self.soft_duration
@@ -271,7 +280,7 @@
         def decoder_input(enc_out_):
             enc_out_ = self.embedding(features, mask=m3, key_len=enc_len, residual=enc_out_)
             return self.length_regulator(enc_out_, len_src, max_len=max_dec_len, alignment=alignment,
-                                         frames=max_dec_len if hard else None)
+                                         frames=max_dec_len if hard else None, qkv_for=qkv_for)
 
         if not (side is not None and self.predictor_first):
             enc_out, dec_lens = decoder_input(enc_out)
@@ -304,7 +313,7 @@
               duration_factor: float = 1.0, pitch_target: Optional[Tensor] = None, pitch_factor: float = 1.0,
               pitch_delta: float = 0., energy_target: Optional[Tensor] = None, energy_factor: float = 1.0,
               energy_delta: float = 0., steps: int = 4, *, noise: Optional[Tensor] = None,
-              max_dec_len: Optional[int] = None, enc_len: Optional[Tensor] = None) -> TemporalAdaptorOutput:
+              max_dec_len: Optional[int] = None, enc_len: Optional[Tensor] = None, qkv_for=None) -> TemporalAdaptorOutput:
         m3 = enc_mask[..., None] if enc_mask is not None else None
         pred = self.predictor.infer(enc_out, mask=m3, steps=steps, noise=noise, key_len=enc_len)
         duration_pred, feats = runtime.infer_features(pred, duration_target, pitch_target, energy_target, duration_factor,
@@ -323,7 +332,7 @@
         if max_dec_len is None:
             max_dec_len = int((duration_pred.sum(dim=1) + 0.5).long().max().item())
         enc_out, dec_lens = self.length_regulator(enc_out, duration_pred, alignment=None, enc_len=enc_lens,
-                                                  frames=max_dec_len)
+                                                  frames=max_dec_len, qkv_for=qkv_for)
         return TemporalAdaptorOutput(enc_out=enc_out, log_duration=None, duration=duration_pred, dec_lengths=dec_lens,
                                      pitch=pitch.squeeze(-1), energy=energy.squeeze(-1), pitch_target=pitch_target,
                                      energy_target=energy_target, dec_mask=self.length_regulator.dec_mask)
diff --git a/isp_tts_amd/csrc/glue.hip b/isp_tts_amd/csrc/glue.hip
--- a/isp_tts_amd/csrc/glue.hip
+++ b/isp_tts_amd/csrc/glue.hip
@@ -13,6 +13,27 @@
     const f32x4* src = reinterpret_cast<const f32x4*>(table + id * ld_table);
     f32x4* dst = reinterpret_cast<f32x4*>(emb + (int64_t)row * D);
     for (int c = lane; c < D / 4; c += 64) dst[c] = src[c];
+    if (mask && lane == 0) {
+        const int b = row / L, l = row - b * L;
+        mask[row] = text_len ? (uint8_t)(l < text_len[b]) : (uint8_t)1;
+    }
+}
+
+__global__ __launch_bounds__(256) void embed_tokens_qkv_kernel(const int64_t* __restrict__ text, const float* __restrict__ table,
+                                                               int64_t ld_table, int vocab, const int64_t* __restrict__ text_len,
+                                                               float* __restrict__ emb, uint8_t* __restrict__ mask,
+                                                               const uint16_t* __restrict__ qkv_table, int64_t ld_qkv_table,
+                                                               uint16_t* __restrict__ qkv, int rows, int L, int D, int N) {
+    const int row = blockIdx.x * 4 + (threadIdx.x >> 6), lane = threadIdx.x & 63;
+    if (row >= rows) return;
+    int64_t id = text[row];
+    id = (id < 0 || id >= vocab) ? 0 : id;
+    const f32x4* src = reinterpret_cast<const f32x4*>(table + id * ld_table);
+    f32x4* dst = reinterpret_cast<f32x4*>(emb + (int64_t)row * D);
+    for (int c = lane; c < D / 4; c += 64) dst[c] = src[c];
+    const f32x4* qsrc = reinterpret_cast<const f32x4*>(qkv_table + id * ld_qkv_table);
+    f32x4* qdst = reinterpret_cast<f32x4*>(qkv + (int64_t)row * N);
+    for (int c = lane; c < N / 8; c += 64) qdst[c] = qsrc[c];
     if (mask && lane == 0) {
         const int b = row / L, l = row - b * L;
         mask[row] = text_len ? (uint8_t)(l < text_len[b]) : (uint8_t)1;
@@ -203,21 +224,39 @@
         return __builtin_amdgcn_mfma_f32_32x32x16_bf16(a, b, c, 0, 0, 0);
 }
 
-template <int NT, int kSplit = 0>
-__global__ __launch_bounds__(256) void length_regulate_kernel(const float* __restrict__ align, const float* __restrict__ dur_f,
-                                                              const int64_t* __restrict__ dur_i,
-                                                              const int64_t* __restrict__ enc_len,
-                                                              const float* __restrict__ x, int64_t ldx,
-                                                              float* __restrict__ out, int64_t* __restrict__ dec_len,
-                                                              uint8_t* __restrict__ dec_mask, int M, int L, int max_len,
-                                                              int dur_cols) {
+struct LrQkv {
+    const float* gamma;
+    const float* beta;
+    float eps;
+    const uint16_t* w;
+    uint16_t* qkv;
+    int64_t ld;
+};
+constexpr int kLrQkvN = 512, kLrQkvLd = kLrQkvN + 8, kLrQkvDepth = 3;
+constexpr size_t kLrQkvLds = 16 + (size_t)kLrRows * kLrQkvLd * 2 + (4 * kLrRows + 2 * kLrRows) * sizeof(float);
+
+template <int NT, int kSplit, bool kQkv>
+__device__ __forceinline__ void length_regulate_body(const float* __restrict__ align, const float* __restrict__ dur_f,
+                                                     const int64_t* __restrict__ dur_i, const int64_t* __restrict__ enc_len,
+                                                     const float* __restrict__ x, int64_t ldx, float* __restrict__ out,
+                                                     int64_t* __restrict__ dec_len, uint8_t* __restrict__ dec_mask, int M, int L,
+                                                     int max_len, int dur_cols, const LrQkv& q) {
     constexpr int D = 128 * NT;
     extern __shared__ __attribute__((aligned(16))) char smem[];
     int64_t& s_dec = *reinterpret_cast<int64_t*>(smem);
     float* As = reinterpret_cast<float*>(smem + 16);
     float* Xs = As + kLrRows * kLrAld;
     float* cum = Xs + kLrChunk * D;
-    const int b = blockIdx.y, y0 = blockIdx.x * kLrRows, tid = threadIdx.x, lane = tid & 63, wave = __builtin_amdgcn_readfirstlane(tid >> 6);
+    int b = blockIdx.y, bx = blockIdx.x;
+    if constexpr (kQkv) {
+        const int gx = gridDim.x, lin = blockIdx.y * gx + blockIdx.x, run = lin / (8 * gx);
+        if ((run + 1) * 8 <= (int)gridDim.y) {
+            const int r = lin - run * 8 * gx;
+            b = run * 8 + (r & 7);
+            bx = r >> 3;
+        }
+    }
+    const int y0 = bx * kLrRows, tid = threadIdx.x, lane = tid & 63, wave = __builtin_amdgcn_readfirstlane(tid >> 6);
     const bool soft = align == nullptr;
 
     if (wave == 0) {
@@ -243,7 +282,7 @@
         if (max_len >= 0 && dl > max_len) dl = max_len;
         if (lane == 0) {
             s_dec = dl;
-            if (blockIdx.x == 0) dec_len[b] = dl;
+            if (bx == 0) dec_len[b] = dl;
         }
     }
     __syncthreads();
@@ -351,6 +390,146 @@
                 const int y = y0 + rt * 32 + (i & 3) + 8 * (i >> 2) + 4 * (lane >> 5);
                 if (y < M) ob[(int64_t)y * D + wave * (32 * NT) + ct * 32 + (lane & 31)] = acc[rt][ct][i];
             }
+
+    if constexpr (kQkv) {
+        static_assert(NT == 3 && kSplit == 1, "the q/kv epilogue is built for dim 384 on the bf16 path");
+        constexpr int kSteps = D / 16, kAld = D + 8, kRing = kLrQkvDepth + 1;
+        uint16_t* An = reinterpret_cast<uint16_t*>(smem + 16);
+        uint16_t* Qs = An;
+        float* red = reinterpret_cast<float*>(smem + 16 + kLrRows * kLrQkvLd * 2);
+        float* stat = red + 4 * kLrRows;
+        const int r = lane & 31, kh = lane >> 5;
+        const uint16_t* wl = q.w + ((int64_t)(wave * 128 + r) * 16 + 8 * kh);
+        bf16x8 bq[kRing][4];
+        auto wload = [&](int s_, bf16x8 (&dst)[4]) {
+#pragma unroll
+            for (int ct = 0; ct < 4; ++ct)
+                dst[ct] = *reinterpret_cast<const bf16x8*>(wl + ((int64_t)s_ * kLrQkvN + ct * 32) * 16);
+        };
+        auto butterfly = [&](float (&v)[32]) {
+            static_for<0, 5>([&](auto st) {
+                constexpr int h = 16 >> decltype(st)::value;
+                const bool up = (lane & h) != 0;
+#pragma unroll
+                for (int k = 0; k < h; ++k) {
+                    const float keep = up ? v[k + h] : v[k], send = up ? v[k] : v[k + h];
+                    v[k] = keep + __shfl_xor(send, h, 64);
+                }
+            });
+        };
+        const int own = 32 * (r >> 4) + (r & 3) + 8 * ((r & 15) >> 2) + 4 * kh;
+        float v[32];
+#pragma unroll
+        for (int rt = 0; rt < 2; ++rt)
+#pragma unroll
+            for (int i = 0; i < 16; ++i) v[16 * rt + i] = (acc[rt][0][i] + acc[rt][1][i]) + acc[rt][2][i];
+        butterfly(v);
+        __syncthreads();
+        red[wave * kLrRows + own] = v[0];
+        __syncthreads();
+        if (tid < kLrRows) stat[tid] = ((red[tid] + red[kLrRows + tid]) + (red[2 * kLrRows + tid] + red[3 * kLrRows + tid])) * (1.0f / D);
+        __syncthreads();
+        auto rows4 = [&](const float* p, int rt, int g) { return *reinterpret_cast<const f32x4*>(p + 32 * rt + 8 * g + 4 * kh); };
+#pragma unroll
+        for (int rt = 0; rt < 2; ++rt)
+#pragma unroll
+            for (int g = 0; g < 4; ++g) {
+                const f32x4 m = rows4(stat, rt, g);
+#pragma unroll
+                for (int e = 0; e < 4; ++e) {
+                    const int i = 4 * g + e;
+                    const float d0 = acc[rt][0][i] - m[e], d1 = acc[rt][1][i] - m[e], d2 = acc[rt][2][i] - m[e];
+                    v[16 * rt + i] = (d0 * d0 + d1 * d1) + d2 * d2;
+                }
+            }
+        butterfly(v);
+#pragma unroll
+        for (int s_ = 0; s_ < kLrQkvDepth; ++s_) wload(s_, bq[s_]);
+        red[wave * kLrRows + own] = v[0];
+        __syncthreads();
+        if (tid < kLrRows) {
+            const float var = ((red[tid] + red[kLrRows + tid]) + (red[2 * kLrRows + tid] + red[3 * kLrRows + tid])) * (1.0f / D);
+            stat[kLrRows + tid] = 1.0f / sqrtf(var + q.eps);
+        }
+        __syncthreads();
+        float ga[NT], be[NT];
+#pragma unroll
+        for (int ct = 0; ct < NT; ++ct) {
+            ga[ct] = q.gamma[wave * (32 * NT) + ct * 32 + r];
+            be[ct] = q.beta[wave * (32 * NT) + ct * 32 + r];
+        }
+#pragma unroll
+        for (int rt = 0; rt < 2; ++rt)
+#pragma unroll
+            for (int g = 0; g < 4; ++g) {
+                const f32x4 m = rows4(stat, rt, g), rs = rows4(stat + kLrRows, rt, g);
+#pragma unroll
+                for (int e = 0; e < 4; ++e) {
+                    const int i = 4 * g + e, row = 32 * rt + 8 * g + 4 * kh + e;
+#pragma unroll
+                    for (int ct = 0; ct < NT; ++ct)
+                        An[row * kAld + wave * (32 * NT) + ct * 32 + r] = f32_to_bf16((acc[rt][ct][i] - m[e]) * rs[e] * ga[ct] + be[ct]);
+                }
+            }
+        __syncthreads();
+        f32x16 qa[2][4];
+#pragma unroll
+        for (int rt = 0; rt < 2; ++rt)
+#pragma unroll
+            for (int ct = 0; ct < 4; ++ct)
+#pragma unroll
+                for (int i = 0; i < 16; ++i) qa[rt][ct][i] = 0.f;
+        static_assert(kSteps % kRing == 0, "the ring is walked in whole turns");
+#pragma unroll 1
+        for (int s0 = 0; s0 < kSteps; s0 += kRing)
+            static_for<0, kRing>([&](auto s_) {
+                constexpr int S = decltype(s_)::value;
+                if (s0 + S + kLrQkvDepth < kSteps) wload(s0 + S + kLrQkvDepth, bq[(S + kLrQkvDepth) % kRing]);
+                const bf16x8 a0 = *reinterpret_cast<const bf16x8*>(An + r * kAld + 16 * (s0 + S) + 8 * kh);
+                const bf16x8 a1 = *reinterpret_cast<const bf16x8*>(An + (32 + r) * kAld + 16 * (s0 + S) + 8 * kh);
+#pragma unroll
+                for (int ct = 0; ct < 4; ++ct) {
+                    qa[0][ct] = __builtin_amdgcn_mfma_f32_32x32x16_bf16(a0, bq[S][ct], qa[0][ct], 0, 0, 0);
+                    qa[1][ct] = __builtin_amdgcn_mfma_f32_32x32x16_bf16(a1, bq[S][ct], qa[1][ct], 0, 0, 0);
+                }
+            });
+        __syncthreads();
+#pragma unroll
+        for (int rt = 0; rt < 2; ++rt)
+#pragma unroll
+            for (int ct = 0; ct < 4; ++ct)
+#pragma unroll
+                for (int i = 0; i < 16; ++i)
+                    Qs[(32 * rt + (i & 3) + 8 * (i >> 2) + 4 * kh) * kLrQkvLd + wave * 128 + ct * 32 + r] = f32_to_bf16(qa[rt][ct][i]);
+        __syncthreads();
+        uint16_t* qb = q.qkv + (int64_t)b * M * q.ld;
+        for (int row = wave; row < kLrRows; row += 4)
+            if (y0 + row < M)
+                *reinterpret_cast<u32x4*>(qb + (int64_t)(y0 + row) * q.ld + lane * 8) =
+                    *reinterpret_cast<const u32x4*>(Qs + row * kLrQkvLd + lane * 8);
+    }
+}
+
+template <int NT, int kSplit = 0>
+__global__ __launch_bounds__(256) void length_regulate_kernel(const float* __restrict__ align, const float* __restrict__ dur_f,
+                                                              const int64_t* __restrict__ dur_i,
+                                                              const int64_t* __restrict__ enc_len,
+                                                              const float* __restrict__ x, int64_t ldx,
+                                                              float* __restrict__ out, int64_t* __restrict__ dec_len,
+                                                              uint8_t* __restrict__ dec_mask, int M, int L, int max_len,
+                                                              int dur_cols) {
+    length_regulate_body<NT, kSplit, false>(align, dur_f, dur_i, enc_len, x, ldx, out, dec_len, dec_mask, M, L, max_len, dur_cols,
+                                            LrQkv{});
+}
+
+__global__ __launch_bounds__(256, 2) void length_regulate_qkv_kernel(const float* __restrict__ align, const float* __restrict__ dur_f,
+                                                                     const int64_t* __restrict__ dur_i,
+                                                                     const int64_t* __restrict__ enc_len,
+                                                                     const float* __restrict__ x, int64_t ldx,
+                                                                     float* __restrict__ out, int64_t* __restrict__ dec_len,
+                                                                     uint8_t* __restrict__ dec_mask, int M, int L, int max_len,
+                                                                     int dur_cols, LrQkv q) {
+    length_regulate_body<3, 1, true>(align, dur_f, dur_i, enc_len, x, ldx, out, dec_len, dec_mask, M, L, max_len, dur_cols, q);
 }
 
 }
@@ -367,6 +546,26 @@
     const int rows = B * L;
     hipLaunchKernelGGL(embed_tokens_kernel, dim3((rows + 3) / 4), dim3(256), 0, reinterpret_cast<hipStream_t>(stream), text,
                        table, ld_table, vocab, text_len, emb, mask, rows, L, D);
+    return ispk_launch_status();
+}
+
+extern "C" int32_t ispk_embed_tokens_qkv(const int64_t* text, const float* table, int64_t ld_table, int32_t vocab,
+                                         const int64_t* text_len, float* emb, uint8_t* mask, const uint16_t* qkv_table,
+                                         int64_t ld_qkv_table, uint16_t* qkv, int32_t B, int32_t L, int32_t D, int32_t N,
+                                         ispk_stream_t stream) {
+    ISPK_REQUIRE(text && table && emb && qkv_table && qkv, ISPK_E_NULL, "embed_tokens_qkv: null pointer");
+    ISPK_REQUIRE(B >= 0 && L >= 1 && D >= 4 && N >= 8 && vocab >= 1, ISPK_E_SHAPE,
+                 "embed_tokens_qkv: bad shape B=%d L=%d D=%d N=%d V=%d", B, L, D, N, vocab);
+    ISPK_REQUIRE((int64_t)B * L <= INT32_MAX, ISPK_E_SHAPE, "embed_tokens_qkv: B * L = %lld rows exceed int32",
+                 (long long)B * L);
+    ISPK_REQUIRE(D % 4 == 0 && ld_table % 4 == 0 && ld_table >= D && ispk_aligned(table, 16) && ispk_aligned(emb, 16),
+                 ISPK_E_ALIGN, "embed_tokens_qkv: D / ld_table must be multiples of 4 and table / emb 16-byte aligned");
+    ISPK_REQUIRE(N % 8 == 0 && ld_qkv_table % 8 == 0 && ld_qkv_table >= N && ispk_aligned(qkv_table, 16) && ispk_aligned(qkv, 16),
+                 ISPK_E_ALIGN, "embed_tokens_qkv: N / ld_qkv_table must be multiples of 8 and qkv_table / qkv 16-byte aligned");
+    if (B == 0) return 0;
+    const int rows = B * L;
+    hipLaunchKernelGGL(embed_tokens_qkv_kernel, dim3((rows + 3) / 4), dim3(256), 0, reinterpret_cast<hipStream_t>(stream), text,
+                       table, ld_table, vocab, text_len, emb, mask, qkv_table, ld_qkv_table, qkv, rows, L, D, N);
     return ispk_launch_status();
 }
 
@@ -439,7 +638,7 @@
 static int32_t length_regulate_launch(const float* alignment, const float* dur_f32, const int64_t* dur_i64, const int64_t* enc_len,
                                       const float* x, int64_t ldx, float* out, int64_t* dec_len, uint8_t* dec_mask, int32_t B,
                                       int32_t M, int32_t L, int32_t D, int32_t max_len, int32_t dur_cols, ispk_stream_t stream,
-                                      int split) {
+                                      int split, const LrQkv* qkv = nullptr) {
     ISPK_REQUIRE(x && out && dec_len, ISPK_E_NULL, "length_regulate: null pointer");
     ISPK_REQUIRE((dur_f32 != nullptr) != (dur_i64 != nullptr), ISPK_E_NULL,
                  "length_regulate: exactly one of dur_f32 / dur_i64 must be given");
@@ -461,6 +660,17 @@
         hipLaunchKernelGGL((length_regulate_kernel<NT_, SP_>), grid, dim3(256), lds, s, alignment, dur_f32, dur_i64, enc_len, x, \
                            ldx, out, dec_len, dec_mask, M, L, max_len, dur_cols);                                      \
     } while (0)
+    if (qkv) {
+        ISPK_REQUIRE(qkv->gamma && qkv->beta && qkv->w && qkv->qkv, ISPK_E_NULL, "length_regulate_qkv: null pointer");
+        ISPK_REQUIRE(D == 384 && split == 1, ISPK_E_UNSUPPORTED, "length_regulate_qkv: dim %d (built for 384, bf16 terms)", D);
+        ISPK_REQUIRE(qkv->ld >= kLrQkvN && qkv->ld % 8 == 0 && ispk_aligned(qkv->qkv, 16) && ispk_aligned(qkv->w, 16), ISPK_E_ALIGN,
+                     "length_regulate_qkv: ld_qkv must be a multiple of 8 and >= 512, qkv / Wqkv_chunks 16-byte aligned");
+        const size_t lds_q = lds > kLrQkvLds ? lds : kLrQkvLds;
+        ISPK_RESERVE_LDS((&length_regulate_qkv_kernel), lds_q, "length_regulate_qkv");
+        hipLaunchKernelGGL(length_regulate_qkv_kernel, grid, dim3(256), lds_q, s, alignment, dur_f32, dur_i64, enc_len, x, ldx, out,
+                           dec_len, dec_mask, M, L, max_len, dur_cols, *qkv);
+        return ispk_launch_status();
+    }
     if (D == 384) { if (split == 2) ISPK_LR(3, 2); else if (split) ISPK_LR(3, 1); else ISPK_LR(3, 0); }
     else { if (split == 2) ISPK_LR(2, 2); else if (split) ISPK_LR(2, 1); else ISPK_LR(2, 0); }
 #undef ISPK_LR
@@ -483,6 +693,17 @@
                                   stream, 1);
 }
 
+extern "C" int32_t ispk_length_regulate_qkv_bf16(const float* alignment, const float* dur_f32, const int64_t* dur_i64,
+                                                 const int64_t* enc_len, const float* x, int64_t ldx, float* out,
+                                                 int64_t* dec_len, uint8_t* dec_mask, const float* norm_gamma,
+                                                 const float* norm_beta, float norm_eps, const uint16_t* Wqkv_chunks, uint16_t* qkv,
+                                                 int64_t ld_qkv, int32_t B, int32_t M, int32_t L, int32_t D, int32_t max_len,
+                                                 int32_t dur_cols, ispk_stream_t stream) {
+    const LrQkv q{norm_gamma, norm_beta, norm_eps, Wqkv_chunks, qkv, ld_qkv};
+    return length_regulate_launch(alignment, dur_f32, dur_i64, enc_len, x, ldx, out, dec_len, dec_mask, B, M, L, D, max_len, dur_cols,
+                                  stream, 1, &q);
+}
+
 extern "C" int32_t ispk_length_regulate_split_f16(const float* alignment, const float* dur_f32, const int64_t* dur_i64,
                                                   const int64_t* enc_len, const float* x, int64_t ldx, float* out,
                                                   int64_t* dec_len, uint8_t* dec_mask, int32_t B, int32_t M, int32_t L,
diff --git a/isp_tts_amd/graph.py b/isp_tts_amd/graph.py
--- a/isp_tts_amd/graph.py
+++ b/isp_tts_amd/graph.py
@@ -88,6 +88,10 @@
                            "flow_time": flow_time.clone() if flow_time is not None else torch.rand(b, device=dev)}
         self.model, self.side = model, torch.cuda.Stream(device=dev, priority=side_priority)
         frames = mel.shape[2]
+        st = model.forward_front(s["text"], s["text_len"], s["mel"], s["mel_len"], s["pitch"], s["energy"])
+        model.forward_side(st, s["text_len"], s["mel_len"], s["pitch"], s["energy"], s["flow_noise"], s["flow_time"])
+        model.forward_back(st, s["text_len"], s["mel_len"], frames)
+        torch.cuda.synchronize()
         self.g_front = GraphedCall(lambda: model.forward_front(s["text"], s["text_len"], s["mel"], s["mel_len"], s["pitch"],
                                                                s["energy"]), warmup)
         st = self.g_front.out
diff --git a/isp_tts_amd/modules/transformer/transformer.py b/isp_tts_amd/modules/transformer/transformer.py
--- a/isp_tts_amd/modules/transformer/transformer.py
+++ b/isp_tts_amd/modules/transformer/transformer.py
@@ -201,7 +201,7 @@
                 context_mask: Optional[Tensor] = None, attention_mask: Optional[Tensor] = None,
                 adaptive_condition: Optional[Tensor] = None, return_intermediates: bool = False, *,
                 key_len: Optional[Tensor] = None, projected: Optional[Tensor] = None,
-                out_dtype: torch.dtype = torch.float32, final_norm: bool = True):
+                out_dtype: torch.dtype = torch.float32, final_norm: bool = True, handed: Handed = Handed()):
         if projected is not None:
             out = projected
         elif isinstance(self.project_emb, nn.Identity):
@@ -212,7 +212,6 @@
             key_len = mask.sum(dim=1)
         intermediates = []
         ada = self._ada_all(adaptive_condition) if (self.adaptive_norm and adaptive_condition is not None) else None
-        handed = Handed()
         for li, layer in enumerate(self.layers):
             res = layer(out, mask=mask, context=context, context_mask=context_mask, attention_mask=attention_mask,
                         adaptive_condition=adaptive_condition, key_len=key_len, ada=None if ada is None else ada[li],
diff --git a/isp_tts_amd/runtime.py b/isp_tts_amd/runtime.py
--- a/isp_tts_amd/runtime.py
+++ b/isp_tts_amd/runtime.py
@@ -78,12 +78,15 @@
     "ispk_hard_regulate_bwd_f32": [_P, _P, _P, _P, _I32, _I32, _I32, _I32, _I32, _P],
     "ispk_hard_average_f32": [_P, _P, _P, _P, _P, _I32, _I32, _I32, _P],
     "ispk_embed_tokens_f32": [_P, _P, _I64, _I32, _P, _P, _P, _I32, _I32, _I32, _P],
+    "ispk_embed_tokens_qkv": [_P, _P, _I64, _I32, _P, _P, _P, _P, _I64, _P, _I32, _I32, _I32, _I32, _P],
     "ispk_add_speaker_f32": [_P, _P, _I64, _I32, _P, _I32, _I32, _I32, _I32, _P],
     "ispk_add_speaker_out_f32": [_P, _P, _P, _I64, _I32, _P, _I32, _I32, _I32, _I32, _P],
     "ispk_speaker_grad_f32": [_P, _P, _I32, _P, _P, _I64, _P, _I64, _I32, _I32, _I32, _I32, _I32, _P],
     "ispk_time_embedding_f32": [_P, _I32, _P, _P, _I32, _P, _P, _P, _P, _I32, _P, _P],
     "ispk_length_regulate_f32": [_P, _P, _P, _P, _P, _I64, _P, _P, _P, _I32, _I32, _I32, _I32, _I32, _I32, _P],
     "ispk_length_regulate_split_bf16": [_P, _P, _P, _P, _P, _I64, _P, _P, _P, _I32, _I32, _I32, _I32, _I32, _I32, _P],
+    "ispk_length_regulate_qkv_bf16": [_P, _P, _P, _P, _P, _I64, _P, _P, _P, _P, _P, _F32, _P, _P, _I64, _I32, _I32, _I32, _I32, _I32,
+                                      _I32, _P],
     "ispk_length_regulate_split_f16": [_P, _P, _P, _P, _P, _I64, _P, _P, _P, _I32, _I32, _I32, _I32, _I32, _I32, _P],
     "ispk_pad_rows_f32": [_P, _I64, _I64, _I64, _P, _P, _I32, _I32, _I32, _I32, _P],
     "ispk_masked_instnorm_f32": [_P, _P, _P, _P, _P, _I32, _I32, _I32, _I32, _F32, _P],
@@ -956,6 +959,25 @@
     return emb, mask
 
 
+def embed_tokens_qkv(text: Tensor, table: Tensor, qkv_table: Tensor, text_len: Optional[Tensor] = None, want_mask: bool = True):
+    _dev(text, table, qkv_table, text_len)
+    assert text.dtype == torch.int64 and text.ndim == 2 and table.dtype == torch.float32 and table.stride(1) == 1
+    B, L = text.shape
+    V, D = table.shape
+    N = qkv_table.shape[1]
+    assert qkv_table.dtype == torch.bfloat16 and qkv_table.shape == (V, N) and qkv_table.stride(1) == 1
+    text = text.contiguous()
+    emb = torch.empty((B, L, D), dtype=torch.float32, device=text.device)
+    qkv = torch.empty((B, L, N), dtype=torch.bfloat16, device=text.device)
+    mask = torch.empty((B, L), dtype=torch.bool, device=text.device) if want_mask else None
+    if text_len is not None:
+        text_len = text_len.to(torch.int64).contiguous()
+    _launch("embed_tokens_qkv_kernel", 0.0, B * L * (8.0 * D + 4.0 * N), lib().ispk_embed_tokens_qkv, text.data_ptr(),
+            table.data_ptr(), table.stride(0), V, _ptr(text_len), emb.data_ptr(), _ptr(mask), qkv_table.data_ptr(),
+            qkv_table.stride(0), qkv.data_ptr(), B, L, D, N, _stream())
+    return emb, mask, qkv
+
+
 def _speaker_ids(speaker: Tensor, B: int):
     assert speaker.dtype == torch.int64
     if speaker.numel() == 1:
@@ -1023,7 +1045,7 @@
 
 
 def length_regulate(x: Tensor, durations: Tensor, alignment: Optional[Tensor], frames: int, max_len: int = -1,
-                    enc_len: Optional[Tensor] = None, want_mask: bool = True, split_bf16=False):
+                    enc_len: Optional[Tensor] = None, want_mask: bool = True, split_bf16=False, next_qkv: Optional[tuple] = None):
     _dev(x, durations, alignment, enc_len)
     assert x.dtype == torch.float32 and x.ndim == 3
     if x.stride(2) != 1 or x.stride(0) != x.shape[1] * x.stride(1):
@@ -1047,6 +1069,18 @@
     dec_len = torch.empty((B,), dtype=torch.int64, device=x.device)
     mask = torch.empty((B, frames), dtype=torch.bool, device=x.device) if want_mask else None
     nb = 4.0 * B * (frames * D + L * D + (frames * L if alignment is not None else 0))
+    if next_qkv is not None:
+        gamma, beta, eps, wqc = next_qkv
+        _dev(gamma, beta, wqc)
+        assert split_bf16 is True and D == 384, "the q/kv epilogue is built for the bf16 path at dim 384"
+        assert wqc.dtype == torch.bfloat16 and wqc.shape == (D // 16, 512, 16) and wqc.is_contiguous()
+        assert gamma.dtype == beta.dtype == torch.float32 and gamma.numel() == beta.numel() == D
+        qkv = torch.empty((B, frames, 512), dtype=torch.bfloat16, device=x.device)
+        _launch("length_regulate_qkv_kernel", 2.0 * B * frames * (L + 512) * D, nb + 2.0 * (B * frames * 512 + 512 * D),
+                lib().ispk_length_regulate_qkv_bf16, _ptr(alignment), _ptr(dur_f), _ptr(dur_i), _ptr(enc_len), x.data_ptr(),
+                x.stride(1), out.data_ptr(), dec_len.data_ptr(), _ptr(mask), gamma.data_ptr(), beta.data_ptr(), float(eps),
+                wqc.data_ptr(), qkv.data_ptr(), 512, B, frames, L, D, max_len, dur_cols, _stream())
+        return out, dec_len, mask, qkv
     fn = (lib().ispk_length_regulate_split_f16 if split_bf16 == "f16" else
           lib().ispk_length_regulate_split_bf16 if split_bf16 else lib().ispk_length_regulate_f32)
     _launch("length_regulate_kernel<split_f16>" if split_bf16 == "f16" else "length_regulate_kernel<bf16x3>" if split_bf16
```

After: 16.45 million mel-frames/s, median of 6. 2.0% higher.
